# Emanem/spath

Measured on AMD Instinct MI355X. Metric: Mray/s (primary x spp x bounces), higher is better.
Workload: dtype f32 (stage-1 filter: f16 hi/lo products on the matrix pipe, f32 accumulate)

## Files before the change

spath_amd/csrc/sp_cyl_scan.h:

```cpp
#pragma once

#include "sp_kernels.h"
#include "sp_filter_scan.h"

namespace sp {

#ifndef SP_CYL_TILE
#define SP_CYL_TILE 384
#endif
constexpr uint32_t kCylTile = SP_CYL_TILE;
static_assert(kCylTile % 128 == 0, "whole waves per LDS-DMA pass, whole words of group bits");
constexpr uint32_t kCylTileQ = 2u * kCylTile;
constexpr uint32_t kCylGroups = kCylTile / 4u;
SP_DEV constexpr uint32_t cyl_slot(uint32_t group, uint32_t chunk) { return chunk * kCylGroups + group; }

struct CylStream {
	const float4* rec;
	const uint32_t* hdr;
	const float4* big;
};

SP_DEV void cyl_store(float4* __restrict__ tile, uint32_t grp, uint32_t u, const float4 q0, const float4 q1) {
	tile[cyl_slot(grp, u)] = q0;
	float* mh = (float*)(tile + cyl_slot(grp, 4u + (u >> 1))) + 2u * (u & 1u);
	mh[0] = q1.x; mh[1] = q1.y;
	((float*)(tile + cyl_slot(grp, 6u)))[u] = q1.z;
	if (u == 0u) tile[cyl_slot(grp, 7u)] = make_float4(0.0f, 0.0f, 0.0f, 0.0f);
}

struct CylGroup {
	float4 q0[4];
	float4 mh01, mh23;
};
SP_DEV CylGroup cyl_group(const float4* tile, uint32_t grp) {
	CylGroup G;
#pragma unroll
	for (int u = 0; u < 4; ++u) G.q0[u] = tile[cyl_slot(grp, (uint32_t)u)];
	G.mh01 = tile[cyl_slot(grp, 4u)]; G.mh23 = tile[cyl_slot(grp, 5u)];
	return G;
}
SP_DEV float cyl_mz(const CylGroup& G, int u) { return u == 0 ? G.mh01.x : u == 1 ? G.mh01.z : u == 2 ? G.mh23.x : G.mh23.z; }
SP_DEV float cyl_h(const CylGroup& G, int u) { return u == 0 ? G.mh01.y : u == 1 ? G.mh01.w : u == 2 ? G.mh23.y : G.mh23.w; }

SP_DEV int cyl_record(const float* __restrict__ t, uint32_t idx, float4& q0, float4& q1) {
	const double A[3] = { t[0], t[1], t[2] }, B[3] = { t[3], t[4], t[5] }, C[3] = { t[6], t[7], t[8] };
	const double e1[3] = { (double)(t[3] - t[0]), (double)(t[4] - t[1]), (double)(t[5] - t[2]) };
	const double e2[3] = { (double)(t[6] - t[0]), (double)(t[7] - t[1]), (double)(t[8] - t[2]) };
	const double c[3] = { e2[0] - e1[0], e2[1] - e1[1], e2[2] - e1[2] };
	const double l1 = e1[0] * e1[0] + e1[1] * e1[1] + e1[2] * e1[2];
	const double l2 = e2[0] * e2[0] + e2[1] * e2[1] + e2[2] * e2[2];
	const double lc = c[0] * c[0] + c[1] * c[1] + c[2] * c[2];
	const double* w3; const double* p0; const double* p1; double len2;
	if (l2 >= l1 && l2 >= lc) { w3 = e2; p0 = A; p1 = B; len2 = l2; }
	else if (l1 >= lc)        { w3 = e1; p0 = A; p1 = C; len2 = l1; }
	else                      { w3 = c;  p0 = B; p1 = A; len2 = lc; }
	const double len = sqrt(len2);
	const double w[3] = { w3[0] / len, w3[1] / len, w3[2] / len };
	const double ax = fabs(w[0]), ay = fabs(w[1]), az = fabs(w[2]);
	const int a = (ax >= ay && ax >= az) ? 0 : (ay >= az ? 1 : 2);
	const int b = a == 2 ? 0 : a + 1, cc = b == 2 ? 0 : b + 1;
	const double s = 1.0 / w[a];
	const double pc[3] = { 0.5 * (p0[0] + p1[0]), 0.5 * (p0[1] + p1[1]), 0.5 * (p0[2] + p1[2]) };
	const double ph[3] = { 0.5 * (p1[0] - p0[0]), 0.5 * (p1[1] - p0[1]), 0.5 * (p1[2] - p0[2]) };
	const double mc[3] = { (w[1] * pc[2] - w[2] * pc[1]) * s, (w[2] * pc[0] - w[0] * pc[2]) * s, (w[0] * pc[1] - w[1] * pc[0]) * s };
	const double hv[3] = { (w[1] * ph[2] - w[2] * ph[1]) * s, (w[2] * ph[0] - w[0] * ph[2]) * s, (w[0] * ph[1] - w[1] * ph[0]) * s };
	const float beta = (float)(w[b] * s), gamma = (float)(w[cc] * s);
	const float mx = (float)mc[0], my = (float)mc[1], mz = (float)mc[2];
	float H = (float)(sqrt(hv[0] * hv[0] + hv[1] * hv[1] + hv[2] * hv[2]) * (1.0 + 0x1p-20));
	const float chk = beta + gamma + mx + my + mz + H;
	const bool ok = (chk - chk) == 0.0f;
	q0 = ok ? make_float4(beta, gamma, mx, my) : make_float4(0.0f, 0.0f, 0.0f, 0.0f);
	q1 = make_float4(ok ? mz : 0.0f, ok ? H : __builtin_inff(), __uint_as_float(idx), 0.0f);
	return ok ? a : 0;
}

SP_DEV int cyl_class(const float* __restrict__ t) {
	float4 q0, q1;
	return cyl_record(t, 0u, q0, q1);
}

__global__ void __launch_bounds__(256) k_cyl_count(const float* __restrict__ tris, uint32_t n, uint32_t* __restrict__ block_counts) {
	const uint32_t i = blockIdx.x * 256u + threadIdx.x;
	const int cls = i < n ? cyl_class(tris + (size_t)i * 12) : -1;
#pragma unroll
	for (int k = 0; k < 3; ++k) {
		const int cnt = __syncthreads_count(cls == k);
		if (threadIdx.x == 0) block_counts[(size_t)blockIdx.x * 3 + k] = (uint32_t)cnt;
	}
}

__global__ void __launch_bounds__(256) k_cyl_offsets(uint32_t* __restrict__ block_counts, uint32_t nblocks, uint32_t* __restrict__ hdr, uint32_t tile_sz) {
	__shared__ uint32_t part[256];
	__shared__ uint32_t total[3];
	const uint32_t tid = threadIdx.x;
	const uint32_t per = (nblocks + 255u) / 256u;
	const uint32_t lo = tid * per < nblocks ? tid * per : nblocks, hi = lo + per < nblocks ? lo + per : nblocks;
	for (int k = 0; k < 3; ++k) {
		uint32_t sum = 0;
		for (uint32_t b = lo; b < hi; ++b) sum += block_counts[(size_t)b * 3 + k];
		part[tid] = sum;
		__syncthreads();
		if (tid == 0) {
			uint32_t run = 0;
			for (int j = 0; j < 256; ++j) { const uint32_t v = part[j]; part[j] = run; run += v; }
			total[k] = run;
		}
		__syncthreads();
		uint32_t run = part[tid];
		for (uint32_t b = lo; b < hi; ++b) { const uint32_t v = block_counts[(size_t)b * 3 + k]; block_counts[(size_t)b * 3 + k] = run; run += v; }
		__syncthreads();
	}
	if (tid == 0) {
		uint32_t tile = 0;
		for (int k = 0; k < 3; ++k) { hdr[k] = total[k]; hdr[3 + k] = tile; tile += (total[k] + tile_sz - 1u) / tile_sz; }
		hdr[6] = tile;
	}
}

__global__ void __launch_bounds__(256) k_cyl_scatter(const float* __restrict__ tris, uint32_t n, const uint32_t* __restrict__ block_offsets,
                                                    const uint32_t* __restrict__ hdr, float4* __restrict__ rec) {
	__shared__ uint32_t wave_cnt[4][3];
	const uint32_t tid = threadIdx.x, i = blockIdx.x * 256u + tid, wv = tid >> 6, lane = tid & 63u;
	float4 q0, q1;
	q0 = q1 = make_float4(0.0f, 0.0f, 0.0f, 0.0f);
	const int cls = i < n ? cyl_record(tris + (size_t)i * 12, i, q0, q1) : -1;
	uint32_t rank = 0;
#pragma unroll
	for (int k = 0; k < 3; ++k) {
		const unsigned long long m = __ballot(cls == k);
		if (cls == k) rank = (uint32_t)__popcll(m & ((1ull << lane) - 1ull));
		if (lane == 0) wave_cnt[wv][k] = (uint32_t)__popcll(m);
	}
	__syncthreads();
	if (cls >= 0) {
		for (uint32_t v = 0; v < wv; ++v) rank += wave_cnt[v][cls];
		const size_t pos = (size_t)hdr[3 + cls] * kCylTile + block_offsets[(size_t)blockIdx.x * 3 + cls] + rank;
		const size_t tile = pos / kCylTile;
		const uint32_t in_tile = (uint32_t)(pos - tile * kCylTile), grp = in_tile >> 2, u = in_tile & 3u;
		cyl_store(rec + tile * kCylTileQ, grp, u, q0, q1);
	}
}

__global__ void __launch_bounds__(256) k_cyl_pad(const uint32_t* __restrict__ hdr, uint32_t n_tris, float4* __restrict__ rec) {
	const uint32_t k = blockIdx.x, tid = threadIdx.x;
	const uint32_t n = hdr[k], first = hdr[3 + k] * kCylTile;
	for (uint32_t pos = n + tid; pos < (n + kCylTile - 1u) / kCylTile * kCylTile; pos += 256u) {
		const size_t gpos = (size_t)first + pos, tile = gpos / kCylTile;
		const uint32_t in_tile = (uint32_t)(gpos - tile * kCylTile), grp = in_tile >> 2, u = in_tile & 3u;
		cyl_store(rec + tile * kCylTileQ, grp, u, make_float4(0.0f, 0.0f, 0.0f, 0.0f), make_float4(0.0f, -__builtin_inff(), __uint_as_float(n_tris), 0.0f));
	}
}

SP_DEV void cyl_tile_dma(const float4* __restrict__ src, float4* dst, uint32_t tid, uint32_t wbase) {
	typedef __attribute__((address_space(1))) const void* gptr_t;
	typedef __attribute__((address_space(3))) void* lptr_t;
	static_assert(kCylTileQ % 256 == 0, "whole workgroup passes");
#pragma unroll
	for (int p = 0; p < (int)(kCylTileQ / 256u); ++p)
		__builtin_amdgcn_global_load_lds((gptr_t)(src + p * 256 + tid), (lptr_t)(dst + p * 256 + wbase), 16, 0, 0);
}

SP_DEV float cyl_x(const float4 q0, float mz, float H, float Pa, float Pb, float Pc, float ndx, float ndy, float ndz, float D) {
	float gm = __builtin_fmaf(q0.x, Pb, Pa);
	gm = __builtin_fmaf(q0.y, Pc, gm);
	gm = __builtin_fmaf(ndx, q0.z, gm);
	gm = __builtin_fmaf(ndy, q0.w, gm);
	gm = __builtin_fmaf(ndz, mz, gm);
	return __builtin_fmaf(-H, D, __builtin_fabsf(gm));
}

template <int R>
struct CylRay {
	float Pa[R], Pb[R], Pc[R];
	float ndx[R], ndy[R], ndz[R];
	float D[R], Dq[R];
};

template <int R>
SP_DEV void cyl_setup(float rv, const RaySlots<R>& s, CylRay<R>& f) {
#pragma unroll
	for (int r = 0; r < R; ++r) {
		const f3 P = cross3(s.o[r], s.dir[r]);
		const float adx = fabsf(s.dir[r].x), ady = fabsf(s.dir[r].y), adz = fabsf(s.dir[r].z);
		const float dn = adx + ady + adz;
		const float on = fabsf(s.o[r].x) + fabsf(s.o[r].y) + fabsf(s.o[r].z);
		const float dmax = fmaxf(adx, fmaxf(ady, adz));
		const float mag = dn * (on + 2.0f * rv);
		const bool fin = (mag < 1e37f) && (dmax > 1e-18f) && (dmax < 1e18f);
		const bool on_ = fin && s.act[r];
		f.Pa[r] = on_ ? P.x : 0.0f; f.Pb[r] = on_ ? P.y : 0.0f; f.Pc[r] = on_ ? P.z : 0.0f;
		f.ndx[r] = on_ ? -s.dir[r].x : 0.0f; f.ndy[r] = on_ ? -s.dir[r].y : 0.0f; f.ndz[r] = on_ ? -s.dir[r].z : 0.0f;
		f.D[r] = on_ ? __builtin_sqrtf(s.dir[r].x * s.dir[r].x + s.dir[r].y * s.dir[r].y + s.dir[r].z * s.dir[r].z) * (1.0f + 0x1p-21f) : 1.0f;
		const float dq = fmaxf(0x1p-16f * 1.01f * mag * (1.0f + 0x1p-20f), 1e-37f);
		f.Dq[r] = !s.act[r] ? -__builtin_inff() : (fin ? dq : __builtin_inff());
	}
}

template <int R>
SP_DEV void scan_cyl(const KArgs& a, const CylStream cs, float rv, const RaySlots<R>& s, float (&bd)[R], int (&bi)[R]) {
	__shared__ float4 sm[2 * kCylTileQ];
	static_assert(R == 1 || R == 2 || R == 4, "bits per group must divide 32");
	constexpr uint32_t kGPW = 32u / R;
	constexpr int kNW = (int)((kCylTile / 4u) / kGPW);
	__shared__ uint32_t wq[kNW * 256];
	const uint32_t tid = threadIdx.x;
	const uint32_t wbase = tid & ~63u;

	CylRay<R> f;
	cyl_setup<R>(rv, s, f);
#pragma unroll
	for (int r = 0; r < R; ++r) { bd[r] = kMaxDist; bi[r] = -1; }

	const uint32_t total_tiles = cs.hdr[6];
	uint32_t cls = 0;
	__syncthreads();
	cyl_tile_dma(cs.rec, sm, tid, wbase);
	__syncthreads();
	for (uint32_t gt = 0; gt < total_tiles; ++gt) {
		while (cls < 2u && gt >= cs.hdr[4 + cls]) {
#pragma unroll
			for (int r = 0; r < R; ++r) { const float t0 = f.Pa[r]; f.Pa[r] = f.Pb[r]; f.Pb[r] = f.Pc[r]; f.Pc[r] = t0; }
			++cls;
		}
		const float4* cur = sm + (gt & 1u) * kCylTileQ;
		const uint32_t left = cs.hdr[cls] - (gt - cs.hdr[3 + cls]) * kCylTile;
		const uint32_t ngroups = (uint32_t)__builtin_amdgcn_readfirstlane((int)(((left < kCylTile ? left : kCylTile) + 3u) / 4u));
		uint32_t nz = 0;
		uint32_t g = 0;
#pragma unroll
		for (int wi = 0; wi < kNW; ++wi) {
			uint32_t wv = 0;
			const uint32_t gend = ngroups < (uint32_t)(wi + 1) * kGPW ? ngroups : (uint32_t)(wi + 1) * kGPW;
			const uint32_t g0 = g;
			for (; g < gend; ++g) {
				const CylGroup G = cyl_group(cur, g);
#pragma unroll
				for (int r = 0; r < R; ++r) {
					float x[4];
#pragma unroll
					for (int u = 0; u < 4; ++u) x[u] = cyl_x(G.q0[u], cyl_mz(G, u), cyl_h(G, u), f.Pa[r], f.Pb[r], f.Pc[r], f.ndx[r], f.ndy[r], f.ndz[r], f.D[r]);
					const float m = __builtin_fminf(__builtin_fminf(x[0], x[1]), __builtin_fminf(x[2], x[3]));
					wv = __builtin_amdgcn_alignbit(wv, __float_as_uint(m - f.Dq[r]), 31);
				}
			}
			const uint32_t done = (g - g0) * R;
			const uint32_t wd = done == 0u ? 0u : (wv << (32u - done));
			wq[wi * 256 + tid] = wd;
			nz |= (wd != 0u ? 1u : 0u) << wi;
		}
		if (gt + 1u < total_tiles) cyl_tile_dma(cs.rec + (size_t)(gt + 1u) * kCylTileQ, sm + ((gt + 1u) & 1u) * kCylTileQ, tid, wbase);
#ifdef SP_FILTER_STATS
		uint32_t st_bits = 0, st_rounds = 0, st_exact = 0;
#pragma unroll
		for (int wi = 0; wi < kNW; ++wi) st_bits += (uint32_t)__builtin_popcount(wq[wi * 256 + tid]);
#endif
		uint32_t sub = 0;
		uint32_t wid = nz ? (uint32_t)__builtin_ctz(nz) : 0u;
		uint32_t curw = nz ? wq[wid * 256 + tid] : 0u;
		for (;;) {
			if (!__any(nz != 0u)) break;
#ifdef SP_FILTER_STATS
			++st_rounds;
#endif
			if (nz != 0u) {
				const uint32_t nz2 = nz & (nz - 1u);
				const uint32_t wid2 = nz2 ? (uint32_t)__builtin_ctz(nz2) : 0u;
				const uint32_t nextw = wq[wid2 * 256 + tid];
				const uint32_t e = (uint32_t)__builtin_clz(curw);
				const uint32_t grp = wid * kGPW + e / R;
				const int slot = (int)(e % R);
				float Pa = f.Pa[0], Pb = f.Pb[0], Pc = f.Pc[0], ndx = f.ndx[0], ndy = f.ndy[0], ndz = f.ndz[0], D = f.D[0], Dq = f.Dq[0];
				float ox = s.o[0].x, oy = s.o[0].y, oz = s.o[0].z;
				float dx = s.dir[0].x, dy = s.dir[0].y, dz = s.dir[0].z;
				int src = s.src[0];
				float best = bd[0]; int besti = bi[0];
#pragma unroll
				for (int r = 1; r < R; ++r) {
					const bool pick = (slot == r);
					Pa = pick ? f.Pa[r] : Pa; Pb = pick ? f.Pb[r] : Pb; Pc = pick ? f.Pc[r] : Pc;
					ndx = pick ? f.ndx[r] : ndx; ndy = pick ? f.ndy[r] : ndy; ndz = pick ? f.ndz[r] : ndz;
					D = pick ? f.D[r] : D; Dq = pick ? f.Dq[r] : Dq;
					ox = pick ? s.o[r].x : ox; oy = pick ? s.o[r].y : oy; oz = pick ? s.o[r].z : oz;
					dx = pick ? s.dir[r].x : dx; dy = pick ? s.dir[r].y : dy; dz = pick ? s.dir[r].z : dz;
					src = pick ? s.src[r] : src;
					best = pick ? bd[r] : best; besti = pick ? bi[r] : besti;
				}
				uint32_t cand = 0; int idx = 0;
				const CylGroup G = cyl_group(cur, grp);
				const float4 gi = cur[cyl_slot(grp, 6u)];
#pragma unroll
				for (int u = 3; u >= 0; --u) {
					const float x = cyl_x(G.q0[u], cyl_mz(G, u), cyl_h(G, u), Pa, Pb, Pc, ndx, ndy, ndz, D);
					const bool sv = !(x - Dq >= 0.0f) && !((sub >> u) & 1u);
					cand = sv ? (cand | (1u << u)) : cand;
					idx = sv ? (int)__float_as_uint(u == 0 ? gi.x : u == 1 ? gi.y : u == 2 ? gi.z : gi.w) : idx;
				}
				const uint32_t lowest = cand & (0u - cand);
				const bool last = (cand == lowest);
				sub = last ? 0u : (sub | lowest);
				curw = last ? (curw & ~(0x80000000u >> e)) : curw;
				if (cand != 0u) {
#ifdef SP_FILTER_STATS
					++st_exact;
#endif
					const float4 x0 = a.scan[3 * (size_t)idx + 0], x1 = a.scan[3 * (size_t)idx + 1], x2 = a.scan[3 * (size_t)idx + 2];
					const float d = ray_tri_strict(mk3(ox, oy, oz), mk3(dx, dy, dz), mk3(x0.x, x0.y, x0.z), mk3(x0.w, x1.x, x1.y), mk3(x1.z, x1.w, x2.x));
					const bool take = (d > 0.0f) && (idx != src) && ((d < best) || (d == best && idx < besti));
					best = take ? d : best;
					besti = take ? idx : besti;
#pragma unroll
					for (int r = 0; r < R; ++r) { const bool pick = (slot == r); bd[r] = pick ? best : bd[r]; bi[r] = pick ? besti : bi[r]; }
				}
				const bool adv = (curw == 0u);
				nz = adv ? nz2 : nz;
				wid = adv ? wid2 : wid;
				curw = adv ? nextw : curw;
			}
		}
#ifdef SP_FILTER_STATS
		{
			uint32_t v = st_bits, x = st_exact;
			for (int off = 32; off > 0; off >>= 1) { v += __shfl_xor(v, off, 64); x += __shfl_xor(x, off, 64); }
// ... 171 lines not shown
```

spath_amd/csrc/sp_cylm_scan.h:

```cpp
#ifndef SP_CYLM_NS
#error "include sp_cylm_both.h, not this file"
#endif

namespace sp { namespace SP_CYLM_NS {

typedef _Float16 half8 __attribute__((ext_vector_type(8)));
typedef float float16v __attribute__((ext_vector_type(16)));

#ifndef SP_CYLM_TILE
#define SP_CYLM_TILE SP_CYLM_THREADS
#endif

constexpr uint32_t kMThreads = SP_CYLM_THREADS;
constexpr uint32_t kMWaves = kMThreads / 64u;
constexpr uint32_t kMTile = SP_CYLM_TILE;
constexpr uint32_t kMGroups = kMTile / 4u;
constexpr uint32_t kMBlocks = kMTile / 32u;
#ifndef SP_CYLM_GROUP
#define SP_CYLM_GROUP 4
#endif
constexpr uint32_t kMGrp = SP_CYLM_GROUP;
static_assert(kMGrp == 4u || kMGrp == 8u, "quads or octets (all sixteen rows of a lane as one group: -8 % / -4 % at 10^5 / 10^6 triangles against octets)");
constexpr uint32_t kMBitsFrag = 16u / kMGrp;
constexpr uint32_t kMFragsPerWord = 32u / kMBitsFrag;
constexpr uint32_t kMWords = (kMBlocks * kMBitsFrag + 31u) / 32u;
constexpr uint32_t kMRecQ = kMGroups * 8u;
constexpr uint32_t kMTileQ = kMRecQ + kMBlocks * 64u;
static_assert(kMThreads % 64u == 0u && kMThreads <= 1024u, "whole waves");
static_assert(kMTileQ % kMThreads == 0u, "whole workgroup LDS-DMA passes");
static_assert(kMGroups <= 128u, "7-bit group index in a list entry");
static_assert(kMBlocks * 2u <= kMGroups, "the Hmax table fits chunk 7");
SP_DEV constexpr uint32_t cylm_slot(uint32_t group, uint32_t chunk) { return chunk * kMGroups + group; }
SP_DEV constexpr uint32_t cylm_hmq(uint32_t tb, uint32_t hh) { return 7u * kMGroups + tb * 2u + hh; }
SP_DEV constexpr uint32_t cylm_kq() { return 7u * kMGroups + kMBlocks * 2u; }
static_assert(kMBlocks * 2u + 1u <= kMGroups, "Hmax table and kappa fit chunk 7");

SP_DEV float cylm_scale(float rv) {
	if (!(rv > 1e-30f && rv < 1e30f)) return 0.0f;
	const uint32_t e = (__float_as_uint(rv) >> 23) & 255u;
	return __uint_as_float((e + 2u) << 23);
}

SP_DEV _Float16 to_half(float v) {
	uint32_t b = (uint32_t)__builtin_bit_cast(unsigned short, (_Float16)v);
#ifndef SP_CYLM_UNPINNED
	__asm__ volatile("" : "+v"(b));
#endif
	return __builtin_bit_cast(_Float16, (unsigned short)b);
}

SP_DEV void half_split(float v, _Float16& hi, _Float16& lo) {
	hi = to_half(v);
	lo = to_half(v - (float)hi);
}

SP_DEV void cylm_store(float4* __restrict__ tile, uint32_t in_tile, const float4 q0, const float4 q1, float S) {
	const uint32_t grp = in_tile >> 2, u = in_tile & 3u;
	tile[cylm_slot(grp, u)] = q0;
	float* mh = (float*)(tile + cylm_slot(grp, 4u + (u >> 1))) + 2u * (u & 1u);
	mh[0] = q1.x; mh[1] = q1.y;
	((float*)(tile + cylm_slot(grp, 6u)))[u] = q1.z;
	const float m = S > 0.0f ? 16.0f / S : 0.0f;
	_Float16 bh, bl, ch, cl, xh, xl, yh, yl, zh, zl;
	half_split(S > 0.0f ? 16.0f * q0.x : 0.0f, bh, bl); half_split(S > 0.0f ? 16.0f * q0.y : 0.0f, ch, cl);
	half_split(q0.z * m, xh, xl); half_split(q0.w * m, yh, yl); half_split(q1.x * m, zh, zl);
	const _Float16 z = (_Float16)0.0f;
	const half8 k0 = { bh, bl, bh, ch, cl, ch, xh, xl }, k1 = { xh, yh, yl, yh, zh, zl, zh, S > 0.0f ? (_Float16)16.0f : z };
	half8* frag = (half8*)(tile + kMRecQ) + (in_tile >> 5) * 64u + (in_tile & 31u);
	frag[0] = k0; frag[32] = k1;
}

constexpr uint32_t kMBig = 64u;
constexpr int kMBigLevels = 4;

SP_DEV int cylm_big_level(float H, float S) {
	if (!(S > 0.0f) || !(H < __builtin_inff())) return -1;
	const float r = H / S;
	return r >= 1.0f ? 3 : r >= 0.25f ? 2 : r >= 0.0625f ? 1 : r >= 0.015625f ? 0 : -1;
}

__global__ void __launch_bounds__(256) k_cylm_count_big(const float* __restrict__ tris, uint32_t n, const unsigned int* __restrict__ bounds, uint32_t* __restrict__ hdr) {
	const uint32_t i = blockIdx.x * 256u + threadIdx.x;
	const float S = cylm_scale(__uint_as_float(bounds[0]));
	int lvl = -1;
	if (i < n) {
		float4 q0, q1;
		(void)cyl_record(tris + (size_t)i * 12, i, q0, q1);
		lvl = cylm_big_level(q1.y, S);
	}
#pragma unroll
	for (int k = 0; k < kMBigLevels; ++k) {
		const int cnt = __syncthreads_count(lvl >= k);
		if (threadIdx.x == 0 && cnt) atomicAdd(hdr + 9 + k, (uint32_t)cnt);
	}
}

SP_DEV int cylm_big_threshold(const uint32_t* __restrict__ hdr) {
	for (int k = 0; k < kMBigLevels; ++k) if (hdr[9 + k] <= kMBig) return k;
	return kMBigLevels;
}

__global__ void __launch_bounds__(256) k_cylm_keys(const float* __restrict__ tris, uint32_t n, const unsigned int* __restrict__ bounds, uint32_t* __restrict__ keys,
                                                  uint32_t* __restrict__ vals, uint32_t* __restrict__ hdr) {
	const uint32_t i = blockIdx.x * 256u + threadIdx.x;
	const float S = cylm_scale(__uint_as_float(bounds[0]));
	const int thr = cylm_big_threshold(hdr);
	int cls = -1;
	if (i < n) {
		float4 q0, q1;
		cls = cyl_record(tris + (size_t)i * 12, i, q0, q1);
		const int lvl = cylm_big_level(q1.y, S);
		if (lvl >= 0 && lvl >= thr) cls = 3;
		keys[i] = ((uint32_t)cls << 30) | (__float_as_uint(q1.y) >> 2);
		vals[i] = i;
	}
#pragma unroll
	for (int k = 0; k < 4; ++k) {
		const int cnt = __syncthreads_count(cls == k);
		if (threadIdx.x == 0 && cnt) atomicAdd(hdr + (k < 3 ? k : 8), (uint32_t)cnt);
	}
}

__global__ void k_cylm_hdr(uint32_t* __restrict__ hdr, const unsigned int* __restrict__ bounds) {
	uint32_t tile = 0;
	for (int k = 0; k < 3; ++k) { hdr[3 + k] = tile; tile += (hdr[k] + kMTile - 1u) / kMTile; }
	hdr[6] = tile;
	((float*)hdr)[7] = cylm_scale(__uint_as_float(bounds[0]));
}

__global__ void __launch_bounds__(256) k_cylm_scatter(const float* __restrict__ tris, uint32_t n, const uint32_t* __restrict__ sorted,
                                                     const uint32_t* __restrict__ hdr, float4* __restrict__ rec, const float4* __restrict__ scan, float4* __restrict__ big) {
	const uint32_t p = blockIdx.x * 256u + threadIdx.x;
	if (p >= n) return;
	const uint32_t i = sorted[p];
	const float S = ((const float*)hdr)[7];
	const uint32_t n_stream = hdr[0] + hdr[1] + hdr[2];
	if (p >= n_stream) {
		const uint32_t b = p - n_stream;
		const float4 x2 = scan[3 * (size_t)i + 2];
		big[3 * b + 0] = scan[3 * (size_t)i + 0]; big[3 * b + 1] = scan[3 * (size_t)i + 1];
		big[3 * b + 2] = make_float4(x2.x, __uint_as_float(i), 0.0f, 0.0f);
		return;
	}
	float4 q0, q1;
	const int cls = cyl_record(tris + (size_t)i * 12, i, q0, q1);
	const uint32_t c0 = cls == 0 ? 0u : cls == 1 ? hdr[0] : hdr[0] + hdr[1];
	const size_t pos = (size_t)hdr[3 + cls] * kMTile + (p - c0);
	const size_t tile = pos / kMTile;
	cylm_store(rec + tile * kMTileQ, (uint32_t)(pos - tile * kMTile), q0, q1, S);
}

__global__ void __launch_bounds__(256) k_cylm_pad(const uint32_t* __restrict__ hdr, uint32_t n_tris, float4* __restrict__ rec) {
	const uint32_t k = blockIdx.x, tid = threadIdx.x;
	const uint32_t n = hdr[k], first = hdr[3 + k] * kMTile;
	const float S = ((const float*)hdr)[7];
	for (uint32_t pos = n + tid; pos < (n + kMTile - 1u) / kMTile * kMTile; pos += 256u) {
		const size_t gpos = (size_t)first + pos, tile = gpos / kMTile;
		cylm_store(rec + tile * kMTileQ, (uint32_t)(gpos - tile * kMTile), make_float4(0.0f, 0.0f, 0.0f, 0.0f),
		           make_float4(0.0f, -__builtin_inff(), __uint_as_float(n_tris), 0.0f), S);
	}
}

__global__ void __launch_bounds__(kMGroups) k_cylm_hmax(const uint32_t* __restrict__ hdr, float4* __restrict__ rec) {
	__shared__ uint32_t s_max, s_min;
	__shared__ float s_h[kMGroups];
	if (blockIdx.x >= hdr[6]) return;
	if (threadIdx.x == 0) { s_max = 0u; s_min = 0x7f800000u; }
	float4* tile = rec + (size_t)blockIdx.x * kMTileQ;
	const uint32_t grp = threadIdx.x, tb = grp >> 3, j = (grp & 7u) >> 1, hh = grp & 1u;
	const float S = ((const float*)hdr)[7];
	const float k = S > 0.0f ? 256.0f / S : 1.0f;
	const float4 a = tile[cylm_slot(grp, 4u)], b = tile[cylm_slot(grp, 5u)];
	s_h[grp] = fmaxf(fmaxf(a.y, a.w), fmaxf(b.y, b.w)) * k;
	__syncthreads();
	float hm = kMGrp == 8u ? fmaxf(s_h[grp], s_h[grp ^ 2u]) : s_h[grp];
	const bool regular = hm >= 0.0f && hm < __builtin_inff();
	if (regular) atomicMax(&s_max, __float_as_uint(hm));
	__syncthreads();
	const float floor_ = fmaxf(__uint_as_float(s_max) * 0x1p-10f, 0x1p-60f);
	if (regular) { hm = fmaxf(hm, floor_); atomicMin(&s_min, __float_as_uint(hm)); }
	__syncthreads();
	if (kMGrp == 4u) ((float*)(tile + cylm_hmq(tb, hh)))[j] = hm;
	else if ((j & 1u) == 0u) ((float*)(tile + cylm_hmq(tb, hh)))[j >> 1] = hm;
	if (threadIdx.x == 0) {
		const float hmin = s_min == 0x7f800000u ? 1.0f : __uint_as_float(s_min);
		tile[cylm_kq()] = make_float4((1.0f / hmin) * (1.0f + 0x1p-20f), 0.0f, 0.0f, 0.0f);
	}
}

SP_DEV void cylm_tile_dma(const float4* __restrict__ src, float4* dst, uint32_t tid, uint32_t wbase) {
	typedef __attribute__((address_space(1))) const void* gptr_t;
	typedef __attribute__((address_space(3))) void* lptr_t;
#pragma unroll
	for (int p = 0; p < (int)(kMTileQ / kMThreads); ++p)
		__builtin_amdgcn_global_load_lds((gptr_t)(src + p * kMThreads + tid), (lptr_t)(dst + p * kMThreads + wbase), 16, 0, 0);
}

struct CylmGroup { float4 q0[4]; float4 mh01, mh23; };
SP_DEV CylmGroup cylm_group(const float4* tile, uint32_t grp) {
	CylmGroup G;
#pragma unroll
	for (int u = 0; u < 4; ++u) G.q0[u] = tile[cylm_slot(grp, (uint32_t)u)];
	G.mh01 = tile[cylm_slot(grp, 4u)]; G.mh23 = tile[cylm_slot(grp, 5u)];
	return G;
}

__global__ void __launch_bounds__(64) k_selftest_cylm(const float* __restrict__ in, uint32_t n, float* __restrict__ out) {
	const uint32_t i = blockIdx.x, lane = threadIdx.x, hh = lane >> 5;
	if (i >= n) return;
	const float* q = in + 12 * (size_t)i;
	_Float16 th[5], tl[5], rh[5], rl[5];
#pragma unroll
	for (int k = 0; k < 5; ++k) { half_split(q[k], th[k], tl[k]); half_split(q[5 + k], rh[k], rl[k]); }
	const _Float16 ah = to_half(q[10]), z = (_Float16)0.0f, one16 = (_Float16)16.0f;
	const half8 a0 = { th[0], tl[0], th[0], th[1], tl[1], th[1], th[2], tl[2] }, a1 = { th[2], th[3], tl[3], th[3], th[4], tl[4], th[4], one16 };
	const half8 b0 = { rh[0], rh[0], rl[0], rh[1], rh[1], rl[1], rh[2], rh[2] }, b1 = { rl[2], rh[3], rh[3], rl[3], rh[4], rh[4], rl[4], ah };
	const half8 zero8 = { z, z, z, z, z, z, z, z };
	const bool mine = (lane & 31u) == 0u;
	const half8 af = mine ? (hh ? a1 : a0) : zero8, bf = mine ? (hh ? b1 : b0) : zero8;
	float16v c;
#pragma unroll
	for (int k = 0; k < 16; ++k) c[k] = 0.0f;
	const float16v g = __builtin_amdgcn_mfma_f32_32x32x16_f16(af, bf, c, 0, 0, 0);
	if (lane == 0) {
		double sum = 0.0;
#pragma unroll
		for (int k = 0; k < 8; ++k) sum += (double)(float)a0[k] * (double)(float)b0[k] + (double)(float)a1[k] * (double)(float)b1[k];
		out[2 * (size_t)i] = g[0];
		out[2 * (size_t)i + 1] = (float)sum;
	}
}

struct CylmHdr {
	uint32_t n0, n1, n2, f1, f2, tiles;
	uint32_t nbig;
	float S;
	uint32_t cls, cn, cfirst, cend;
	SP_DEV void load(const uint32_t* __restrict__ hdr) {
		n0 = (uint32_t)__builtin_amdgcn_readfirstlane((int)hdr[0]); n1 = (uint32_t)__builtin_amdgcn_readfirstlane((int)hdr[1]);
		n2 = (uint32_t)__builtin_amdgcn_readfirstlane((int)hdr[2]);
		f1 = (uint32_t)__builtin_amdgcn_readfirstlane((int)hdr[4]); f2 = (uint32_t)__builtin_amdgcn_readfirstlane((int)hdr[5]);
		tiles = (uint32_t)__builtin_amdgcn_readfirstlane((int)hdr[6]);
		S = __uint_as_float((uint32_t)__builtin_amdgcn_readfirstlane((int)hdr[7]));
		nbig = (uint32_t)__builtin_amdgcn_readfirstlane((int)hdr[8]);
		cls = 0u; cn = n0; cfirst = 0u; cend = f1;
	}
	SP_DEV bool next_class(uint32_t gt) {
		if (cls >= 2u || gt < cend) return false;
		++cls;
		if (cls == 1u) { cn = n1; cfirst = f1; cend = f2; } else { cn = n2; cfirst = f2; cend = tiles; }
		return true;
	}
	SP_DEV uint32_t fragments(uint32_t gt) const {
		const uint32_t left = cn - (gt - cfirst) * kMTile;
		return ((left < kMTile ? left : kMTile) + 31u) / 32u;
	}
};

struct CylmRay {
	CylRay<1> f;
	float Pw[3], Nw[3];
	float Dh, Dqh;
	bool on_m;
	half8 bfr[2];
	float Dn[2], Dqn[2];

	SP_DEV void setup(float rv, float S, const RaySlots<1>& s) {
		cyl_setup<1>(rv, s, f);
		const float adx = fabsf(s.dir[0].x), ady = fabsf(s.dir[0].y), adz = fabsf(s.dir[0].z);
		const float on = fabsf(s.o[0].x) + fabsf(s.o[0].y) + fabsf(s.o[0].z);
		const float dmax = fmaxf(adx, fmaxf(ady, adz));
		const bool on0 = (f.Dq[0] < __builtin_inff()) && (f.Dq[0] > 0.0f) && (S > 0.0f) && (on + 2.0f * rv <= 512.0f * S);
		const uint32_t ed = (__float_as_uint(dmax) >> 23) & 255u;
		const float sd0 = on0 ? __uint_as_float((254u - ed) << 23) : 0.0f;
		const float kP0 = on0 ? sd0 * (16.0f / S) : 0.0f, kC0 = on0 ? sd0 * (256.0f / S) : 0.0f;
		on_m = on0 && (kC0 < 1e30f) && (kP0 > 1e-30f);
		const float s_d = on_m ? sd0 : 0.0f;
		const float kP = on_m ? kP0 : 0.0f, kN = 16.0f * s_d, kC = on_m ? kC0 : 0.0f;
		Dh = on_m ? f.D[0] * s_d : 1.0f;
		Dqh = on_m ? f.Dq[0] * kC : (s.act[0] ? __builtin_inff() : -__builtin_inff());
		Pw[0] = f.Pa[0] * kP; Pw[1] = f.Pb[0] * kP; Pw[2] = f.Pc[0] * kP;
		Nw[0] = f.ndx[0] * kN; Nw[1] = f.ndy[0] * kN; Nw[2] = f.ndz[0] * kN;
	}

	SP_DEV void build(uint32_t cls, uint32_t lane) {
		const uint32_t hh = lane >> 5;
		const float Pa_ = cls == 0u ? Pw[0] : cls == 1u ? Pw[1] : Pw[2];
		const float Pb_ = cls == 0u ? Pw[1] : cls == 1u ? Pw[2] : Pw[0], Pc_ = cls == 0u ? Pw[2] : cls == 1u ? Pw[0] : Pw[1];
		const _Float16 ah = to_half(Pa_);
		const float fa = (float)ah;
		const bool big = fabsf(Pa_) >= 0x1p-10f;
		const float t = big ? fa / Pa_ : 1.0f;
		const float extra = big ? 0.0f : fabsf(Pa_ - fa) * 16.0f;
		_Float16 bh, bl, ch, cl, nh[3], nl[3];
		half_split(Pb_ * t, bh, bl); half_split(Pc_ * t, ch, cl);
		half_split(Nw[0] * t, nh[0], nl[0]); half_split(Nw[1] * t, nh[1], nl[1]); half_split(Nw[2] * t, nh[2], nl[2]);
		const half8 k0 = { bh, bh, bl, ch, ch, cl, nh[0], nh[0] };
		const half8 k1 = { nl[0], nh[1], nh[1], nl[1], nh[2], nh[2], nl[2], ah };
		const float Dt = Dh * t;
		const float Dqt = on_m ? (Dqh * t + extra) * (1.0f + 0x1p-20f) : Dqh;
		typedef int int4v __attribute__((ext_vector_type(4)));
		const int4v v0 = __builtin_bit_cast(int4v, k0), v1 = __builtin_bit_cast(int4v, k1);
#pragma unroll
		for (int rb = 0; rb < 2; ++rb) {
			const int src = (int)((lane & 31u) + 32u * (uint32_t)rb);
			int4v o;
#pragma unroll
			for (int c = 0; c < 4; ++c) { const int va = __shfl(v0[c], src, 64), vb = __shfl(v1[c], src, 64); o[c] = hh ? vb : va; }
			bfr[rb] = __builtin_bit_cast(half8, o);
			Dn[rb] = __shfl(Dt, src, 64);
			Dqn[rb] = __shfl(Dqt, src, 64);
		}
	}
};

#ifndef SP_CYLM_MIN
#define SP_CYLM_MIN 1
#endif
SP_DEV float min4_abs(float a, float b, float c, float d) {
#if SP_CYLM_MIN == 1
	return __builtin_elementwise_minimum(__builtin_elementwise_minimum(__builtin_elementwise_minimum(__builtin_fabsf(a), __builtin_fabsf(b)), __builtin_fabsf(c)), __builtin_fabsf(d));
#elif SP_CYLM_MIN == 2
	return __builtin_fminf(__builtin_fminf(__builtin_amdgcn_fmed3f(__builtin_fabsf(a), __builtin_fabsf(b), 0.0f), __builtin_fabsf(c)), __builtin_fabsf(d));
#else
	return __builtin_fminf(__builtin_fminf(__builtin_fminf(__builtin_fabsf(a), __builtin_fabsf(b)), __builtin_fabsf(c)), __builtin_fabsf(d));
#endif
}

SP_DEV void cylm_tile_bound(const float4* cur, const CylmRay& R, float (&Dt)[2]) {
	const float kappa = cur[cylm_kq()].x;
#pragma unroll
	for (int rb = 0; rb < 2; ++rb) Dt[rb] = __builtin_fmaf(R.Dqn[rb], kappa, R.Dn[rb]) * (1.0f + 0x1p-22f);
}

SP_DEV float min8_abs(float a, float b, float c, float d, float e, float f, float g, float h) {
	typedef float T;
	const T m1 = __builtin_elementwise_minimum(__builtin_elementwise_minimum(__builtin_fabsf(a), __builtin_fabsf(b)), __builtin_fabsf(c));
	const T m2 = __builtin_elementwise_minimum(__builtin_elementwise_minimum(__builtin_fabsf(d), __builtin_fabsf(e)), __builtin_fabsf(f));
	const T m3 = __builtin_elementwise_minimum(__builtin_elementwise_minimum(m1, __builtin_fabsf(g)), __builtin_fabsf(h));
	return __builtin_elementwise_minimum(m3, m2);
}

SP_DEV uint32_t cylm_bits(const float16v& g, const float4 Hm, float Dt, uint32_t word) {
	if constexpr (kMGrp == 4u) {
#pragma unroll
		for (int j = 0; j < 4; ++j) {
			const float hm = j == 0 ? Hm.x : j == 1 ? Hm.y : j == 2 ? Hm.z : Hm.w;
			const float m = min4_abs(g[4 * j + 0], g[4 * j + 1], g[4 * j + 2], g[4 * j + 3]);
			word = __builtin_amdgcn_alignbit(word, __float_as_uint(__builtin_fmaf(-hm, Dt, m)), 31);
		}
	} else {
#pragma unroll
		for (int q = 0; q < 2; ++q) {
			const float hm = q == 0 ? Hm.x : Hm.y;
			const float m = min8_abs(g[8 * q + 0], g[8 * q + 1], g[8 * q + 2], g[8 * q + 3], g[8 * q + 4], g[8 * q + 5], g[8 * q + 6], g[8 * q + 7]);
			word = __builtin_amdgcn_alignbit(word, __float_as_uint(__builtin_fmaf(-hm, Dt, m)), 31);
		}
	}
	return word;
}

SP_DEV void cylm_stage1(const float4* cur, uint32_t tb0, uint32_t nblk, uint32_t lane, const CylmRay& R, const float (&Dt)[2], uint32_t (&word)[2]) {
	if (nblk == 0u) return;
	const half8* frags = (const half8*)(cur + kMRecQ) + tb0 * 64u + lane;
	const float4* hmq = cur + cylm_hmq(tb0, lane >> 5);
	float16v zero;
#pragma unroll
	for (int i = 0; i < 16; ++i) zero[i] = 0.0f;
#define SP_S1_STEP(afr_cur_Hm, afr_next)                                                     \
		__builtin_amdgcn_sched_barrier(0);                                                   \
		word[0] = cylm_bits(g0, afr_cur_Hm, Dt[0], word[0]);                                 \
		__builtin_amdgcn_sched_barrier(0);                                                   \
		g0 = __builtin_amdgcn_mfma_f32_32x32x16_f16(afr_next, R.bfr[0], zero, 0, 0, 0);      \
		__builtin_amdgcn_sched_barrier(0);                                                   \
		word[1] = cylm_bits(g1, afr_cur_Hm, Dt[1], word[1]);                                 \
		__builtin_amdgcn_sched_barrier(0);                                                   \
		g1 = __builtin_amdgcn_mfma_f32_32x32x16_f16(afr_next, R.bfr[1], zero, 0, 0, 0);
	half8 afrA = frags[0], afrB;
	float4 HmA = hmq[0], HmB;
	float16v g0 = __builtin_amdgcn_mfma_f32_32x32x16_f16(afrA, R.bfr[0], zero, 0, 0, 0);
	float16v g1 = __builtin_amdgcn_mfma_f32_32x32x16_f16(afrA, R.bfr[1], zero, 0, 0, 0);
	uint32_t tb = 1;
	for (; tb + 1u < nblk; tb += 2u) {
		afrB = frags[tb * 64u]; HmB = hmq[tb * 2u];
		SP_S1_STEP(HmA, afrB)
		afrA = frags[(tb + 1u) * 64u]; HmA = hmq[(tb + 1u) * 2u];
		SP_S1_STEP(HmB, afrA)
	}
	if (tb < nblk) {
		afrB = frags[tb * 64u]; HmB = hmq[tb * 2u];
		SP_S1_STEP(HmA, afrB)
		HmA = HmB;
	}
#undef SP_S1_STEP
	word[0] = cylm_bits(g0, HmA, Dt[0], word[0]);
	word[1] = cylm_bits(g1, HmA, Dt[1], word[1]);
}

constexpr uint32_t kMCap = 384u;
constexpr uint32_t kMQ2 = 128u;
constexpr uint32_t kMIdxBits = 26u;

SP_DEV float wave_fetch(uint32_t addr4, float v) { return __int_as_float(__builtin_amdgcn_ds_bpermute((int)addr4, __float_as_int(v))); }
SP_DEV int wave_fetch(uint32_t addr4, int v) { return __builtin_amdgcn_ds_bpermute((int)addr4, v); }

SP_DEV uint32_t wave_incl_scan(uint32_t x) {
	x += (uint32_t)__builtin_amdgcn_update_dpp(0, (int)x, 0x111, 0xf, 0xf, true);
	x += (uint32_t)__builtin_amdgcn_update_dpp(0, (int)x, 0x112, 0xf, 0xf, true);
	x += (uint32_t)__builtin_amdgcn_update_dpp(0, (int)x, 0x114, 0xf, 0xf, true);
	x += (uint32_t)__builtin_amdgcn_update_dpp(0, (int)x, 0x118, 0xf, 0xf, true);
	x += (uint32_t)__builtin_amdgcn_update_dpp(0, (int)x, 0x142, 0xa, 0xf, false);
	x += (uint32_t)__builtin_amdgcn_update_dpp(0, (int)x, 0x143, 0xc, 0xf, false);
	return x;
}

template <bool BOUNDED = false>
SP_DEV void scan_cylm(const KArgs& a, const CylStream cs, float rv, const RaySlots<1>& s, float (&bd)[1], int (&bi)[1],
                      const float* tmax = nullptr, bool shadow = false) {
	__shared__ float4 sm0[kMTileQ];
	__shared__ float4 sm1[kMTileQ];
	__shared__ unsigned short lst[kMWaves * kMCap];
	__shared__ uint32_t q2[kMWaves * kMQ2];
	__shared__ unsigned long long cell[kMThreads];
	const uint32_t tid = threadIdx.x, lane = tid & 63u, wbase = tid & ~63u, hh = lane >> 5;
	unsigned short* const mylst = lst + (tid >> 6) * kMCap;
	uint32_t* const myq2 = q2 + (tid >> 6) * kMQ2;
	CylmHdr hd;
	hd.load(cs.hdr);

	CylmRay R;
	R.setup(rv, hd.S, s);
	CylRay<1>& f = R.f;

	const float tm = tmax ? tmax[0] : kMaxDist;
	{
		float bd0 = tm; int bi0 = -1;
		typedef float f4v __attribute__((ext_vector_type(4)));
		typedef __attribute__((address_space(4))) const f4v* cptr_t;
		const cptr_t big = (cptr_t)(uintptr_t)cs.big;
		for (uint32_t b = 0; b < hd.nbig; ++b) {
			const f4v x0 = big[3 * b + 0], x1 = big[3 * b + 1], x2 = big[3 * b + 2];
			const int idx = (int)__float_as_uint(x2.y);
			const float d = ray_tri_strict(s.o[0], s.dir[0], mk3(x0.x, x0.y, x0.z), mk3(x0.w, x1.x, x1.y), mk3(x1.z, x1.w, x2.x));
			const bool take = (d > 0.0f) && (idx != s.src[0]) && ((d < bd0) || (d == bd0 && idx < bi0));
			bd0 = take ? d : bd0;
			bi0 = take ? idx : bi0;
		}
		cell[tid] = ((unsigned long long)__float_as_uint(bd0) << 32) | (unsigned long long)(uint32_t)bi0;
		if (BOUNDED && shadow && !s.act[0]) cell[tid] = 0ull;
	}
	R.build(0u, lane);

	uint32_t q2n = 0;
	auto exact_batch = [&](uint32_t n) {
#ifdef SP_EXP_NO_EXACT
		q2n -= n;
		return;
#endif
		const bool ok = lane < n;
		const uint32_t e = ok ? myq2[q2n - n + lane] : ((lane << kMIdxBits) | a.n_tris);
		const uint32_t la = (e >> (kMIdxBits - 2u)) & 0xfcu;
		const int idx = (int)(e & ((1u << kMIdxBits) - 1u));
		const float4* const rec = (const float4*)((const char*)a.scan + ((((uint32_t)idx << 1) + (uint32_t)idx) << 4));
		const float4 x0 = rec[0], x1 = rec[1], x2 = rec[2];
		const float ox = wave_fetch(la, s.o[0].x), oy = wave_fetch(la, s.o[0].y), oz = wave_fetch(la, s.o[0].z);
		const float dx = wave_fetch(la, s.dir[0].x), dy = wave_fetch(la, s.dir[0].y), dz = wave_fetch(la, s.dir[0].z);
		const int src = wave_fetch(la, s.src[0]);
		const float tmx = tmax ? wave_fetch(la, tm) : kMaxDist;
		const float d = ray_tri_strict(mk3(ox, oy, oz), mk3(dx, dy, dz), mk3(x0.x, x0.y, x0.z), mk3(x0.w, x1.x, x1.y), mk3(x1.z, x1.w, x2.x));
		if (ok && (d > 0.0f) && (d < tmx) && (idx != src))
			atomicMin(&cell[wbase + (la >> 2)], ((unsigned long long)__float_as_uint(d) << 32) | (unsigned long long)(uint32_t)idx);
		q2n -= n;
#ifdef SP_FILTER_STATS
		if (lane == 0) { atomicAdd(a.scans + 5, 1ull); atomicAdd(a.scans + 4, (unsigned long long)n); }
#endif
	};

	const uint32_t total_tiles = hd.tiles;
#ifdef SP_EXP_NO_STAGE2
	uint32_t exp_acc = 0;
#endif
#ifdef SP_PHASE_TIMERS
	unsigned long long ph_s1 = 0, ph_list = 0, ph_retest = 0, ph_exact = 0, ph_bar = 0, ph_t0 = 0, ph_t1 = 0;
#define SP_PH_STAMP(v) v = __builtin_amdgcn_s_memtime()
#define SP_PH_ADD(acc, a_, b_) acc += (b_) - (a_)
#else
#define SP_PH_STAMP(v)
#define SP_PH_ADD(acc, a_, b_)
#endif
	__syncthreads();
	cylm_tile_dma(cs.rec, sm0, tid, wbase);
	__syncthreads();
	auto tile_body = [&](auto parity, const uint32_t gt) {
		const float4* const cur = decltype(parity)::value ? sm1 : sm0;
		float4* const nxt = decltype(parity)::value ? sm0 : sm1;
#ifndef SP_CYLM_LATE_DMA
		if (gt + 1u < total_tiles) cylm_tile_dma(cs.rec + (size_t)(gt + 1u) * kMTileQ, nxt, tid, wbase);
#endif
		SP_PH_STAMP(ph_t0);
		while (hd.next_class(gt)) {
			const float t0 = f.Pa[0]; f.Pa[0] = f.Pb[0]; f.Pb[0] = f.Pc[0]; f.Pc[0] = t0;
			R.build(hd.cls, lane);
		}
		const uint32_t nblk = hd.fragments(gt);
		float Dt[2];
		cylm_tile_bound(cur, R, Dt);
		uint32_t word[kMWords][2];
#pragma unroll
		for (int w = 0; w < (int)kMWords; ++w) {
			word[w][0] = word[w][1] = 0u;
			const uint32_t tb0 = kMFragsPerWord * (uint32_t)w;
			const uint32_t nb = nblk > tb0 ? (nblk - tb0 < kMFragsPerWord ? nblk - tb0 : kMFragsPerWord) : 0u;
			cylm_stage1(cur, tb0, nb, lane, R, Dt, word[w]);
			const uint32_t done = nb * kMBitsFrag;
#pragma unroll
			for (int rb = 0; rb < 2; ++rb) word[w][rb] = done == 0u ? 0u : (word[w][rb] << (32u - done));
#ifdef SP_DBG_ALLBITS
			word[w][0] = word[w][1] = done == 0u ? 0u : (0xffffffffu << (32u - done));
#endif
		}
		if (BOUNDED && shadow) {
#pragma unroll
			for (int rb = 0; rb < 2; ++rb) {
				const bool fin = (uint32_t)cell[wbase + (lane & 31u) + 32u * (uint32_t)rb] != 0xffffffffu;
#pragma unroll
				for (int w = 0; w < (int)kMWords; ++w) word[w][rb] = fin ? 0u : word[w][rb];
			}
		}
		SP_PH_STAMP(ph_t1); SP_PH_ADD(ph_s1, ph_t0, ph_t1);
#ifdef SP_CYLM_LATE_DMA
		if (gt + 1u < total_tiles) cylm_tile_dma(cs.rec + (size_t)(gt + 1u) * kMTileQ, nxt, tid, wbase);
#endif
#ifdef SP_EXP_NO_STAGE2
		for (int w = 0; w < (int)kMWords; ++w) exp_acc ^= word[w][0] ^ word[w][1];
		for (; false;) {
#else
		for (;;) {
#endif
			uint32_t c = 0;
#pragma unroll
			for (int w = 0; w < (int)kMWords; ++w) c += (uint32_t)__builtin_popcount(word[w][0]) + (uint32_t)__builtin_popcount(word[w][1]);
			const uint32_t incl = wave_incl_scan(c);
			const uint32_t all = (uint32_t)__builtin_amdgcn_readlane((int)incl, 63);
			if (all == 0u) break;
			uint32_t j = incl - c;
			const uint32_t jend = incl < kMCap ? incl : kMCap;
			if (all <= kMCap) {
#pragma unroll
				for (int w = 0; w < (int)kMWords; ++w)
#pragma unroll
				for (int rb = 0; rb < 2; ++rb) {
					uint32_t m = word[w][rb];
					const uint32_t eb = (((lane & 31u) + 32u * (uint32_t)rb) << 2) | ((16u * kMGrp * (uint32_t)w + hh) << 8);
					while (m != 0u) {
						const uint32_t e = (uint32_t)__builtin_clz(m);
						mylst[j++] = (unsigned short)(eb + (e << (kMGrp == 8u ? 10 : 9)));
						m &= ~(0x80000000u >> e);
					}
					word[w][rb] = 0u;
				}
			} else
#pragma unroll
			for (int w = 0; w < (int)kMWords; ++w)
#pragma unroll
			for (int rb = 0; rb < 2; ++rb) {
				uint32_t m = word[w][rb];
				const uint32_t ray = (lane & 31u) + 32u * (uint32_t)rb;
				while (__any(m != 0u && j < jend)) {
					if (m != 0u && j < jend) {
						const uint32_t e = (uint32_t)__builtin_clz(m);
						mylst[j++] = (unsigned short)((ray << 2) | ((16u * kMGrp * (uint32_t)w + (kMGrp / 2u) * e + hh) << 8));
						m &= ~(0x80000000u >> e);
					}
				}
				word[w][rb] = m;
			}
			__builtin_amdgcn_wave_barrier();
			const uint32_t total = all < kMCap ? all : kMCap;
#ifdef SP_FILTER_STATS
			if (lane == 0) { atomicAdd(a.scans + 1, (unsigned long long)total); atomicAdd(a.scans + 2, (unsigned long long)((total + 63u) / 64u)); }
#endif
			SP_PH_STAMP(ph_t0); SP_PH_ADD(ph_list, ph_t1, ph_t0);
			for (uint32_t base = 0; base < total; base += 64u) {
				const uint32_t ent = base + lane;
				const bool ok = ent < total;
				const uint32_t entry = ok ? (uint32_t)mylst[ent] : (lane << 2);
				const uint32_t la = entry & 0xfcu;
				const uint32_t grp = entry >> 8;
				const float dx = wave_fetch(la, s.dir[0].x), dy = wave_fetch(la, s.dir[0].y), dz = wave_fetch(la, s.dir[0].z);
				const float Pa = wave_fetch(la, f.Pa[0]), Pb = wave_fetch(la, f.Pb[0]), Pc = wave_fetch(la, f.Pc[0]);
				const float D = wave_fetch(la, f.D[0]), Dq = wave_fetch(la, f.Dq[0]);
				uint32_t cand = 0;
#pragma unroll
				for (int h = 0; h < (int)(kMGrp / 4u); ++h) {
					const CylmGroup G = cylm_group(cur, grp + 2u * (uint32_t)h);
#pragma unroll
					for (int u = 0; u < 4; ++u) {
						const float mz = u == 0 ? G.mh01.x : u == 1 ? G.mh01.z : u == 2 ? G.mh23.x : G.mh23.z;
						const float Hh = u == 0 ? G.mh01.y : u == 1 ? G.mh01.w : u == 2 ? G.mh23.y : G.mh23.w;
						const float x = cyl_x(G.q0[u], mz, Hh, Pa, Pb, Pc, -dx, -dy, -dz, D);
						cand = __builtin_amdgcn_alignbit(cand, __float_as_uint(x - Dq), 31);
					}
				}
				cand = ok ? cand : 0u;
				SP_PH_STAMP(ph_t1); SP_PH_ADD(ph_retest, ph_t0, ph_t1);
				const uint32_t* const gidx = (const uint32_t*)(cur + cylm_slot(grp, 6u));
				const uint32_t lhi = la << (kMIdxBits - 2u);
				for (;;) {
					const bool mine = cand != 0u;
					const unsigned long long mk = __ballot(mine);
					if (mk == 0ull) break;
					const uint32_t cnt = (uint32_t)__popcll(mk);
					if (q2n + cnt > kMQ2) exact_batch(64u);
					const uint32_t k = mine ? (uint32_t)__builtin_ctz(cand) : kMGrp - 1u;
					const uint32_t u = kMGrp - 1u - k;
					const uint32_t idx = gidx[8u * (u >> 2) + (u & 3u)];
					if (mine) myq2[q2n + __builtin_amdgcn_mbcnt_hi((uint32_t)(mk >> 32), __builtin_amdgcn_mbcnt_lo((uint32_t)mk, 0u))] = lhi | idx;
					q2n += cnt;
					cand &= cand - 1u;
				}
				__builtin_amdgcn_wave_barrier();
				SP_PH_STAMP(ph_t0); SP_PH_ADD(ph_exact, ph_t1, ph_t0);
			}
			SP_PH_STAMP(ph_t1);
		}
#ifdef SP_EXP_DRAIN_ALL
		while (q2n) exact_batch(q2n < 64u ? q2n : 64u);
#else
		while (q2n >= 64u) exact_batch(64u);
#endif
#ifdef SP_FILTER_STATS
		if (lane == 0) atomicAdd(a.scans + 3, 1ull);
#endif
		SP_PH_STAMP(ph_t0); SP_PH_ADD(ph_list, ph_t1, ph_t0);
		if (BOUNDED && shadow) {
			__asm__ volatile("s_waitcnt vmcnt(0)" ::: "memory");
			if (!__syncthreads_or((uint32_t)cell[tid] == 0xffffffffu ? 1 : 0)) return false;
		} else
		__syncthreads();
		SP_PH_STAMP(ph_t1); SP_PH_ADD(ph_bar, ph_t0, ph_t1);
		return true;
	};
	if constexpr (BOUNDED) {
		bool all_done = false;
		for (uint32_t gt = 0; gt < total_tiles; gt += 2u) {
			if (!tile_body(std::integral_constant<int, 0>{}, gt)) { all_done = true; break; }
			if (gt + 1u < total_tiles && !tile_body(std::integral_constant<int, 1>{}, gt + 1u)) { all_done = true; break; }
		}
		if (q2n && !all_done) exact_batch(q2n);
	} else {
		for (uint32_t gt = 0; gt < total_tiles; gt += 2u) {
			tile_body(std::integral_constant<int, 0>{}, gt);
			if (gt + 1u < total_tiles) tile_body(std::integral_constant<int, 1>{}, gt + 1u);
		}
		if (q2n) exact_batch(q2n);
	}
#ifdef SP_PHASE_TIMERS
	if (lane == 0) {
		atomicAdd(a.scans + 8, ph_s1); atomicAdd(a.scans + 9, ph_list); atomicAdd(a.scans + 10, ph_retest); atomicAdd(a.scans + 11, ph_exact);
		atomicAdd(a.scans + 12, ph_bar); atomicAdd(a.scans + 13, 1ull);
	}
#endif
#ifdef SP_EXP_NO_STAGE2
	if (exp_acc == 0x12345678u) cell[tid] = 0ull;
#endif
	__builtin_amdgcn_wave_barrier();
	const unsigned long long k = cell[tid];
	bd[0] = __uint_as_float((uint32_t)(k >> 32));
	bi[0] = (int)(uint32_t)k;
}

__global__ void __launch_bounds__(64) k_selftest_stage1(const float* __restrict__ rays, uint32_t n_rays, const CylStream cs, const unsigned int* __restrict__ bounds,
                                                      uint32_t* __restrict__ out_words, uint32_t* __restrict__ out_tri, int* __restrict__ out_order) {
	__shared__ float4 sm[kMTileQ];
	const uint32_t lane = threadIdx.x, hh = lane >> 5;
	const float rv = __uint_as_float(bounds[0]);
	CylmHdr hd;
	hd.load(cs.hdr);
	const uint32_t k = blockIdx.x * 64u + lane, kk = k < n_rays ? k : n_rays - 1u;
	RaySlots<1> s;
	const float* p = rays + (size_t)kk * 6;
	s.o[0] = mk3(p[0], p[1], p[2]); s.dir[0] = mk3(p[3], p[4], p[5]); s.src[0] = -1; s.act[0] = true;
	CylmRay R;
	R.setup(rv, hd.S, s);
	R.build(0u, lane);
	const float kH = hd.S > 0.0f ? 256.0f / hd.S : 1.0f;
	const uint32_t total_tiles = hd.tiles;
	for (uint32_t gt = 0; gt < total_tiles; ++gt) {
		while (hd.next_class(gt)) R.build(hd.cls, lane);
		__syncthreads();
		for (uint32_t q = lane; q < kMTileQ; q += 64u) sm[q] = cs.rec[(size_t)gt * kMTileQ + q];
		__syncthreads();
		const uint32_t nblk = hd.fragments(gt);
		float Dt[2];
		cylm_tile_bound(sm, R, Dt);
		for (uint32_t w = 0; w < kMWords; ++w) {
			uint32_t word[2] = { 0u, 0u };
			const uint32_t tb0 = kMFragsPerWord * w;
			const uint32_t nb = nblk > tb0 ? (nblk - tb0 < kMFragsPerWord ? nblk - tb0 : kMFragsPerWord) : 0u;
			cylm_stage1(sm, tb0, nb, lane, R, Dt, word);
			const uint32_t done = nb * kMBitsFrag;
#pragma unroll
			for (int rb = 0; rb < 2; ++rb)
				if (k < n_rays) out_words[(((size_t)k * total_tiles + gt) * 2u + (uint32_t)rb) * kMWords + w] = done == 0u ? 0u : (word[rb] << (32u - done));
		}
		if (out_tri) {
			float16v zero;
#pragma unroll
			for (int i = 0; i < 16; ++i) zero[i] = 0.0f;
			for (uint32_t tb = 0; tb < kMBlocks; ++tb) {
				const half8 afr = ((const half8*)(sm + kMRecQ))[tb * 64u + lane];
				const float16v g0 = __builtin_amdgcn_mfma_f32_32x32x16_f16(afr, R.bfr[0], zero, 0, 0, 0);
				const float16v g1 = __builtin_amdgcn_mfma_f32_32x32x16_f16(afr, R.bfr[1], zero, 0, 0, 0);
#pragma unroll
				for (int rb = 0; rb < 2; ++rb) {
					const float16v& g = rb == 0 ? g0 : g1;
					uint32_t w = 0;
#pragma unroll
					for (int j = 0; j < 4; ++j) {
						const uint32_t grp = tb * 8u + 2u * (uint32_t)j + hh;
						const float4 a = sm[cylm_slot(grp, 4u)], b = sm[cylm_slot(grp, 5u)];
						const float H4[4] = { a.y * kH, a.w * kH, b.y * kH, b.w * kH };
#pragma unroll
						for (int i = 0; i < 4; ++i) {
							const float x = __builtin_fmaf(-H4[i], R.Dn[rb], __builtin_fabsf(g[4 * j + i]));
							w = __builtin_amdgcn_alignbit(w, __float_as_uint(x - R.Dqn[rb]), 31);
						}
					}
					if (k < n_rays) {
						uint32_t* o = out_tri + (((size_t)k * total_tiles + gt) * 2u + (uint32_t)rb) * (kMTile / 64u) + (tb >> 1);
						if (tb >= nblk) w = 0u;
						if ((tb & 1u) == 0u) *o = w << 16; else *o |= (w & 0xffffu);
					}
				}
			}
		}
		if (blockIdx.x == 0) {
			for (uint32_t grp = lane; grp < kMGroups; grp += 64u) {
				const float4 gi = sm[cylm_slot(grp, 6u)];
				int* o = out_order + (size_t)gt * kMTile + 4u * grp;
				o[0] = (int)__float_as_uint(gi.x); o[1] = (int)__float_as_uint(gi.y); o[2] = (int)__float_as_uint(gi.z); o[3] = (int)__float_as_uint(gi.w);
			}
		}
	}
}

} }
#undef SP_PH_STAMP
#undef SP_PH_ADD
```

spath_amd/csrc/spath_hip.hip:

```cpp
#include "spath_hip.h"
#include "sp_kernels.h"
#include "sp_filter_scan.h"
#include "sp_cyl_scan.h"
#include "sp_scan_kernels.h"
#include "sp_bvh.h"
#include "sp_bvh_build.h"
#include "sp_adaptive.h"
#include "sp_denoise.h"

#include <hip/hip_runtime.h>

#include <cstdarg>
#include <cstdlib>
#include <dlfcn.h>
#include <thread>
#include <mutex>
#include <cstdio>
#include <cstring>
#include <algorithm>
#include <cmath>
#include <string>
#include <vector>

namespace {

thread_local std::string g_create_error;

struct DevBuf {
	void* p = nullptr;
	size_t cap = 0;
};

}

struct sphip_ctx {
	int device = 0;
	hipStream_t own_stream = nullptr;
	hipEvent_t ev_k0 = nullptr, ev_k1 = nullptr, ev_u0 = nullptr, ev_u1 = nullptr, ev_d0 = nullptr, ev_d1 = nullptr;
	DevBuf tris, mats, scan, filt, bounds, samp, rays, rgba, accum, counter, work, bvh_nodes, bvh_rec, bvh_idx, sort_kv, sort_hist, bvh_meta, cyl_rec, cyl_cnt, cyl_hdr, prim, cylm_rec, cylm_hdr, cylm_big;
	bool bvh_valid = false, filt_valid = false, cyl_valid = false, cylm_valid = false;
	bool cylm_wide = false;
	uint32_t bvh_leaves = 0;
	size_t n_tris = 0;
	bool have_scene = false;
	bool have_render = false, timed_upload = false, timed_download = false;
	sphip_stats stats{};
	std::string err;
	std::string desc;
	hipStream_t last_stream = nullptr;
	std::vector<sphip_ctx*> kids;
	int gather_kind = SPHIP_GATHER_NONE;
	void* rccl_lib = nullptr;
	std::vector<void*> comms;
	DevBuf gath, gath_acc, img, img_acc;
	std::vector<hipEvent_t> ev_tile;
	hipEvent_t ev_g0 = nullptr, ev_g1 = nullptr;
	DevBuf acc_rays, acc_sum;
	bool acc_on = false;
	bool acc_stale = false;
	size_t acc_w = 0, acc_h = 0;
	uint64_t acc_seed = 0, acc_total = 0;
	int acc_flags = 0;
	DevBuf adp_s12, adp_cnt, adp_list[2], adp_rays, adp_keep, adp_blk, adp_nact_d, adp_wst;
	bool adp_on = false;
	int adp_cur = 0;
	uint32_t adp_nact = 0, adp_nact_rb = 0;
	double adp_t = 0.0, adp_floor = 0.0;
	uint32_t adp_min = 0;
	DevBuf dn_cls, dn_hit, dn_gbuf, dn_a, dn_b, dn_rays;
	bool dn_cls_valid = false;
	DevBuf nee_tab;
	bool nee_valid = false, nee_bad = false;
	uint32_t nee_n = 0;
	double nee_W = 0.0;
	std::string nee_msg;
	bool dn_gbuf_ok = false;
	sphip_lens lens{};
	sphip_lens acc_lens{};
	sphip_camera acc_cam{};
	bool acc_has_cam = false;
	DevBuf spec;
	bool have_spec = false;
};

namespace {

int fail(sphip_ctx* c, int code, const char* fmt, ...) {
	char buf[512];
	va_list ap;
	va_start(ap, fmt);
	vsnprintf(buf, sizeof buf, fmt, ap);
	va_end(ap);
	if (c) c->err = buf; else g_create_error = buf;
	return code;
}

#define HIP_TRY(c, expr)                                                                         \
	do {                                                                                         \
		hipError_t e_ = (expr);                                                                  \
		if (e_ != hipSuccess)                                                                    \
			return fail((c), SPHIP_E_DEVICE, "%s failed: %s (%s:%d)", #expr, hipGetErrorString(e_), __FILE__, __LINE__); \
	} while (0)

int ensure(sphip_ctx* c, DevBuf& b, size_t bytes) {
	if (bytes <= b.cap && b.p) return SPHIP_OK;
	if (b.p) { HIP_TRY(c, hipFree(b.p)); b.p = nullptr; b.cap = 0; }
	const size_t want = bytes < 256 ? 256 : bytes;
	HIP_TRY(c, hipMalloc(&b.p, want));
	b.cap = want;
	return SPHIP_OK;
}

constexpr int kVariantAccel = 8;
constexpr int kVariantLast = 16;
constexpr uint64_t kChunkTargetBlocks = 262144;
constexpr uint64_t kChunkMaxBytes = 16ull << 30;
const char* const kVariantNames[kVariantLast + 1] = { "auto", "rpl_sload", "rpl_lds", "rpl_filter2", "rpl_filter4", "rpl_filter1", "rpl_filter2s", "rpl_filter4s",
                                                      "accel_lbvh", "rpl_cyl1", "rpl_cyl2", "rpl_cyl4", "rpl_cyl2s", "rpl_cyl4s", "rpl_cylw4", "rpl_cylw4s", "rpl_cylm" };

struct TwoStage { int R; bool split; int scan; };
bool two_stage(int variant, TwoStage* out) {
	static const TwoStage tab[kVariantLast + 1] = { {0, false, 0}, {0, false, 0}, {0, false, 0}, {2, false, 0}, {4, false, 0}, {1, false, 0}, {2, true, 0}, {4, true, 0},
	                                                {0, false, 0}, {1, false, 1}, {2, false, 1}, {4, false, 1}, {2, true, 1}, {4, true, 1}, {4, false, 2}, {4, true, 2}, {1, false, 3} };
	if (variant < 0 || variant > kVariantLast || tab[variant].R == 0) return false;
	if (out) *out = tab[variant];
	return true;
}

constexpr bool shape_shipped(int R, bool split, int scan) { return scan >= 3 || (scan == 2 && R == 4 && split); }
bool variant_shipped(int v) {
	TwoStage ts;
	return v == 1 || v == 2 || v == kVariantAccel || (two_stage(v, &ts) && shape_shipped(ts.R, ts.split, ts.scan));
}
bool variant_built(int v) {
#ifdef SP_ALL_VARIANTS
	return v >= 1 && v <= kVariantLast;
#else
	return variant_shipped(v);
#endif
}

constexpr size_t kSlotHist = 40, kSlotAcc = 12, kSlotNeeL = 48, kSlotMisD = 60, kSlotAdaptWst = 16;
constexpr size_t work_slot_bytes(bool nee, bool mis) { return kSlotHist + kSlotAcc + (mis ? kSlotMisD : nee ? kSlotNeeL : 0); }

int pick_variant(int flags, size_t n_tris) {
	if (flags & SPHIP_FLAG_ACCEL) return kVariantAccel;
	const int v = flags & SPHIP_KERNEL_MASK;
	if (v >= 1 && v <= kVariantLast) return v;
	if (n_tris < 64) return 1;
	if (n_tris >= (1ull << sp::kMIdxBits)) return 15;
	return 16;
}

int repack(sphip_ctx* c, hipStream_t st) {
	const uint32_t n = (uint32_t)c->n_tris;
	const uint32_t n_pad = (n / sp::kTile + 1) * sp::kTile;
	int rc;
	if ((rc = ensure(c, c->scan, (size_t)n_pad * 48)) || (rc = ensure(c, c->bounds, 256))) return rc;
	HIP_TRY(c, hipMemsetAsync(c->bounds.p, 0, 256, st));
	hipLaunchKernelGGL(sp::k_repack, dim3((n_pad + 255) / 256), dim3(256), 0, st,
	                   (const float*)c->tris.p, (float4*)c->scan.p, (unsigned int*)c->bounds.p, n, n_pad);
	HIP_TRY(c, hipGetLastError());
	c->have_scene = true;
	c->bvh_valid = c->filt_valid = c->cyl_valid = c->cylm_valid = false;
	c->nee_valid = false;
	c->have_spec = false;
	return SPHIP_OK;
}

int radix_sort(sphip_ctx* c, uint32_t n, uint32_t key_bits, hipStream_t st, int* out_half) {
	const uint32_t rs_blocks = (n + sp::kRsPerBlock - 1) / sp::kRsPerBlock;
	int rc = ensure(c, c->sort_hist, (size_t)rs_blocks * 16 * 4);
	if (rc) return rc;
	uint32_t* keys[2] = { (uint32_t*)c->sort_kv.p, (uint32_t*)c->sort_kv.p + (size_t)n };
	uint32_t* vals[2] = { (uint32_t*)c->sort_kv.p + (size_t)2 * n, (uint32_t*)c->sort_kv.p + (size_t)3 * n };
	int cur = 0;
	for (uint32_t shift = 0; shift < key_bits; shift += 4, cur ^= 1) {
		hipLaunchKernelGGL(sp::k_rs_hist, dim3(rs_blocks), dim3(256), 0, st, (const uint32_t*)keys[cur], n, shift, rs_blocks, (uint32_t*)c->sort_hist.p);
		hipLaunchKernelGGL(sp::k_rs_scan, dim3(1), dim3(256), 0, st, (uint32_t*)c->sort_hist.p, rs_blocks * 16u);
		hipLaunchKernelGGL(sp::k_rs_scatter, dim3(rs_blocks), dim3(256), 0, st, (const uint32_t*)keys[cur], (const uint32_t*)vals[cur], n, shift, rs_blocks,
		                   (const uint32_t*)c->sort_hist.p, keys[cur ^ 1], vals[cur ^ 1]);
	}
	HIP_TRY(c, hipGetLastError());
	*out_half = cur;
	return SPHIP_OK;
}

template <bool WIDE>
int build_cylm(sphip_ctx* c, hipStream_t st) {
#define SP_CM(x) (WIDE ? sp::cylm512::x : sp::cylm256::x)
	const uint32_t n = (uint32_t)c->n_tris, nblocks = (n + 255) / 256, max_tiles = n / SP_CM(kMTile) + 4;
	int rc;
	if ((rc = ensure(c, c->sort_kv, (size_t)n * 16)) || (rc = ensure(c, c->cylm_hdr, 256)) || (rc = ensure(c, c->cylm_big, sp::cylm256::kMBig * 48)) ||
	    (rc = ensure(c, c->cylm_rec, (size_t)max_tiles * SP_CM(kMTileQ) * 16))) return rc;
	uint32_t* keys = (uint32_t*)c->sort_kv.p;
	uint32_t* vals = (uint32_t*)c->sort_kv.p + (size_t)2 * n;
	uint32_t* hdr = (uint32_t*)c->cylm_hdr.p;
	const float* tris = (const float*)c->tris.p;
	const unsigned int* bnd = (const unsigned int*)c->bounds.p;
	float4* rec = (float4*)c->cylm_rec.p;
	HIP_TRY(c, hipMemsetAsync(hdr, 0, 256, st));
	hipLaunchKernelGGL(sp::cylm256::k_cylm_count_big, dim3(nblocks), dim3(256), 0, st, tris, n, bnd, hdr);
	hipLaunchKernelGGL(sp::cylm256::k_cylm_keys, dim3(nblocks), dim3(256), 0, st, tris, n, bnd, keys, vals, hdr);
	int half = 0;
	if ((rc = radix_sort(c, n, 32, st, &half))) return rc;
	const uint32_t* sorted = vals + (size_t)half * n;
	if (WIDE) {
		hipLaunchKernelGGL(sp::cylm512::k_cylm_hdr, dim3(1), dim3(1), 0, st, hdr, bnd);
		hipLaunchKernelGGL(sp::cylm512::k_cylm_scatter, dim3(nblocks), dim3(256), 0, st, tris, n, sorted, (const uint32_t*)hdr, rec, (const float4*)c->scan.p, (float4*)c->cylm_big.p);
		hipLaunchKernelGGL(sp::cylm512::k_cylm_pad, dim3(3), dim3(256), 0, st, (const uint32_t*)hdr, n, rec);
		hipLaunchKernelGGL(sp::cylm512::k_cylm_hmax, dim3(max_tiles), dim3(sp::cylm512::kMGroups), 0, st, (const uint32_t*)hdr, rec);
	} else {
		hipLaunchKernelGGL(sp::cylm256::k_cylm_hdr, dim3(1), dim3(1), 0, st, hdr, bnd);
		hipLaunchKernelGGL(sp::cylm256::k_cylm_scatter, dim3(nblocks), dim3(256), 0, st, tris, n, sorted, (const uint32_t*)hdr, rec, (const float4*)c->scan.p, (float4*)c->cylm_big.p);
		hipLaunchKernelGGL(sp::cylm256::k_cylm_pad, dim3(3), dim3(256), 0, st, (const uint32_t*)hdr, n, rec);
		hipLaunchKernelGGL(sp::cylm256::k_cylm_hmax, dim3(max_tiles), dim3(sp::cylm256::kMGroups), 0, st, (const uint32_t*)hdr, rec);
	}
#undef SP_CM
	HIP_TRY(c, hipGetLastError());
	c->cylm_valid = true;
	c->cylm_wide = WIDE;
	return SPHIP_OK;
}

bool cylm_wants_wide(const sphip_ctx* c) {
	if (const char* e = getenv("SPATH_HIP_CYLM_SHAPE")) return atoi(e) == 512;
	return c->n_tris >= sp::kMBigSceneTris;
}

int ensure_cylm(sphip_ctx* c, hipStream_t st) {
	if (c->cylm_valid) return SPHIP_OK;
	return cylm_wants_wide(c) ? build_cylm<true>(c, st) : build_cylm<false>(c, st);
}

int ensure_cyl(sphip_ctx* c, hipStream_t st) {
	if (c->cyl_valid) return SPHIP_OK;
	const uint32_t n = (uint32_t)c->n_tris, nblocks = (n + 255) / 256;
	int rc;
	if ((rc = ensure(c, c->cyl_cnt, (size_t)nblocks * 3 * sizeof(uint32_t))) || (rc = ensure(c, c->cyl_hdr, 256)) ||
	    (rc = ensure(c, c->cyl_rec, ((size_t)n / sp::kCylTile + 4) * sp::kCylTile * 32))) return rc;
	hipLaunchKernelGGL(sp::k_cyl_count, dim3(nblocks), dim3(256), 0, st, (const float*)c->tris.p, n, (uint32_t*)c->cyl_cnt.p);
	hipLaunchKernelGGL(sp::k_cyl_offsets, dim3(1), dim3(256), 0, st, (uint32_t*)c->cyl_cnt.p, nblocks, (uint32_t*)c->cyl_hdr.p, sp::kCylTile);
	hipLaunchKernelGGL(sp::k_cyl_scatter, dim3(nblocks), dim3(256), 0, st, (const float*)c->tris.p, n, (const uint32_t*)c->cyl_cnt.p,
	                   (const uint32_t*)c->cyl_hdr.p, (float4*)c->cyl_rec.p);
	hipLaunchKernelGGL(sp::k_cyl_pad, dim3(3), dim3(256), 0, st, (const uint32_t*)c->cyl_hdr.p, n, (float4*)c->cyl_rec.p);
	HIP_TRY(c, hipGetLastError());
	c->cyl_valid = true;
	return SPHIP_OK;
}

#ifdef SP_ALL_VARIANTS
int ensure_filt(sphip_ctx* c, hipStream_t st) {
	if (c->filt_valid) return SPHIP_OK;
	const uint32_t n = (uint32_t)c->n_tris, n_pad = (n / sp::kTile + 1) * sp::kTile;
	int rc = ensure(c, c->filt, (size_t)n_pad * 48);
	if (rc) return rc;
	hipLaunchKernelGGL(sp::k_repack_filter, dim3((n_pad + 255) / 256), dim3(256), 0, st, (const float*)c->tris.p, (float4*)c->filt.p, n, n_pad);
	HIP_TRY(c, hipGetLastError());
	c->filt_valid = true;
	return SPHIP_OK;
}
#endif

int ensure_bvh(sphip_ctx* c, hipStream_t st) {
	if (c->bvh_valid) return SPHIP_OK;
	const uint32_t n = (uint32_t)c->n_tris;
	uint32_t nl = 1;
	while ((uint64_t)nl * 4 < n) nl <<= 1;
	const uint32_t nblocks = (n + 255) / 256;
	int rc;
	if ((rc = ensure(c, c->bvh_nodes, (size_t)2 * nl * 32)) || (rc = ensure(c, c->bvh_rec, ((size_t)nl * 4 + sp::kBvhMaxBig) * 48)) ||
	    (rc = ensure(c, c->bvh_idx, ((size_t)nl * 4 + sp::kBvhMaxBig) * 4)) || (rc = ensure(c, c->sort_kv, (size_t)n * 16)) ||
	    (rc = ensure(c, c->bvh_meta, 256))) return rc;
	uint32_t* meta = (uint32_t*)c->bvh_meta.p;
	uint32_t* vals[2] = { (uint32_t*)c->sort_kv.p + (size_t)2 * n, (uint32_t*)c->sort_kv.p + (size_t)3 * n };
	const float* tris = (const float*)c->tris.p;
	const dim3 b256(256);
	hipLaunchKernelGGL(sp::k_bvh_meta_init, dim3(1), b256, 0, st, meta);
	hipLaunchKernelGGL(sp::k_bvh_box, dim3(nblocks), b256, 0, st, tris, n, meta);
	hipLaunchKernelGGL(sp::k_bvh_count_big, dim3(nblocks), b256, 0, st, tris, n, meta);
	hipLaunchKernelGGL(sp::k_bvh_keys, dim3(nblocks), b256, 0, st, tris, n, meta, (uint32_t*)c->sort_kv.p, vals[0]);
	int cur = 0;
	if ((rc = radix_sort(c, n, 32, st, &cur))) return rc;
	hipLaunchKernelGGL(sp::k_bvh_leaves, dim3((nl + 255) / 256), b256, 0, st, tris, n, (const uint32_t*)meta, (const uint32_t*)vals[cur], nl,
	                   (float4*)c->bvh_nodes.p, (float4*)c->bvh_rec.p, (int*)c->bvh_idx.p);
	hipLaunchKernelGGL(sp::k_bvh_bigs, dim3(1), b256, 0, st, tris, n, (const uint32_t*)meta, (const uint32_t*)vals[cur], nl, (float4*)c->bvh_rec.p, (int*)c->bvh_idx.p);
	for (uint32_t first = nl >> 1; first >= 1; first >>= 1)
		hipLaunchKernelGGL(sp::k_bvh_refit, dim3((first + 255) / 256), b256, 0, st, (float4*)c->bvh_nodes.p, first);
	HIP_TRY(c, hipGetLastError());
	c->bvh_leaves = nl;
	c->bvh_valid = true;
	return SPHIP_OK;
}

int ensure_lights(sphip_ctx* c, hipStream_t st) {
	if (c->nee_valid) return c->nee_bad ? fail(c, SPHIP_E_INVALID, "%s", c->nee_msg.c_str()) : SPHIP_OK;
	const size_t n = c->n_tris;
	std::vector<float> t(n * 12), m(n * 6);
	HIP_TRY(c, hipMemcpyAsync(t.data(), c->tris.p, n * 48, hipMemcpyDeviceToHost, st));
	HIP_TRY(c, hipMemcpyAsync(m.data(), c->mats.p, n * 24, hipMemcpyDeviceToHost, st));
	HIP_TRY(c, hipStreamSynchronize(st));
	std::vector<double> cdf;
	std::vector<int> tri;
	std::vector<float> ipdf;
	std::vector<double> esum;
	double W = 0.0;
	c->nee_bad = false;
	for (size_t i = 0; i < n; ++i) {
		const float* e = &m[i * 6 + 3];
		for (int k = 0; k < 3; ++k)
			if (!(e[k] >= 0.0f) || !std::isfinite(e[k])) {
				char buf[160];
				snprintf(buf, sizeof buf, "SPHIP_FLAG_NEE: triangle %zu has emittance component %d = %g (must be finite and >= 0)", i, k, (double)e[k]);
				c->nee_msg = buf;
				c->nee_bad = true;
				c->nee_valid = true;
				return fail(c, SPHIP_E_INVALID, "%s", buf);
			}
		const double es = ((double)e[0] + (double)e[1]) + (double)e[2];
		if (!(es > 0.0)) continue;
		const float* v = &t[i * 12];
		const double e1[3] = { (double)v[3] - (double)v[0], (double)v[4] - (double)v[1], (double)v[5] - (double)v[2] };
		const double e2[3] = { (double)v[6] - (double)v[0], (double)v[7] - (double)v[1], (double)v[8] - (double)v[2] };
		const double cx = e1[1] * e2[2] - e1[2] * e2[1], cy = e1[2] * e2[0] - e1[0] * e2[2], cz = e1[0] * e2[1] - e1[1] * e2[0];
		const double w = (0.5 * std::sqrt((cx * cx + cy * cy) + cz * cz)) * es;
		if (!(w > 0.0) || !std::isfinite(w)) continue;
		W = W + w;
		cdf.push_back(W); tri.push_back((int)i); esum.push_back(es);
	}
	const size_t ne = cdf.size();
	for (size_t k = 0; k < ne; ++k) ipdf.push_back((float)(W / esum[k]));
	std::vector<float> tipdf(n, 0.0f);
	for (size_t k = 0; k < ne; ++k) tipdf[(size_t)tri[k]] = ipdf[k];
	int rc;
	if ((rc = ensure(c, c->nee_tab, ne * 16 + n * 4 + 16))) return rc;
	std::vector<char> blob(ne * 16 + n * 4);
	memcpy(blob.data(), cdf.data(), ne * 8);
	memcpy(blob.data() + ne * 8, tri.data(), ne * 4);
	memcpy(blob.data() + ne * 12, ipdf.data(), ne * 4);
	memcpy(blob.data() + ne * 16, tipdf.data(), n * 4);
	if (!blob.empty()) {
		HIP_TRY(c, hipMemcpyAsync(c->nee_tab.p, blob.data(), blob.size(), hipMemcpyHostToDevice, st));
		HIP_TRY(c, hipStreamSynchronize(st));
	}
	c->nee_n = (uint32_t)ne;
	c->nee_W = W;
	c->nee_valid = true;
	return SPHIP_OK;
}

constexpr int kModeHits = 2;

template <typename F>
void with_accum(const sp::AccumArgs* prog, const sp::AdaptArgs* ad, F&& f) {
	if (ad) f(*ad);
	else if (prog) f(*prog);
	else f();
}
template <typename F>
void with_pack(const sp::AccumArgs* prog, const sp::AdaptArgs* ad, const sp::NeeArgs* ne, const sp::MisArgs* me, const sp::SpecArgs* spc,
               const sp::CamArgs* cam, F&& f) {
	with_accum(prog, ad, [&](const auto&... acc) {
		auto est = [&](const auto&... e) {
			auto tail = [&](const auto&... t) {
				if (cam) f(acc..., e..., t..., *cam);
				else f(acc..., e..., t...);
			};
			if constexpr (sizeof...(e) == 0 || sp::IsMis<std::decay_t<decltype(e)>...>::value) { if (spc) { tail(*spc); return; } }
			tail();
		};
		if (me) est(*me);
		else if (ne) est(*ne);
		else est();
	});
}

template <int R_, bool SPLIT_, int SCAN_> struct Shape {
	static constexpr int R = R_, SCAN = SCAN_;
	static constexpr bool SPLIT = SPLIT_, shipped = shape_shipped(R_, SPLIT_, SCAN_);
};
template <int SCAN, typename F>
void with_lane_shape(const TwoStage& ts, F&& f) {
	if (ts.split) { if (ts.R == 4) f(Shape<4, true, SCAN>{}); else f(Shape<2, true, SCAN>{}); }
	else if (ts.R == 4) f(Shape<4, false, SCAN>{});
	else if (ts.R == 2) f(Shape<2, false, SCAN>{});
	else f(Shape<1, false, SCAN>{});
}
template <typename F>
void with_scan_shape(const TwoStage& ts, F&& f) {
	if (ts.scan == 3) f(Shape<1, false, 3>{});
	else if (ts.scan == 4) f(Shape<1, false, 4>{});
	else if (ts.scan == 2 && ts.split) f(Shape<4, true, 2>{});
#ifdef SP_ALL_VARIANTS
	else if (ts.scan == 2) f(Shape<4, false, 2>{});
	else if (ts.scan == 1) with_lane_shape<1>(ts, f);
	else with_lane_shape<0>(ts, f);
#endif
}

int launch_render(sphip_ctx* c, const void* d_rays, size_t n_rays, const sphip_shard* shard, size_t ,
                  size_t n_samples, uint64_t seed, int mode, int flags, void* d_rgba, void* d_accum, hipStream_t st,
                  const int* d_src = nullptr, const sp::AccumArgs* prog = nullptr, const sp::AdaptArgs* adapt = nullptr,
                  const sp::CamArgs* cams = nullptr) {
	if (adapt) prog = adapt;
	if (!c->have_scene) return fail(c, SPHIP_E_STATE, "render called before a scene was set");
	if (!d_rays || !d_rgba) return fail(c, SPHIP_E_INVALID, "null ray or output pointer");
	if (n_rays == 0 || n_rays > 0xffffffffull) return fail(c, SPHIP_E_INVALID, "n_rays %zu out of range", n_rays);
	if (mode != SPHIP_MODE_FLAT && mode != SPHIP_MODE_PT && mode != kModeHits) return fail(c, SPHIP_E_INVALID, "unknown mode %d", mode);
	if (mode == kModeHits && !d_accum) return fail(c, SPHIP_E_INVALID, "null distance output");
	if (mode == SPHIP_MODE_PT && (n_samples == 0 || n_samples > 0x7fffffffull))
		return fail(c, SPHIP_E_INVALID, "n_samples must be in [1, 2^31) (the reference divides by it, cpu_renderer.cpp:77)");
	if (prog && (mode != SPHIP_MODE_PT || !prog->sum)) return fail(c, SPHIP_E_INVALID, "progressive accumulation needs path tracing and a sum buffer");
	if (prog && (uint64_t)prog->sample_base + n_samples > 0x7fffffffull)
		return fail(c, SPHIP_E_INVALID, "sample_base + n_samples = %llu: the total must stay below 2^31", (unsigned long long)prog->sample_base + n_samples);
	const uint64_t n_total = (prog ? (uint64_t)prog->sample_base : 0) + n_samples;
	int rc = ensure(c, c->counter, 16 * sizeof(unsigned long long));
	if (rc) return rc;

	sp::KArgs a{};
	a.rays = (const float*)d_rays;
	a.scan = (const float4*)c->scan.p;
	a.tris = (const float*)c->tris.p;
	a.mats = (const float*)c->mats.p;
	a.out_rgba = (uint32_t*)d_rgba;
	a.out_accum = (float*)d_accum;
	a.scans = (unsigned long long*)c->counter.p;
	a.n_rays = (uint32_t)n_rays;
	a.n_tris = (uint32_t)c->n_tris;
	a.n_samples = (uint32_t)n_samples;
	a.flags = (uint32_t)flags;
	a.seed = seed;
	if (shard) {
		if (shard->tile_px == 0) return fail(c, SPHIP_E_INVALID, "shard.tile_px must be > 0");
		a.pixel_base = shard->pixel_base; a.tile_px = shard->tile_px; a.tile_stride_px = shard->tile_stride_px;
	} else {
		a.pixel_base = 0; a.tile_px = n_rays; a.tile_stride_px = 0;
	}
	a.inv_n = (float)(1.0 / (double)(n_total ? n_total : 1));

	const int variant = pick_variant(flags, c->n_tris);
	if (variant == 16 && c->n_tris >= (1ull << sp::kMIdxBits))
		return fail(c, SPHIP_E_INVALID, "rpl_cylm handles scenes of fewer than 2^%u triangles (this one has %zu); use rpl_cylw4s", sp::kMIdxBits, c->n_tris);
	if (!variant_built(variant))
		return fail(c, SPHIP_E_INVALID, "kernel variant %d (%s) is not compiled into this build of libspath_hip (rebuild with -DSP_ALL_VARIANTS)", variant, kVariantNames[variant]);
	const bool nee = mode == SPHIP_MODE_PT && (flags & SPHIP_FLAG_NEE);
	const bool mis = mode == SPHIP_MODE_PT && (flags & SPHIP_FLAG_MIS);
	if (mis && !nee) return fail(c, SPHIP_E_INVALID, "SPHIP_FLAG_MIS needs SPHIP_FLAG_NEE");
	sp::NeeArgs ne{};
	if (nee) {
		if (!variant_shipped(variant))
			return fail(c, SPHIP_E_INVALID, "SPHIP_FLAG_NEE is not available with kernel variant %d (%s)", variant, kVariantNames[variant]);
		if ((rc = ensure_lights(c, st))) return rc;
		ne.cdf = (const double*)c->nee_tab.p;
		ne.tri = (const int*)((const char*)c->nee_tab.p + (size_t)c->nee_n * 8);
		ne.ipdf = (const float*)((const char*)c->nee_tab.p + (size_t)c->nee_n * 12);
		ne.n = c->nee_n;
		ne.W = c->nee_W;
	}
	const bool camf = mode == SPHIP_MODE_PT && (flags & SPHIP_FLAG_CAMERA_SAMPLES);
	if (camf && !cams)
		return fail(c, SPHIP_E_INVALID, "SPHIP_FLAG_CAMERA_SAMPLES needs a camera (sphip_render_camera, sphip_accum_begin[_adaptive] with cam), not rays");
	if (camf && (flags & SPHIP_FLAG_PRIMARY_REUSE))
		return fail(c, SPHIP_E_INVALID, "SPHIP_FLAG_CAMERA_SAMPLES and SPHIP_FLAG_PRIMARY_REUSE exclude each other (every sample has its own primary ray)");
	if (camf && !variant_shipped(variant))
		return fail(c, SPHIP_E_INVALID, "SPHIP_FLAG_CAMERA_SAMPLES is not available with kernel variant %d (%s)", variant, kVariantNames[variant]);
	if (!camf) cams = nullptr;
	if (mode == SPHIP_MODE_FLAT && (flags & SPHIP_FLAG_SPECULAR)) return fail(c, SPHIP_E_INVALID, "SPHIP_FLAG_SPECULAR is valid for SPHIP_MODE_PT only");
	const bool specf = mode == SPHIP_MODE_PT && (flags & SPHIP_FLAG_SPECULAR);
	if (specf && nee && !mis)
		return fail(c, SPHIP_E_INVALID, "SPHIP_FLAG_SPECULAR works with the plain estimator and with SPHIP_FLAG_NEE | SPHIP_FLAG_MIS, not with SPHIP_FLAG_NEE alone");
	if (specf && !variant_shipped(variant))
		return fail(c, SPHIP_E_INVALID, "SPHIP_FLAG_SPECULAR is not available with kernel variant %d (%s)", variant, kVariantNames[variant]);
	if (specf && !c->have_spec) return fail(c, SPHIP_E_STATE, "SPHIP_FLAG_SPECULAR needs a specular table (sphip_set_specular)");
	const sp::SpecArgs spa{ (const float4*)c->spec.p };
	HIP_TRY(c, hipMemsetAsync(c->counter.p, 0, 16 * sizeof(unsigned long long), st));
	uint32_t chunks = 1;
	TwoStage ts{1, false, 0};
	const bool is_ts = two_stage(variant, &ts);
	const uint32_t slots = is_ts && ts.split ? (uint32_t)ts.R : 1u;
	if (is_ts && ts.scan == 3 && (rc = ensure_cylm(c, st))) return rc;
	if (is_ts && ts.scan == 3 && c->cylm_wide) ts.scan = 4;
	const uint32_t bthreads = is_ts && ts.scan == 4 ? sp::cylm512::kMThreads : 256u;
	const uint32_t rays_per_block = is_ts && !ts.split ? bthreads * (uint32_t)ts.R : bthreads;
	const uint64_t chunk_target = kChunkTargetBlocks * 256u / bthreads;
	if (mode == SPHIP_MODE_PT && is_ts) {
		const uint64_t px_blocks = (n_rays + rays_per_block - 1) / rays_per_block;
		const uint64_t n_iter = (n_samples + slots - 1) / slots;
		const uint32_t forced = ((uint32_t)flags & SPHIP_FLAG_CHUNKS_MASK) >> SPHIP_FLAG_CHUNKS_SHIFT;
		if (forced) chunks = forced;
		else while (px_blocks * chunks < chunk_target && chunks < 128) chunks *= 2;
		if (chunks > n_iter) chunks = (uint32_t)n_iter;
		const uint64_t samp_bytes = (uint64_t)n_samples * 12 * ((n_rays + 255) / 256 * 256);
		if (chunks > 1 && !forced) {
			size_t free_b = 0, total_b = 0;
			bool asked = false;
			if (samp_bytes > kChunkMaxBytes) chunks = 1;
			const uint64_t lanes = (uint64_t)((n_rays + 1023) / 1024 * 1024) * slots;
			while (chunks > 1) {
				const uint64_t work_bytes = lanes * chunks * (work_slot_bytes(nee, mis) + (adapt ? kSlotAdaptWst : 0));
				const uint64_t need = (samp_bytes > c->samp.cap ? samp_bytes : 0) + (work_bytes > c->work.cap ? work_bytes : 0);
				if (need == 0) break;
				if (!asked) { asked = true; if (hipMemGetInfo(&free_b, &total_b) != hipSuccess) { chunks = 1; break; } }
				if (need <= (uint64_t)((double)free_b * 0.9)) break;
				chunks /= 2;
			}
		}
		if (chunks > 1) {
			a.n_chunks = chunks; a.px_blocks = (uint32_t)px_blocks; a.samp_stride = (uint32_t)((n_rays + 255) / 256 * 256);
			if ((rc = ensure(c, c->samp, (size_t)samp_bytes))) return rc;
			a.samp = (float*)c->samp.p;
		}
	}
	const dim3 block(256), block_ts(bthreads);
	const dim3 grid((unsigned)((n_rays + 255) / 256 * chunks));
	const uint32_t rpb1 = is_ts ? bthreads * (uint32_t)ts.R : 256u;
	const dim3 grid_px((unsigned)((n_rays + rpb1 - 1) / rpb1));
	const dim3 grid_pt((unsigned)((n_rays + rays_per_block - 1) / rays_per_block * chunks));
	const uint64_t n_work64 = (uint64_t)((n_rays + 1023) / 1024 * 1024) * slots * chunks;
	if (mode == SPHIP_MODE_PT && is_ts && n_work64 > 0xffffffffull)
		return fail(c, SPHIP_E_INVALID, "n_rays %zu too large for one launch of this kernel variant; shard the frame", n_rays);
	const uint32_t n_work = (uint32_t)n_work64;
	int2* hist = nullptr; float* acc = nullptr;
	sp::AdaptArgs ad{};
	if (adapt) ad = *adapt;
	if (mode == SPHIP_MODE_PT && is_ts) {
		if ((rc = ensure(c, c->work, (size_t)n_work * work_slot_bytes(nee, mis)))) return rc;
		hist = (int2*)c->work.p;
		acc = (float*)((char*)c->work.p + (size_t)n_work * kSlotHist);
		ne.L = (float*)((char*)c->work.p + (size_t)n_work * (kSlotHist + kSlotAcc));
		if (adapt && (rc = ensure(c, c->adp_wst, (size_t)n_work * kSlotAdaptWst))) return rc;
		ad.wst = (double*)c->adp_wst.p;
	}
	sp::ScanSrc src2{};
	if (is_ts && (ts.scan == 1 || ts.scan == 2) && (rc = ensure_cyl(c, st))) return rc;
#ifdef SP_ALL_VARIANTS
	if (is_ts && ts.scan == 0 && (rc = ensure_filt(c, st))) return rc;
#endif
	src2.filt = (const float4*)c->filt.p;
	src2.cyl.rec = (const float4*)c->cyl_rec.p;
	src2.cyl.hdr = (const uint32_t*)c->cyl_hdr.p;
	src2.cylm.rec = (const float4*)c->cylm_rec.p;
	src2.cylm.hdr = (const uint32_t*)c->cylm_hdr.p;
	src2.cylm.big = (const float4*)c->cylm_big.p;
	const unsigned int* bnd = (const unsigned int*)c->bounds.p;
	sp::BvhArgs B{};
	if (variant == kVariantAccel) {
		if ((rc = ensure_bvh(c, st))) return rc;
		B.nodes = (const float4*)c->bvh_nodes.p; B.leaf_rec = (const float4*)c->bvh_rec.p; B.leaf_idx = (const int*)c->bvh_idx.p;
		B.n_leaves = c->bvh_leaves; B.first_leaf = c->bvh_leaves; B.meta = (const uint32_t*)c->bvh_meta.p;
	}
	HIP_TRY(c, hipEventRecord(c->ev_k0, st));
	auto hit_filter = [&](const sp::KArgs& ka, const int* src_idx, int* oi, float* od) {
		with_scan_shape(ts, [&](auto shape) {
			using S = decltype(shape);
			hipLaunchKernelGGL((sp::k_hit_filter<S::R, S::SCAN>), grid_px, block_ts, 0, st, ka, src2, bnd, src_idx, oi, od);
		});
	};
	bool prim_pass = false;
	if (mode == SPHIP_MODE_PT && is_ts && (flags & SPHIP_FLAG_PRIMARY_REUSE)) {
		if ((rc = ensure(c, c->prim, n_rays * 8))) return rc;
		int* oi = (int*)c->prim.p; float* od = (float*)((char*)c->prim.p + n_rays * 4);
		sp::KArgs h = a;
		h.n_chunks = 0; h.samp = nullptr;
		hit_filter(h, nullptr, oi, od);
		a.prim_idx = oi; a.prim_d = od;
		prim_pass = true;
	}
	sp::MisArgs me{};
	if (mis) {
		static_cast<sp::NeeArgs&>(me) = ne;
		me.tipdf = (const float*)((const char*)c->nee_tab.p + (size_t)c->nee_n * 16);
	}
	const sp::AdaptArgs* adp = adapt ? &ad : nullptr;
	auto pt_pack = [&](auto&& f) { with_pack(prog, adp, nee ? &ne : nullptr, mis ? &me : nullptr, specf ? &spa : nullptr, cams, f); };
	auto accel = [&](auto mode_c, const int* src_idx, int* oi, float* od, const auto&... p) {
		hipLaunchKernelGGL((sp::k_accel<decltype(mode_c)::value, std::decay_t<decltype(p)>...>), grid, block, 0, st, a, B, src_idx, oi, od, p...);
	};
	auto with_exact = [&](auto&& f) {
		if (variant == 2) f(std::integral_constant<int, 2>{});
		else f(std::integral_constant<int, 1>{});
	};
	if (mode == kModeHits) {
		int* oi = (int*)d_rgba; float* od = (float*)d_accum;
		if (variant == kVariantAccel) accel(std::integral_constant<int, 2>{}, d_src, oi, od);
		else if (is_ts) hit_filter(a, d_src, oi, od);
		else with_exact([&](auto v) { hipLaunchKernelGGL((sp::k_hit<decltype(v)::value>), grid, block, 0, st, a, d_src, oi, od); });
	} else if (mode == SPHIP_MODE_FLAT) {
		if (variant == kVariantAccel) accel(std::integral_constant<int, 0>{}, nullptr, nullptr, nullptr);
		else if (is_ts) with_scan_shape(ts, [&](auto shape) {
			using S = decltype(shape);
			hipLaunchKernelGGL((sp::k_flat_filter<S::R, S::SCAN>), grid_px, block_ts, 0, st, a, src2, bnd);
		});
		else with_exact([&](auto v) { hipLaunchKernelGGL((sp::k_flat<decltype(v)::value>), grid, block, 0, st, a); });
	} else if (variant == kVariantAccel) {
		pt_pack([&](const auto&... p) { accel(std::integral_constant<int, 1>{}, nullptr, nullptr, nullptr, p...); });
	} else if (is_ts) {
		with_scan_shape(ts, [&](auto shape) {
			using S = decltype(shape);
			pt_pack([&](const auto&... p) {
				if constexpr (S::shipped || !(sp::IsNee<std::decay_t<decltype(p)>...>::value || sp::IsCam<std::decay_t<decltype(p)>...>::value ||
				                              sp::IsSpec<std::decay_t<decltype(p)>...>::value))
					hipLaunchKernelGGL((sp::k_pt_filter<S::R, S::SPLIT, S::SCAN, std::decay_t<decltype(p)>...>), grid_pt, block_ts, 0, st,
					                   a, src2, bnd, hist, acc, n_work, p...);
			});
		});
	} else {
		with_exact([&](auto v) {
			pt_pack([&](const auto&... p) { hipLaunchKernelGGL((sp::k_pt<decltype(v)::value, std::decay_t<decltype(p)>...>), grid, block, 0, st, a, p...); });
		});
	}
	if (chunks > 1)
		with_accum(prog, adp, [&](const auto&... q) {
			hipLaunchKernelGGL((sp::k_resolve<std::decay_t<decltype(q)>...>), dim3((unsigned)((n_rays + 255) / 256)), block, 0, st, a, q...);
		});
	HIP_TRY(c, hipGetLastError());
	HIP_TRY(c, hipEventRecord(c->ev_k1, st));
	c->have_render = true;
	c->last_stream = st;
	c->stats.n_tris = c->n_tris;
	c->stats.n_pixels = n_rays;
	c->stats.kernel_variant = (uint32_t)variant;
	c->stats.n_launches = (chunks > 1 ? 2u : 1u) + (prim_pass ? 1u : 0u);
	return SPHIP_OK;
}


sp::ViewArgs view_args(const sphip_camera* cam) {
	sp::ViewArgs v{};
	const float x_size = (float)(1.0 * (double)cam->res_x / (double)cam->res_y), y_size = 1.0f;
	v.x_max = (float)((double)x_size / 2.0);
	v.x_step = x_size / (float)cam->res_x;
	v.h_x_step = (float)((double)v.x_step / 2.0);
	v.y_max = (float)((double)y_size / 2.0);
	v.y_step = y_size / (float)cam->res_y;
	v.h_y_step = (float)((double)v.y_step / 2.0);
	v.focal = cam->focal; v.cos_y = cam->cos_y; v.sin_y = cam->sin_y; v.cos_x = cam->cos_x; v.sin_x = cam->sin_x;
	v.px = cam->pos[0]; v.py = cam->pos[1]; v.pz = cam->pos[2];
	v.res_x = cam->res_x; v.res_y = cam->res_y;
	v.n_local = cam->res_x * cam->res_y;
	v.pixel_base = 0; v.tile_px = v.n_local; v.tile_stride_px = 0;
	return v;
}

sp::CamArgs cam_args_of(const sphip_camera* cam, const sphip_lens& lens) {
	sp::CamArgs ca{};
	ca.v = view_args(cam);
	ca.aperture = lens.aperture;
	ca.focus_dist = lens.focus_dist;
	return ca;
}

int launch_viewport(sphip_ctx* c, const sphip_camera* cam, void* d_rays, hipStream_t st, const sphip_shard* shard = nullptr, size_t n_local = 0) {
	if (!cam || !d_rays) return fail(c, SPHIP_E_INVALID, "null camera or ray pointer");
	if (cam->res_x == 0 || cam->res_y == 0 || (uint64_t)cam->res_x * cam->res_y > 0xffffffffull)
		return fail(c, SPHIP_E_INVALID, "bad viewport size %ux%u", cam->res_x, cam->res_y);
	sp::ViewArgs v = view_args(cam);
	const uint32_t n = shard ? (uint32_t)n_local : cam->res_x * cam->res_y;
	v.n_local = n;
	if (shard) { v.pixel_base = shard->pixel_base; v.tile_px = shard->tile_px; v.tile_stride_px = shard->tile_stride_px; }
	else { v.pixel_base = 0; v.tile_px = n; v.tile_stride_px = 0; }
	if (n == 0) return SPHIP_OK;
	hipLaunchKernelGGL(sp::k_viewport, dim3((n + 255) / 256), dim3(256), 0, st, v, (float*)d_rays);
	HIP_TRY(c, hipGetLastError());
	return SPHIP_OK;
}



int plan_tile_rows(size_t height, int n_dev) {
	for (int tr = 8; tr >= 1; --tr)
		if (height % (size_t)tr == 0 && (height / (size_t)tr) % (size_t)n_dev == 0) return tr;
	return 8;
}

struct RowPlan {
	size_t w, h, tile_rows, tile_px, n_tiles, npix;
	int g;
	RowPlan(size_t w_, size_t h_, int g_, size_t tr) : w(w_), h(h_), tile_rows(tr), tile_px(tr * w_), n_tiles((h_ + tr - 1) / tr), npix(w_ * h_), g(g_) {}
	size_t n_rays(int rank) const {
		size_t n = 0;
		for (size_t t = (size_t)rank; t < n_tiles; t += (size_t)g) n += std::min(tile_px, npix - t * tile_px);
		return n;
	}
	size_t max_rays() const { size_t m = 0; for (int r = 0; r < g; ++r) m = std::max(m, n_rays(r)); return m; }
	sphip_shard shard(int rank) const { return sphip_shard{ (uint64_t)rank * tile_px, (uint64_t)tile_px, (uint64_t)g * tile_px }; }
};

typedef int (*nccl_init_all_t)(void**, int, const int*);
typedef int (*nccl_comm_destroy_t)(void*);
typedef int (*nccl_group_t)(void);
typedef int (*nccl_send_t)(const void*, size_t, int, int, void*, hipStream_t);
typedef int (*nccl_recv_t)(void*, size_t, int, int, void*, hipStream_t);
typedef const char* (*nccl_errstr_t)(int);
struct Rccl {
	nccl_init_all_t init_all = nullptr; nccl_comm_destroy_t destroy = nullptr; nccl_group_t group_start = nullptr, group_end = nullptr;
	nccl_send_t send = nullptr; nccl_recv_t recv = nullptr; nccl_errstr_t errstr = nullptr;
} g_rccl;
constexpr int kNcclUint8 = 1;

void* load_rccl() {
	static std::mutex mu;
	static void* loaded = nullptr;
	std::lock_guard<std::mutex> lock(mu);
	if (loaded) return loaded;
	const char* names[] = { "librccl.so.1", "librccl.so", "/opt/rocm/lib/librccl.so.1" };
	for (const char* n : names) {
		void* h = dlopen(n, RTLD_NOW | RTLD_LOCAL);
		if (!h) continue;
		g_rccl.init_all = (nccl_init_all_t)dlsym(h, "ncclCommInitAll");
		g_rccl.destroy = (nccl_comm_destroy_t)dlsym(h, "ncclCommDestroy");
		g_rccl.group_start = (nccl_group_t)dlsym(h, "ncclGroupStart");
		g_rccl.group_end = (nccl_group_t)dlsym(h, "ncclGroupEnd");
		g_rccl.send = (nccl_send_t)dlsym(h, "ncclSend");
		g_rccl.recv = (nccl_recv_t)dlsym(h, "ncclRecv");
		g_rccl.errstr = (nccl_errstr_t)dlsym(h, "ncclGetErrorString");
		if (g_rccl.init_all && g_rccl.destroy && g_rccl.group_start && g_rccl.group_end && g_rccl.send && g_rccl.recv) { loaded = h; return h; }
		g_rccl = Rccl{};
		dlclose(h);
	}
	return nullptr;
}

int multi_set_scene(sphip_ctx* c, const float* tris, const float* mats, size_t n_tris) {
	const int g = (int)c->kids.size();
	std::vector<int> rcs((size_t)g, SPHIP_OK);
	std::vector<std::thread> th;
	for (int r = 0; r < g; ++r) th.emplace_back([&, r] { rcs[(size_t)r] = sphip_set_scene(c->kids[(size_t)r], tris, mats, n_tris); });
	for (auto& t : th) t.join();
	for (int r = 0; r < g; ++r)
		if (rcs[(size_t)r]) return fail(c, rcs[(size_t)r], "device %d: %s", c->kids[(size_t)r]->device, c->kids[(size_t)r]->err.c_str());
	c->n_tris = n_tris;
	c->have_scene = true;
	c->have_spec = false;
	return SPHIP_OK;
}

int deal_rays(sphip_ctx* k, const RowPlan& plan, int r, const float* rays, const sphip_camera* cam, void* d_rays, hipStream_t st) {
	if (rays) {
		size_t k0 = 0;
		for (size_t t = (size_t)r; t < plan.n_tiles; t += (size_t)plan.g) {
			const size_t cnt = std::min(plan.tile_px, plan.npix - t * plan.tile_px);
			HIP_TRY(k, hipMemcpyAsync((char*)d_rays + k0 * 24, rays + t * plan.tile_px * 6, cnt * 24, hipMemcpyHostToDevice, st));
			k0 += cnt;
		}
		return SPHIP_OK;
	}
	const sphip_shard sh = plan.shard(r);
	return launch_viewport(k, cam, d_rays, st, &sh, plan.n_rays(r));
}

template <class RenderShard>
int multi_frame_impl(sphip_ctx* c, size_t w, size_t h, uint8_t* out_rgba, float* out_accum, const RenderShard& render_shard) {
	const int g = (int)c->kids.size();
	const RowPlan plan(w, h, g, (size_t)plan_tile_rows(h, g));
	const size_t pad = plan.max_rays(), npix = plan.npix;
	sphip_ctx* root = c->kids[0];
	HIP_TRY(c, hipSetDevice(root->device));
	int rc;
	if ((rc = ensure(c, c->gath, (size_t)g * pad * 4)) || (rc = ensure(c, c->img, npix * 4))) return rc;
	if (out_accum && ((rc = ensure(c, c->gath_acc, (size_t)g * pad * 12)) || (rc = ensure(c, c->img_acc, npix * 12)))) return rc;
	HIP_TRY(c, hipEventRecord(c->ev_g0, root->own_stream));
	const bool peer = c->gather_kind != SPHIP_GATHER_RCCL;
	std::vector<int> rcs((size_t)g, SPHIP_OK);
	std::vector<std::thread> th;
	for (int r = 0; r < g; ++r) th.emplace_back([&, r] {
		sphip_ctx* k = c->kids[(size_t)r];
		auto body = [&]() -> int {
			const size_t n = plan.n_rays(r);
			k->have_render = false;
			if (n == 0) return SPHIP_OK;
			HIP_TRY(k, hipSetDevice(k->device));
			hipStream_t st = k->own_stream;
			int rc2;
			if ((rc2 = ensure(k, k->rgba, pad * 4))) return rc2;
			if (out_accum && (rc2 = ensure(k, k->accum, pad * 12))) return rc2;
			if ((rc2 = render_shard(k, r, n, plan.shard(r)))) return rc2;
			k->timed_upload = k->timed_download = false;
			if (peer) {
				const bool same = k->device == root->device;
				if (same) HIP_TRY(k, hipMemcpyAsync((char*)c->gath.p + (size_t)r * pad * 4, k->rgba.p, n * 4, hipMemcpyDeviceToDevice, st));
				else HIP_TRY(k, hipMemcpyPeerAsync((char*)c->gath.p + (size_t)r * pad * 4, root->device, k->rgba.p, k->device, n * 4, st));
				if (out_accum && same) HIP_TRY(k, hipMemcpyAsync((char*)c->gath_acc.p + (size_t)r * pad * 12, k->accum.p, n * 12, hipMemcpyDeviceToDevice, st));
				else if (out_accum) HIP_TRY(k, hipMemcpyPeerAsync((char*)c->gath_acc.p + (size_t)r * pad * 12, root->device, k->accum.p, k->device, n * 12, st));
				HIP_TRY(k, hipEventRecord(c->ev_tile[(size_t)r], st));
			}
			return SPHIP_OK;
		};
		rcs[(size_t)r] = body();
	});
	for (auto& t : th) t.join();
	for (int r = 0; r < g; ++r)
		if (rcs[(size_t)r]) return fail(c, rcs[(size_t)r], "device %d: %s", c->kids[(size_t)r]->device, c->kids[(size_t)r]->err.c_str());
	HIP_TRY(c, hipSetDevice(root->device));
	hipStream_t rs = root->own_stream;
	auto gather_peer_now = [&]() -> int {
		for (int r = 0; r < g; ++r) {
			const size_t n = plan.n_rays(r);
			if (!n) continue;
			sphip_ctx* k = c->kids[(size_t)r];
			HIP_TRY(c, hipSetDevice(k->device));
			const bool same = k->device == root->device;
			if (same) HIP_TRY(c, hipMemcpyAsync((char*)c->gath.p + (size_t)r * pad * 4, k->rgba.p, n * 4, hipMemcpyDeviceToDevice, k->own_stream));
			else HIP_TRY(c, hipMemcpyPeerAsync((char*)c->gath.p + (size_t)r * pad * 4, root->device, k->rgba.p, k->device, n * 4, k->own_stream));
			if (out_accum && same) HIP_TRY(c, hipMemcpyAsync((char*)c->gath_acc.p + (size_t)r * pad * 12, k->accum.p, n * 12, hipMemcpyDeviceToDevice, k->own_stream));
			else if (out_accum) HIP_TRY(c, hipMemcpyPeerAsync((char*)c->gath_acc.p + (size_t)r * pad * 12, root->device, k->accum.p, k->device, n * 12, k->own_stream));
			HIP_TRY(c, hipEventRecord(c->ev_tile[(size_t)r], k->own_stream));
		}
		HIP_TRY(c, hipSetDevice(root->device));
		return SPHIP_OK;
	};
	bool wait_tiles = peer;
	if (!peer) {
		if (plan.n_rays(0)) {
			HIP_TRY(c, hipMemcpyAsync(c->gath.p, root->rgba.p, plan.n_rays(0) * 4, hipMemcpyDeviceToDevice, rs));
			if (out_accum) HIP_TRY(c, hipMemcpyAsync(c->gath_acc.p, root->accum.p, plan.n_rays(0) * 12, hipMemcpyDeviceToDevice, rs));
		}
		int nrc = g_rccl.group_start();
		for (int r = 1; r < g && !nrc; ++r) {
			const size_t n = plan.n_rays(r);
			if (!n) continue;
			sphip_ctx* k = c->kids[(size_t)r];
			if (!nrc) nrc = g_rccl.send(k->rgba.p, n * 4, kNcclUint8, 0, c->comms[(size_t)r], k->own_stream);
			if (!nrc) nrc = g_rccl.recv((char*)c->gath.p + (size_t)r * pad * 4, n * 4, kNcclUint8, r, c->comms[0], rs);
			if (out_accum && !nrc) nrc = g_rccl.send(k->accum.p, n * 12, kNcclUint8, 0, c->comms[(size_t)r], k->own_stream);
			if (out_accum && !nrc) nrc = g_rccl.recv((char*)c->gath_acc.p + (size_t)r * pad * 12, n * 12, kNcclUint8, r, c->comms[0], rs);
		}
		const int erc = g_rccl.group_end();
		if (nrc || erc) {
			fprintf(stderr, "libspath_hip: RCCL gather failed (%s); falling back to peer copies\n", g_rccl.errstr ? g_rccl.errstr(nrc ? nrc : erc) : "?");
			c->gather_kind = SPHIP_GATHER_PEER;
			if ((rc = gather_peer_now())) return rc;
			wait_tiles = true;
		}
	}
	if (wait_tiles)
		for (int r = 1; r < g; ++r) if (plan.n_rays(r)) HIP_TRY(c, hipStreamWaitEvent(rs, c->ev_tile[(size_t)r], 0));
	const dim3 grid((unsigned)((npix + 255) / 256)), block(256);
	hipLaunchKernelGGL(sp::k_assemble<1>, grid, block, 0, rs, (const uint32_t*)c->gath.p, (uint32_t*)c->img.p, (uint32_t)npix, (uint32_t)plan.tile_px, (uint32_t)g, (uint32_t)pad);
	if (out_accum)
		hipLaunchKernelGGL(sp::k_assemble<3>, grid, block, 0, rs, (const uint32_t*)c->gath_acc.p, (uint32_t*)c->img_acc.p, (uint32_t)npix, (uint32_t)plan.tile_px, (uint32_t)g, (uint32_t)pad);
	HIP_TRY(c, hipGetLastError());
	HIP_TRY(c, hipEventRecord(c->ev_g1, rs));
	HIP_TRY(c, hipMemcpyAsync(out_rgba, c->img.p, npix * 4, hipMemcpyDeviceToHost, rs));
	if (out_accum) HIP_TRY(c, hipMemcpyAsync(out_accum, c->img_acc.p, npix * 12, hipMemcpyDeviceToHost, rs));
	HIP_TRY(c, hipStreamSynchronize(rs));
	for (int r = 1; r < g; ++r) {
// ... 257 lines not shown
int gbuffer_dev(sphip_ctx* c, const void* d_rays, size_t n, int flags, void* d_out, hipStream_t st) {
	if (!c->have_scene) return fail(c, SPHIP_E_STATE, "G-buffer requested before a scene was set");
	if (!d_rays || !d_out) return fail(c, SPHIP_E_INVALID, "null ray or G-buffer pointer");
	if (n == 0 || n > 0xffffffffull) return fail(c, SPHIP_E_INVALID, "n_rays %zu out of range", n);
	int rc;
	if ((rc = ensure_classes(c, st)) || (rc = ensure(c, c->dn_hit, n * 8))) return rc;
	int* idx = (int*)c->dn_hit.p;
	float* dist = (float*)((char*)c->dn_hit.p + n * 4);
	if ((rc = launch_render(c, d_rays, n, nullptr, 0, 1, 0, kModeHits, flags, idx, dist, st))) return rc;
	hipLaunchKernelGGL(sp::k_gbuffer, dim3((unsigned)((n + 255) / 256)), dim3(256), 0, st, (const float*)d_rays, (const int*)idx,
	                   (const float*)dist, (const float*)c->tris.p, (const float*)c->mats.p, (const int*)c->dn_cls.p, (uint32_t)n, (float4*)d_out);
	HIP_TRY(c, hipGetLastError());
	HIP_TRY(c, hipEventRecord(c->ev_k1, st));
	c->stats.n_launches += 1;
	return SPHIP_OK;
}

int atrous_run(sphip_ctx* c, const DevBuf& a, const DevBuf& b, const sphip_denoise* P, size_t w, size_t h, bool use_var, const void* gbuf,
               uint32_t* rgba, float* rgb, hipStream_t st, uint32_t* launches) {
	const char* kenv = std::getenv("SPATH_HIP_ATROUS");
	const bool lds = !(kenv && std::strcmp(kenv, "l2") == 0);
	for (uint32_t i = 0; i < P->iterations; ++i) {
		const bool last = i + 1 == P->iterations;
		sp::AtrousArgs A{};
		A.in = (const float4*)(i % 2 ? b.p : a.p);
		A.out = (float4*)(i % 2 ? a.p : b.p);
		A.gbuf = (const float4*)gbuf;
		A.w = (uint32_t)w; A.h = (uint32_t)h;
		A.s = 1 << i;
		A.zs = P->sigma_depth * (float)A.s;
		A.sl2 = P->sigma_lum * P->sigma_lum;
		A.normal_log2 = P->normal_log2;
		A.use_var = use_var ? 1u : 0u;
		A.rgba = last ? rgba : nullptr;
		A.rgb = last ? rgb : nullptr;
		if (lds) {
			const size_t su = (w + (size_t)A.s - 1) / (size_t)A.s, sv = (h + (size_t)A.s - 1) / (size_t)A.s;
			const dim3 grid((unsigned)((su + 15) / 16 * (size_t)A.s), (unsigned)((sv + 15) / 16 * (size_t)A.s));
			hipLaunchKernelGGL(sp::k_atrous_lds, grid, dim3(256), 0, st, A);
		} else {
			const dim3 grid((unsigned)((w + 15) / 16), (unsigned)((h + 15) / 16));
			hipLaunchKernelGGL(sp::k_atrous, grid, dim3(256), 0, st, A);
		}
	}
	HIP_TRY(c, hipGetLastError());
	*launches += P->iterations;
	return SPHIP_OK;
}

int dn_clock_start(sphip_ctx* c, hipStream_t st) {
	int rc;
	if ((rc = ensure(c, c->counter, 16 * sizeof(unsigned long long)))) return rc;
	HIP_TRY(c, hipMemsetAsync(c->counter.p, 0, 16 * sizeof(unsigned long long), st));
	HIP_TRY(c, hipEventRecord(c->ev_k0, st));
	c->stats.n_launches = 0;
	return SPHIP_OK;
}

int accum_denoise_dev(sphip_ctx* c, sphip_ctx* k, const sphip_denoise* P, const void* d_rays, bool have4, bool use_var, bool want_rgb,
                      hipStream_t st) {
	const size_t w = c->acc_w, h = c->acc_h, n = w * h;
	int rc;
	if ((rc = ensure(c, c->dn_gbuf, n * 32)) || (rc = ensure(c, c->dn_a, n * 16)) || (rc = ensure(c, c->dn_b, n * 16)) ||
	    (rc = ensure(k, k->rgba, n * 4)) || (want_rgb && (rc = ensure(k, k->accum, n * 12)))) return rc;
	const bool build = !c->dn_gbuf_ok;
	if (build) {
		if ((rc = gbuffer_dev(k, d_rays, n, c->acc_flags, c->dn_gbuf.p, st))) return rc;
	} else if ((rc = dn_clock_start(k, st))) return rc;
	uint32_t* rgba = (uint32_t*)k->rgba.p;
	float* rgb = want_rgb ? (float*)k->accum.p : nullptr;
	const bool k0 = P->iterations == 0;
	if (!have4) {
		hipLaunchKernelGGL(sp::k_dn_prep, dim3((unsigned)((n + 255) / 256)), dim3(256), 0, st, (const float*)c->acc_sum.p,
		                   c->adp_on ? (const uint32_t*)c->adp_cnt.p : nullptr, (uint32_t)c->acc_total, c->adp_on ? (const double*)c->adp_s12.p : nullptr,
		                   (uint32_t)n, (float4*)c->dn_a.p, k0 ? rgba : nullptr, k0 ? rgb : nullptr);
		k->stats.n_launches += 1;
	} else if (k0) {
		hipLaunchKernelGGL(sp::k_dn_emit4, dim3((unsigned)((n + 255) / 256)), dim3(256), 0, st, (const float4*)c->dn_a.p, (uint32_t)n, rgba, rgb);
		k->stats.n_launches += 1;
	}
	HIP_TRY(k, hipGetLastError());
	if ((rc = atrous_run(k, c->dn_a, c->dn_b, P, w, h, use_var, c->dn_gbuf.p, rgba, rgb, st, &k->stats.n_launches))) return rc;
	HIP_TRY(k, hipEventRecord(k->ev_k1, st));
	if (build) c->dn_gbuf_ok = true;
	k->have_render = true;
	k->last_stream = st;
	k->stats.n_pixels = n;
	k->stats.n_tris = k->n_tris;
	k->stats.kernel_variant = (uint32_t)pick_variant(c->acc_flags, k->n_tris);
	return SPHIP_OK;
}

int multi_accum_denoise(sphip_ctx* c, const sphip_denoise* P, uint8_t* out_rgba, float* out_rgb) {
	const int g = (int)c->kids.size();
	const RowPlan plan(c->acc_w, c->acc_h, g, (size_t)plan_tile_rows(c->acc_h, g));
	const size_t npix = plan.npix;
	const bool need_rays = !c->dn_gbuf_ok;
	sphip_ctx* root = c->kids[0];
	auto body = [&]() -> int {
		std::vector<float4> img4(npix), loc;
		std::vector<float> rays(need_rays ? npix * 6 : 0), lrays;
		int rc;
		for (int r = 0; r < g; ++r) {
			sphip_ctx* k = c->kids[(size_t)r];
			k->have_render = false;
			const size_t n = plan.n_rays(r);
			if (n == 0) continue;
			HIP_TRY(c, hipSetDevice(k->device));
			hipStream_t st = k->own_stream;
			if ((rc = ensure(k, k->dn_a, n * 16))) return fail(c, rc, "device %d: %s", k->device, k->err.c_str());
			hipLaunchKernelGGL(sp::k_dn_prep, dim3((unsigned)((n + 255) / 256)), dim3(256), 0, st, (const float*)k->acc_sum.p,
			                   c->adp_on ? (const uint32_t*)k->adp_cnt.p : nullptr, (uint32_t)c->acc_total, c->adp_on ? (const double*)k->adp_s12.p : nullptr,
			                   (uint32_t)n, (float4*)k->dn_a.p, (uint32_t*)nullptr, (float*)nullptr);
			HIP_TRY(c, hipGetLastError());
			loc.resize(n);
			HIP_TRY(c, hipMemcpyAsync(loc.data(), k->dn_a.p, n * 16, hipMemcpyDeviceToHost, st));
			if (need_rays) { lrays.resize(n * 6); HIP_TRY(c, hipMemcpyAsync(lrays.data(), k->acc_rays.p, n * 24, hipMemcpyDeviceToHost, st)); }
			HIP_TRY(c, hipStreamSynchronize(st));
			const sphip_shard sh = plan.shard(r);
			for (size_t i = 0; i < n; ++i) {
				const size_t p = sh.pixel_base + (i / sh.tile_px) * sh.tile_stride_px + i % sh.tile_px;
				img4[p] = loc[i];
				if (need_rays) std::memcpy(&rays[p * 6], &lrays[i * 6], 24);
			}
		}
		HIP_TRY(c, hipSetDevice(root->device));
		hipStream_t rs = root->own_stream;
		if ((rc = ensure(c, c->dn_a, npix * 16)) || (need_rays && (rc = ensure(c, c->dn_rays, npix * 24)))) return rc;
		HIP_TRY(c, hipEventRecord(c->ev_g0, rs));
		HIP_TRY(c, hipMemcpyAsync(c->dn_a.p, img4.data(), npix * 16, hipMemcpyHostToDevice, rs));
		if (need_rays) HIP_TRY(c, hipMemcpyAsync(c->dn_rays.p, rays.data(), npix * 24, hipMemcpyHostToDevice, rs));
		if ((rc = accum_denoise_dev(c, root, P, c->dn_rays.p, true, c->adp_on, out_rgb != nullptr, rs)))
			return fail(c, rc, "device %d: %s", root->device, root->err.c_str());
		HIP_TRY(c, hipEventRecord(c->ev_g1, rs));
		HIP_TRY(c, hipMemcpyAsync(out_rgba, root->rgba.p, npix * 4, hipMemcpyDeviceToHost, rs));
		if (out_rgb) HIP_TRY(c, hipMemcpyAsync(out_rgb, root->accum.p, npix * 12, hipMemcpyDeviceToHost, rs));
		HIP_TRY(c, hipStreamSynchronize(rs));
		root->timed_upload = root->timed_download = false;
		c->have_render = true;
		c->stats.n_pixels = npix;
		c->stats.n_tris = c->n_tris;
		return SPHIP_OK;
	};
	const int rc = body();
	if (rc) {
		for (sphip_ctx* k : c->kids)
			if (hipSetDevice(k->device) == hipSuccess && k->own_stream) (void)hipStreamSynchronize(k->own_stream);
		(void)hipGetLastError();
	}
	return rc;
}

}

extern "C" {

int sphip_abi_version(void) { return SPHIP_ABI_VERSION; }

const char* sphip_kernel_name(int variant) {
	if (variant < 0 || variant > kVariantLast) return nullptr;
	return kVariantNames[variant];
}

#ifndef SP_SOURCE_HASH
#define SP_SOURCE_HASH "unknown"
#endif
const char* sphip_build_info(void) { return "src=" SP_SOURCE_HASH; }

int sphip_kernel_available(int variant) { return variant_built(variant) ? 1 : 0; }

int sphip_plan_tile_rows(size_t height, int n_devices) {
	if (height == 0 || n_devices < 1) return SPHIP_E_INVALID;
	return plan_tile_rows(height, n_devices);
}

int sphip_plan_shard(size_t width, size_t height, int n_devices, size_t tile_rows, int rank, sphip_shard* shard_out, size_t* n_rays_out) {
	if (width == 0 || height == 0 || n_devices < 1 || tile_rows == 0 || rank < 0 || rank >= n_devices) return SPHIP_E_INVALID;
	const RowPlan plan(width, height, n_devices, tile_rows);
	if (shard_out) *shard_out = plan.shard(rank);
	if (n_rays_out) *n_rays_out = plan.n_rays(rank);
	return SPHIP_OK;
}

int sphip_device_count(const sphip_t* c) { return c ? (c->kids.empty() ? 1 : (int)c->kids.size()) : 0; }

int sphip_create_multi(const int* device_ids, int n_devices, sphip_t** out) {
	if (!out) return fail(nullptr, SPHIP_E_INVALID, "out is NULL");
	*out = nullptr;
	std::vector<int> ids;
	if (device_ids) {
		if (n_devices < 1 || n_devices > 64) return fail(nullptr, SPHIP_E_INVALID, "n_devices %d out of range [1,64]", n_devices);
		ids.assign(device_ids, device_ids + n_devices);
	} else if (const char* env = getenv("SPATH_HIP_DEVICES")) {
		for (const char* p = env; *p;) {
			char* end = nullptr;
			const long v = strtol(p, &end, 10);
			if (end == p) return fail(nullptr, SPHIP_E_INVALID, "SPATH_HIP_DEVICES=\"%s\" is not a comma-separated list of device numbers", env);
			ids.push_back((int)v);
			p = (*end == ',') ? end + 1 : end;
			if (*end && *end != ',') return fail(nullptr, SPHIP_E_INVALID, "SPATH_HIP_DEVICES=\"%s\" is not a comma-separated list of device numbers", env);
		}
		if (ids.empty() || ids.size() > 64) return fail(nullptr, SPHIP_E_INVALID, "SPATH_HIP_DEVICES lists %zu devices", ids.size());
	} else {
		int n = 0;
		const hipError_t e = hipGetDeviceCount(&n);
		if (e != hipSuccess || n <= 0)
			return fail(nullptr, SPHIP_E_DEVICE, "no HIP device available (%s)", e != hipSuccess ? hipGetErrorString(e) : "device count 0");
		for (int i = 0; i < n; ++i) ids.push_back(i);
	}
	const char* want = getenv("SPATH_HIP_GATHER");
	if (ids.size() == 1 && !(want && !strcmp(want, "rccl"))) return sphip_create(ids[0], out);
	sphip_ctx* c = new (std::nothrow) sphip_ctx();
	if (!c) return fail(nullptr, SPHIP_E_DEVICE, "out of host memory");
	bool distinct = true;
	for (size_t i = 0; i < ids.size(); ++i) for (size_t j = 0; j < i; ++j) distinct &= ids[i] != ids[j];
	for (int id : ids) {
		sphip_ctx* k = nullptr;
		if (sphip_create(id, &k) != SPHIP_OK) { sphip_destroy(c); return SPHIP_E_DEVICE; }
		c->kids.push_back(k);
	}
	sphip_ctx* root = c->kids[0];
	c->device = root->device;
	hipError_t e = hipSetDevice(root->device);
	if (e == hipSuccess) e = hipEventCreate(&c->ev_g0);
	if (e == hipSuccess) e = hipEventCreate(&c->ev_g1);
	for (size_t r = 0; r < c->kids.size() && e == hipSuccess; ++r) {
		hipEvent_t ev = nullptr;
		if ((e = hipSetDevice(c->kids[r]->device)) == hipSuccess && (e = hipEventCreateWithFlags(&ev, hipEventDisableTiming)) == hipSuccess) c->ev_tile.push_back(ev);
		if (e == hipSuccess && c->kids[r]->device != root->device) (void)hipDeviceEnablePeerAccess(root->device, 0);
		(void)hipGetLastError();
	}
	if (e != hipSuccess) { fail(nullptr, SPHIP_E_DEVICE, "multi-device init failed: %s", hipGetErrorString(e)); sphip_destroy(c); return SPHIP_E_DEVICE; }
	c->gather_kind = SPHIP_GATHER_PEER;
	if (distinct && !(want && !strcmp(want, "peer"))) {
		c->rccl_lib = load_rccl();
		if (c->rccl_lib) {
			c->comms.assign(ids.size(), nullptr);
			const int nrc = g_rccl.init_all(c->comms.data(), (int)ids.size(), ids.data());
			if (nrc == 0) c->gather_kind = SPHIP_GATHER_RCCL;
			else { c->comms.clear(); if (want && !strcmp(want, "rccl")) { fail(nullptr, SPHIP_E_DEVICE, "ncclCommInitAll failed: %s", g_rccl.errstr ? g_rccl.errstr(nrc) : "?"); sphip_destroy(c); return SPHIP_E_DEVICE; } }
		} else if (want && !strcmp(want, "rccl")) { fail(nullptr, SPHIP_E_DEVICE, "SPATH_HIP_GATHER=rccl but librccl could not be loaded: %s", dlerror()); sphip_destroy(c); return SPHIP_E_DEVICE; }
	} else if (want && !strcmp(want, "rccl") && !distinct) {
		fail(nullptr, SPHIP_E_INVALID, "SPATH_HIP_GATHER=rccl needs distinct devices (a communicator holds a GPU once)"); sphip_destroy(c); return SPHIP_E_INVALID;
	}
	char d[320];
	snprintf(d, sizeof d, "HIP - Path Tracing (%zu devices, first: %s; pixel-row tiles, %s gather)", ids.size(),
	         root->desc.c_str() + (root->desc.rfind("(") == std::string::npos ? 0 : root->desc.rfind("(") + 1), c->gather_kind == SPHIP_GATHER_RCCL ? "RCCL" : "peer-copy");
	c->desc = d;
	*out = c;
	return SPHIP_OK;
}

int sphip_create(int device_id, sphip_t** out) {
	if (!out) return fail(nullptr, SPHIP_E_INVALID, "out is NULL");
	*out = nullptr;
	int n = 0;
	hipError_t e = hipGetDeviceCount(&n);
	if (e != hipSuccess || n <= 0)
		return fail(nullptr, SPHIP_E_DEVICE, "no HIP device available (%s)", e != hipSuccess ? hipGetErrorString(e) : "device count 0");
	if (device_id < 0 || device_id >= n) return fail(nullptr, SPHIP_E_INVALID, "device %d out of range [0,%d)", device_id, n);
	sphip_ctx* c = new (std::nothrow) sphip_ctx();
	if (!c) return fail(nullptr, SPHIP_E_DEVICE, "out of host memory");
	c->device = device_id;
	hipDeviceProp_t prop;
	if ((e = hipSetDevice(device_id)) != hipSuccess || (e = hipGetDeviceProperties(&prop, device_id)) != hipSuccess ||
	    (e = hipStreamCreateWithFlags(&c->own_stream, hipStreamNonBlocking)) != hipSuccess) {
		fail(nullptr, SPHIP_E_DEVICE, "device %d init failed: %s", device_id, hipGetErrorString(e));
		delete c;
		return SPHIP_E_DEVICE;
	}
	hipEvent_t* evs[6] = { &c->ev_k0, &c->ev_k1, &c->ev_u0, &c->ev_u1, &c->ev_d0, &c->ev_d1 };
	for (auto ev : evs) {
		if ((e = hipEventCreate(ev)) != hipSuccess) {
			fail(nullptr, SPHIP_E_DEVICE, "hipEventCreate failed: %s", hipGetErrorString(e));
			sphip_destroy(c);
			return SPHIP_E_DEVICE;
		}
	}
	char d[256];
	snprintf(d, sizeof d, "HIP - Path Tracing (%s, %s, %d CUs)", prop.name, prop.gcnArchName, prop.multiProcessorCount);
	c->desc = d;
	*out = c;
	return SPHIP_OK;
}

void sphip_destroy(sphip_t* c) {
	if (!c) return;
	if (!c->kids.empty()) {
		for (void* comm : c->comms) if (comm) (void)g_rccl.destroy(comm);
		(void)hipSetDevice(c->kids[0]->device);
		(void)hipDeviceSynchronize();
		DevBuf* mb[9] = { &c->gath, &c->gath_acc, &c->img, &c->img_acc, &c->dn_hit, &c->dn_gbuf, &c->dn_a, &c->dn_b, &c->dn_rays };
		for (auto b : mb) if (b->p) (void)hipFree(b->p);
		if (c->ev_g0) (void)hipEventDestroy(c->ev_g0);
		if (c->ev_g1) (void)hipEventDestroy(c->ev_g1);
		for (size_t r = 0; r < c->ev_tile.size(); ++r) { (void)hipSetDevice(c->kids[r]->device); (void)hipEventDestroy(c->ev_tile[r]); }
		for (sphip_ctx* k : c->kids) sphip_destroy(k);
		delete c;
		return;
	}
	(void)hipSetDevice(c->device);
	if (c->own_stream) (void)hipStreamSynchronize(c->own_stream);
	DevBuf* bufs[] = { &c->tris, &c->mats, &c->scan, &c->filt, &c->bounds, &c->samp, &c->rays, &c->rgba, &c->accum, &c->counter, &c->work,
	                   &c->bvh_nodes, &c->bvh_rec, &c->bvh_idx, &c->sort_kv, &c->sort_hist, &c->bvh_meta, &c->cyl_rec, &c->cyl_cnt, &c->cyl_hdr, &c->prim, &c->cylm_rec, &c->cylm_hdr, &c->cylm_big,
	                   &c->acc_rays, &c->acc_sum, &c->adp_s12, &c->adp_cnt, &c->adp_list[0], &c->adp_list[1], &c->adp_rays, &c->adp_keep,
	                   &c->adp_blk, &c->adp_nact_d, &c->adp_wst, &c->dn_cls, &c->dn_hit, &c->dn_gbuf, &c->dn_a, &c->dn_b, &c->dn_rays, &c->nee_tab, &c->spec };
	for (auto b : bufs) if (b->p) (void)hipFree(b->p);
	hipEvent_t evs[6] = { c->ev_k0, c->ev_k1, c->ev_u0, c->ev_u1, c->ev_d0, c->ev_d1 };
	for (auto ev : evs) if (ev) (void)hipEventDestroy(ev);
	if (c->own_stream) (void)hipStreamDestroy(c->own_stream);
	delete c;
}

const char* sphip_last_error(const sphip_t* c) { return c ? c->err.c_str() : g_create_error.c_str(); }

const char* sphip_description(const sphip_t* c) { return c ? c->desc.c_str() : "HIP - Path Tracing"; }

int sphip_set_scene(sphip_t* c, const float* tris, const float* mats, size_t n_tris) {
	if (!c) return SPHIP_E_INVALID;
	if (!tris || !mats || n_tris == 0 || n_tris > 0x7fffffffull) return fail(c, SPHIP_E_INVALID, "bad scene arguments (n_tris=%zu)", n_tris);
	c->acc_stale = c->acc_on;
	c->dn_cls_valid = false;
	if (!c->kids.empty()) return multi_set_scene(c, tris, mats, n_tris);
	HIP_TRY(c, hipSetDevice(c->device));
	int rc;
	if ((rc = ensure(c, c->tris, n_tris * 48)) || (rc = ensure(c, c->mats, n_tris * 24))) return rc;
	c->n_tris = n_tris;
	HIP_TRY(c, hipMemcpyAsync(c->tris.p, tris, n_tris * 48, hipMemcpyHostToDevice, c->own_stream));
	HIP_TRY(c, hipMemcpyAsync(c->mats.p, mats, n_tris * 24, hipMemcpyHostToDevice, c->own_stream));
	if ((rc = repack(c, c->own_stream))) return rc;
	HIP_TRY(c, hipStreamSynchronize(c->own_stream));
	return SPHIP_OK;
}

int sphip_set_scene_device(sphip_t* c, const void* d_tris, const void* d_mats, size_t n_tris, void* stream) {
	if (!c) return SPHIP_E_INVALID;
	if (!c->kids.empty()) return fail(c, SPHIP_E_STATE, "device-pointer entry points need a single-device context (sphip_create)");
	if (!d_tris || !d_mats || n_tris == 0 || n_tris > 0x7fffffffull) return fail(c, SPHIP_E_INVALID, "bad scene arguments (n_tris=%zu)", n_tris);
	c->acc_stale = c->acc_on;
	c->dn_cls_valid = false;
	HIP_TRY(c, hipSetDevice(c->device));
	hipStream_t st = (hipStream_t)stream;
	int rc;
	if ((rc = ensure(c, c->tris, n_tris * 48)) || (rc = ensure(c, c->mats, n_tris * 24))) return rc;
	c->n_tris = n_tris;
	HIP_TRY(c, hipMemcpyAsync(c->tris.p, d_tris, n_tris * 48, hipMemcpyDeviceToDevice, st));
	HIP_TRY(c, hipMemcpyAsync(c->mats.p, d_mats, n_tris * 24, hipMemcpyDeviceToDevice, st));
	return repack(c, st);
}

static size_t spec_first_bad(const float* spec, size_t n_tris) {
	for (size_t i = 0; i < n_tris; ++i) {
		const float* q = spec + i * 4;
		for (int k = 0; k < 4; ++k) if (!std::isfinite(q[k]) || !(q[k] >= 0.0f)) return i;
		if (!(q[3] <= 1.0f)) return i;
	}
	return n_tris;
}

int sphip_set_specular(sphip_t* c, const float* spec) {
	if (!c) return SPHIP_E_INVALID;
	if (!c->have_scene) return fail(c, SPHIP_E_STATE, "sphip_set_specular called before a scene was set");
	if (spec) {
		if (c->n_tris >= (size_t)sp::kSpecBit) return fail(c, SPHIP_E_INVALID, "a specular table needs a scene of fewer than 2^30 triangles (this one has %zu)", c->n_tris);
		const size_t bad = spec_first_bad(spec, c->n_tris);
		if (bad < c->n_tris) {
			const float* q = spec + bad * 4;
			return fail(c, SPHIP_E_INVALID, "specular table: triangle %zu has {ks %g %g %g, p %g} (every value finite, ks >= 0, 0 <= p <= 1)", bad,
			            (double)q[0], (double)q[1], (double)q[2], (double)q[3]);
		}
	}
	c->acc_stale = c->acc_on;
	if (!c->kids.empty()) {
		c->have_spec = false;
		for (sphip_ctx* k : c->kids)
			if (const int rc = sphip_set_specular(k, spec)) {
				for (sphip_ctx* q : c->kids) q->have_spec = false;
				return fail(c, rc, "device %d: %s", k->device, k->err.c_str());
			}
		c->have_spec = spec != nullptr;
		return SPHIP_OK;
	}
	c->have_spec = false;
	if (!spec) return SPHIP_OK;
	HIP_TRY(c, hipSetDevice(c->device));
	int rc;
	if ((rc = ensure(c, c->spec, c->n_tris * 16))) return rc;
	HIP_TRY(c, hipMemcpyAsync(c->spec.p, spec, c->n_tris * 16, hipMemcpyHostToDevice, c->own_stream));
	HIP_TRY(c, hipStreamSynchronize(c->own_stream));
	c->have_spec = true;
	return SPHIP_OK;
}

int sphip_set_specular_device(sphip_t* c, const void* d_spec, void* stream) {
	if (!c) return SPHIP_E_INVALID;
	if (!c->kids.empty()) return fail(c, SPHIP_E_STATE, "device-pointer entry points need a single-device context (sphip_create)");
	if (!c->have_scene) return fail(c, SPHIP_E_STATE, "sphip_set_specular_device called before a scene was set");
	c->acc_stale = c->acc_on;
	c->have_spec = false;
	if (!d_spec) return SPHIP_OK;
	if (c->n_tris >= (size_t)sp::kSpecBit) return fail(c, SPHIP_E_INVALID, "a specular table needs a scene of fewer than 2^30 triangles (this one has %zu)", c->n_tris);
	HIP_TRY(c, hipSetDevice(c->device));
	int rc;
	if ((rc = ensure(c, c->spec, c->n_tris * 16))) return rc;
	HIP_TRY(c, hipMemcpyAsync(c->spec.p, d_spec, c->n_tris * 16, hipMemcpyDeviceToDevice, (hipStream_t)stream));
	c->have_spec = true;
	return SPHIP_OK;
}

int sphip_render_device(sphip_t* c, const void* d_rays, size_t n_rays, const sphip_shard* shard, size_t image_width,
                        size_t n_samples, uint64_t seed, int mode, int flags, void* d_out_rgba, void* d_out_accum, void* stream) {
	if (!c) return SPHIP_E_INVALID;
	if (!c->kids.empty()) return fail(c, SPHIP_E_STATE, "device-pointer entry points need a single-device context (sphip_create)");
	HIP_TRY(c, hipSetDevice(c->device));
	c->timed_upload = c->timed_download = false;
	return launch_render(c, d_rays, n_rays, shard, image_width, n_samples, seed, mode, flags, d_out_rgba, d_out_accum, (hipStream_t)stream);
}

int sphip_render_device_accum(sphip_t* c, const void* d_rays, size_t n_rays, const sphip_shard* shard, size_t image_width,
                              uint64_t sample_base, size_t n_samples, uint64_t seed, int flags, void* d_sum,
                              void* d_out_rgba, void* d_out_mean, void* stream) {
	if (!c) return SPHIP_E_INVALID;
	if (!c->kids.empty()) return fail(c, SPHIP_E_STATE, "device-pointer entry points need a single-device context (sphip_create)");
	if (!d_sum) return fail(c, SPHIP_E_INVALID, "null sum pointer");
	if (sample_base > 0x7fffffffull) return fail(c, SPHIP_E_INVALID, "sample_base %llu: the total must stay below 2^31", (unsigned long long)sample_base);
	HIP_TRY(c, hipSetDevice(c->device));
	c->timed_upload = c->timed_download = false;
	const sp::AccumArgs p{ (float*)d_sum, (uint32_t)sample_base };
	return launch_render(c, d_rays, n_rays, shard, image_width, n_samples, seed, SPHIP_MODE_PT, flags, d_out_rgba, d_out_mean, (hipStream_t)stream,
	                     nullptr, &p);
}


int sphip_accum_begin(sphip_t* c, const float* rays, const sphip_camera* cam, size_t w, size_t h, uint64_t seed, int flags) {
	if (!c) return SPHIP_E_INVALID;
	return accum_begin(c, rays, cam, w, h, seed, flags, nullptr);
}

int sphip_accum_begin_adaptive(sphip_t* c, const float* rays, const sphip_camera* cam, size_t w, size_t h, uint64_t seed, int flags,
                               const sphip_adaptive* a) {
	if (!c) return SPHIP_E_INVALID;
	if (!a) return fail(c, SPHIP_E_INVALID, "null sphip_adaptive");
	if (!std::isfinite(a->rel_error) || a->rel_error < 0.0 || !std::isfinite(a->floor) || a->floor < 0.0 || a->min_samples < 2 || a->reserved != 0)
		return fail(c, SPHIP_E_INVALID, "bad sphip_adaptive {rel_error %g, floor %g, min_samples %u, reserved %u}: t and floor finite and >= 0, "
		            "min_samples >= 2, reserved 0", a->rel_error, a->floor, a->min_samples, a->reserved);
	return accum_begin(c, rays, cam, w, h, seed, flags, a);
}

int sphip_accum_counts(sphip_t* c, uint32_t* out_counts, uint64_t* n_active_out) {
	if (!c) return SPHIP_E_INVALID;
	if (!c->acc_on) return fail(c, SPHIP_E_STATE, "sphip_accum_counts called with no accumulation begun");
	const size_t npix = c->acc_w * c->acc_h;
	if (n_active_out) *n_active_out = c->adp_on ? c->adp_nact : npix;
	if (!out_counts) return SPHIP_OK;
	if (!c->adp_on) {
		std::fill(out_counts, out_counts + npix, (uint32_t)c->acc_total);
		return SPHIP_OK;
	}
	if (c->kids.empty()) {
		HIP_TRY(c, hipSetDevice(c->device));
		HIP_TRY(c, hipMemcpyAsync(out_counts, c->adp_cnt.p, npix * 4, hipMemcpyDeviceToHost, c->own_stream));
		HIP_TRY(c, hipStreamSynchronize(c->own_stream));
		return SPHIP_OK;
	}
	const int g = (int)c->kids.size();
	const RowPlan plan(c->acc_w, c->acc_h, g, (size_t)plan_tile_rows(c->acc_h, g));
	std::vector<uint32_t> loc;
	for (int r = 0; r < g; ++r) {
		sphip_ctx* k = c->kids[(size_t)r];
		const size_t n = plan.n_rays(r);
		if (n == 0) continue;
		loc.resize(n);
		HIP_TRY(c, hipSetDevice(k->device));
		HIP_TRY(c, hipMemcpyAsync(loc.data(), k->adp_cnt.p, n * 4, hipMemcpyDeviceToHost, k->own_stream));
		HIP_TRY(c, hipStreamSynchronize(k->own_stream));
		const sphip_shard sh = plan.shard(r);
		for (size_t i = 0; i < n; ++i) out_counts[sh.pixel_base + (i / sh.tile_px) * sh.tile_stride_px + i % sh.tile_px] = loc[i];
	}
	return SPHIP_OK;
}

int sphip_accum_step(sphip_t* c, size_t n_samples, uint8_t* out_rgba, float* out_mean, uint64_t* total_out) {
	if (!c) return SPHIP_E_INVALID;
	if (!c->acc_on) return fail(c, SPHIP_E_STATE, "sphip_accum_step called with no accumulation begun (sphip_accum_begin)");
	if (c->acc_stale) return fail(c, SPHIP_E_STATE, "the scene changed since sphip_accum_begin: begin a new accumulation");
	if (!out_rgba) return fail(c, SPHIP_E_INVALID, "null output pointer");
	if (n_samples == 0 || c->acc_total + n_samples > 0x7fffffffull)
		return fail(c, SPHIP_E_INVALID, "n_samples = %zu after %llu: each step renders at least one sample, and the total must stay below 2^31",
		            n_samples, (unsigned long long)c->acc_total);
	const bool traced = !c->adp_on || c->adp_nact > 0;
	int rc;
	if (!c->kids.empty()) {
		rc = multi_accum_step(c, n_samples, out_rgba, out_mean);
	} else {
		auto body = [&]() -> int {
			HIP_TRY(c, hipSetDevice(c->device));
			const size_t n = c->acc_w * c->acc_h;
			hipStream_t st = c->own_stream;
			int rc2;
			if ((rc2 = ensure(c, c->rgba, n * 4))) return rc2;
			if (out_mean && (rc2 = ensure(c, c->accum, n * 12))) return rc2;
			const sp::AccumArgs p{ (float*)c->acc_sum.p, (uint32_t)c->acc_total };
			const sphip_shard whole{ 0, n, 0 };
			if (c->adp_on) {
				if ((rc2 = adapt_step_dev(c, c, n, whole, n_samples, out_mean ? (float*)c->accum.p : nullptr, st))) return rc2;
			} else {
				const sp::CamArgs ca = cam_args_of(&c->acc_cam, c->acc_lens);
				if ((rc2 = launch_render(c, c->acc_rays.p, n, nullptr, c->acc_w, n_samples, c->acc_seed, SPHIP_MODE_PT, c->acc_flags, c->rgba.p,
				                         out_mean ? c->accum.p : nullptr, st, nullptr, &p, nullptr, c->acc_has_cam ? &ca : nullptr))) return rc2;
			}
			HIP_TRY(c, hipEventRecord(c->ev_d0, st));
			HIP_TRY(c, hipMemcpyAsync(out_rgba, c->rgba.p, n * 4, hipMemcpyDeviceToHost, st));
			if (out_mean) HIP_TRY(c, hipMemcpyAsync(out_mean, c->accum.p, n * 12, hipMemcpyDeviceToHost, st));
			HIP_TRY(c, hipEventRecord(c->ev_d1, st));
			HIP_TRY(c, hipStreamSynchronize(st));
			c->adp_nact = c->adp_nact_rb;
			c->timed_upload = false;
			c->timed_download = true;
			return SPHIP_OK;
		};
		rc = body();
		if (rc) { (void)hipStreamSynchronize(c->own_stream); (void)hipGetLastError(); }
	}
	if (rc) {
		c->acc_on = false;
		return rc;
	}
	if (traced) c->acc_total += n_samples;
	if (total_out) *total_out = c->acc_total;
	return SPHIP_OK;
}

int sphip_viewport_device(sphip_t* c, const sphip_camera* cam, void* d_rays_out, void* stream) {
	if (!c) return SPHIP_E_INVALID;
	if (!c->kids.empty()) return fail(c, SPHIP_E_STATE, "device-pointer entry points need a single-device context (sphip_create)");
	HIP_TRY(c, hipSetDevice(c->device));
	return launch_viewport(c, cam, d_rays_out, (hipStream_t)stream);
}

int sphip_set_lens(sphip_t* c, const sphip_lens* lens) {
	if (!c) return SPHIP_E_INVALID;
	const sphip_lens l = lens ? *lens : sphip_lens{ 0.0f, 0.0f, 0 };
	if (!std::isfinite(l.aperture) || l.aperture < 0.0f || (l.aperture > 0.0f && !(std::isfinite(l.focus_dist) && l.focus_dist > 0.0f)) || l.reserved != 0)
		return fail(c, SPHIP_E_INVALID, "bad sphip_lens {aperture %g, focus_dist %g, reserved %u}: aperture finite and >= 0, focus_dist finite and > 0 "
		            "when aperture > 0, reserved 0", (double)l.aperture, (double)l.focus_dist, l.reserved);
	c->lens = l;
	return SPHIP_OK;
}

int sphip_camera_rays_device(sphip_t* c, const sphip_camera* cam, uint64_t seed, uint32_t sample, void* d_rays_out, void* stream) {
	if (!c) return SPHIP_E_INVALID;
	if (!c->kids.empty()) return fail(c, SPHIP_E_STATE, "device-pointer entry points need a single-device context (sphip_create)");
	if (!cam || !d_rays_out) return fail(c, SPHIP_E_INVALID, "null camera or ray pointer");
	if (cam->res_x == 0 || cam->res_y == 0 || (uint64_t)cam->res_x * cam->res_y > 0xffffffffull)
		return fail(c, SPHIP_E_INVALID, "bad viewport size %ux%u", cam->res_x, cam->res_y);
	HIP_TRY(c, hipSetDevice(c->device));
	const sp::CamArgs ca = cam_args_of(cam, c->lens);
	hipLaunchKernelGGL(sp::k_camera_rays, dim3((ca.v.n_local + 255) / 256), dim3(256), 0, (hipStream_t)stream, ca, seed, sample, (float*)d_rays_out);
	HIP_TRY(c, hipGetLastError());
	return SPHIP_OK;
}

int sphip_render_camera(sphip_t* c, const sphip_camera* cam, size_t n_samples, uint64_t seed, int mode, int flags,
                        uint8_t* out_rgba, float* out_accum) {
	if (!c) return SPHIP_E_INVALID;
	if (!cam || !out_rgba) return fail(c, SPHIP_E_INVALID, "null camera or output pointer");
	if (!c->kids.empty()) return multi_render(c, nullptr, cam, cam->res_x, cam->res_y, n_samples, seed, mode, flags, out_rgba, out_accum);
	HIP_TRY(c, hipSetDevice(c->device));
	const size_t n = (size_t)cam->res_x * cam->res_y;
	hipStream_t st = c->own_stream;
	int rc;
	if ((rc = ensure(c, c->rays, (n ? n : 1) * 24)) || (rc = ensure(c, c->rgba, (n ? n : 1) * 4))) return rc;
	if (out_accum && (rc = ensure(c, c->accum, n * 12))) return rc;
	if ((rc = launch_viewport(c, cam, c->rays.p, st))) return rc;
	const sp::CamArgs ca = cam_args_of(cam, c->lens);
	if ((rc = launch_render(c, c->rays.p, n, nullptr, cam->res_x, n_samples, seed, mode, flags, c->rgba.p, out_accum ? c->accum.p : nullptr, st,
	                        nullptr, nullptr, nullptr, &ca))) return rc;
	HIP_TRY(c, hipEventRecord(c->ev_d0, st));
	HIP_TRY(c, hipMemcpyAsync(out_rgba, c->rgba.p, n * 4, hipMemcpyDeviceToHost, st));
	if (out_accum) HIP_TRY(c, hipMemcpyAsync(out_accum, c->accum.p, n * 12, hipMemcpyDeviceToHost, st));
	HIP_TRY(c, hipEventRecord(c->ev_d1, st));
	HIP_TRY(c, hipStreamSynchronize(st));
	c->timed_upload = false;
	c->timed_download = true;
	return SPHIP_OK;
}

int sphip_closest_hit_device(sphip_t* c, const void* d_rays, size_t n_rays, const void* d_src_idx, int flags,
                             void* d_out_idx, void* d_out_dist, void* stream) {
	if (!c) return SPHIP_E_INVALID;
	if (!c->kids.empty()) return fail(c, SPHIP_E_STATE, "device-pointer entry points need a single-device context (sphip_create)");
	HIP_TRY(c, hipSetDevice(c->device));
	c->timed_upload = c->timed_download = false;
	return launch_render(c, d_rays, n_rays, nullptr, 0, 1, 0, kModeHits, flags, d_out_idx, d_out_dist, (hipStream_t)stream, (const int*)d_src_idx);
}

int sphip_render(sphip_t* c, const float* rays, size_t w, size_t h, size_t n_samples, uint64_t seed, int mode, int flags,
                 uint8_t* out_rgba, float* out_accum) {
	if (!c) return SPHIP_E_INVALID;
	if (!rays || !out_rgba || w == 0 || h == 0) return fail(c, SPHIP_E_INVALID, "bad render arguments (w=%zu h=%zu)", w, h);
	if (!c->kids.empty()) return multi_render(c, rays, nullptr, w, h, n_samples, seed, mode, flags, out_rgba, out_accum);
	HIP_TRY(c, hipSetDevice(c->device));
	const size_t n = w * h;
	hipStream_t st = c->own_stream;
	int rc;
	if ((rc = ensure(c, c->rays, n * 24)) || (rc = ensure(c, c->rgba, n * 4))) return rc;
	if (out_accum && (rc = ensure(c, c->accum, n * 12))) return rc;
	HIP_TRY(c, hipEventRecord(c->ev_u0, st));
	HIP_TRY(c, hipMemcpyAsync(c->rays.p, rays, n * 24, hipMemcpyHostToDevice, st));
	HIP_TRY(c, hipEventRecord(c->ev_u1, st));
	if ((rc = launch_render(c, c->rays.p, n, nullptr, w, n_samples, seed, mode, flags, c->rgba.p, out_accum ? c->accum.p : nullptr, st))) return rc;
	HIP_TRY(c, hipEventRecord(c->ev_d0, st));
	HIP_TRY(c, hipMemcpyAsync(out_rgba, c->rgba.p, n * 4, hipMemcpyDeviceToHost, st));
	if (out_accum) HIP_TRY(c, hipMemcpyAsync(out_accum, c->accum.p, n * 12, hipMemcpyDeviceToHost, st));
	HIP_TRY(c, hipEventRecord(c->ev_d1, st));
	HIP_TRY(c, hipStreamSynchronize(st));
	c->timed_upload = c->timed_download = true;
	return SPHIP_OK;
}

int sphip_selftest_device(sphip_t* c, int what, const void* in, size_t n, void* out) {
	if (!c) return SPHIP_E_INVALID;
	static const size_t in_b[7] = { 4, 4, 20, 40, 60, 12, 48 }, out_b[7] = { 8, 4, 16, 12, 4, 4, 8 };
	if (what < 0 || what > 6 || !in || !out || n == 0 || n > 0x7fffffffull) return fail(c, SPHIP_E_INVALID, "bad selftest arguments (what=%d n=%zu)", what, n);
	sphip_ctx* k = c->kids.empty() ? c : c->kids[0];
	HIP_TRY(c, hipSetDevice(k->device));
	void *d_in = nullptr, *d_out = nullptr;
	HIP_TRY(c, hipMalloc(&d_in, n * in_b[what]));
	hipError_t e = hipMalloc(&d_out, n * out_b[what]);
	if (e == hipSuccess) e = hipMemcpy(d_in, in, n * in_b[what], hipMemcpyHostToDevice);
	if (e == hipSuccess) {
		if (what == 6) hipLaunchKernelGGL(sp::cylm256::k_selftest_cylm, dim3((unsigned)n), dim3(64), 0, k->own_stream, (const float*)d_in, (uint32_t)n, (float*)d_out);
		else hipLaunchKernelGGL(sp::k_selftest, dim3((unsigned)((n + 255) / 256)), dim3(256), 0, k->own_stream, what, (const void*)d_in, (uint32_t)n, d_out);
		e = hipGetLastError();
	}
	if (e == hipSuccess) e = hipStreamSynchronize(k->own_stream);
	if (e == hipSuccess) e = hipMemcpy(out, d_out, n * out_b[what], hipMemcpyDeviceToHost);
	(void)hipFree(d_in);
	if (d_out) (void)hipFree(d_out);
	if (e != hipSuccess) return fail(c, SPHIP_E_DEVICE, "selftest failed: %s", hipGetErrorString(e));
	return SPHIP_OK;
}

int sphip_selftest_stage1(sphip_t* c, const float* rays, size_t n_rays, uint32_t* out_words, uint32_t* out_tri, int32_t* out_order, uint32_t* tiles_out) {
	if (!c) return SPHIP_E_INVALID;
	if (!c->kids.empty()) return fail(c, SPHIP_E_STATE, "sphip_selftest_stage1 needs a single-device context (sphip_create)");
	if (!c->have_scene) return fail(c, SPHIP_E_STATE, "sphip_selftest_stage1 called before a scene was set");
	if (!tiles_out) return fail(c, SPHIP_E_INVALID, "tiles_out is NULL");
	HIP_TRY(c, hipSetDevice(c->device));
	hipStream_t st = c->own_stream;
	int rc = ensure_cylm(c, st);
	if (rc) return rc;
	uint32_t hdr[8];
	HIP_TRY(c, hipMemcpyAsync(hdr, c->cylm_hdr.p, sizeof hdr, hipMemcpyDeviceToHost, st));
	HIP_TRY(c, hipStreamSynchronize(st));
	const uint32_t tiles = hdr[6];
	const uint32_t T = c->cylm_wide ? sp::cylm512::kMTile : sp::cylm256::kMTile, W = c->cylm_wide ? sp::cylm512::kMWords : sp::cylm256::kMWords;
	const uint32_t grp8 = (c->cylm_wide ? sp::cylm512::kMGrp : sp::cylm256::kMGrp) == 8u ? 1u : 0u;
	*tiles_out = tiles | (T << 20) | (grp8 << 31);
	if (!out_words) return SPHIP_OK;
	if (!rays || !out_order || n_rays == 0 || n_rays % 64 || n_rays > 0x7fffffffull) return fail(c, SPHIP_E_INVALID, "bad stage-1 selftest arguments (n_rays=%zu)", n_rays);
	const size_t words_b = n_rays * tiles * 2 * W * sizeof(uint32_t), tri_b = n_rays * tiles * 2 * (T / 64) * sizeof(uint32_t),
	             order_b = (size_t)tiles * T * sizeof(int32_t);
	void *d_rays = nullptr, *d_words = nullptr, *d_order = nullptr, *d_tri = nullptr;
	hipError_t e = hipMalloc(&d_rays, n_rays * 24);
	if (e == hipSuccess) e = hipMalloc(&d_words, words_b);
	if (e == hipSuccess && out_tri) e = hipMalloc(&d_tri, tri_b);
	if (e == hipSuccess) e = hipMalloc(&d_order, order_b);
	if (e == hipSuccess) e = hipMemcpyAsync(d_rays, rays, n_rays * 24, hipMemcpyHostToDevice, st);
	if (e == hipSuccess) {
		sp::CylStream cs{ (const float4*)c->cylm_rec.p, (const uint32_t*)c->cylm_hdr.p, (const float4*)c->cylm_big.p };
		if (c->cylm_wide)
			hipLaunchKernelGGL(sp::cylm512::k_selftest_stage1, dim3((unsigned)(n_rays / 64)), dim3(64), 0, st, (const float*)d_rays, (uint32_t)n_rays, cs,
		                   (const unsigned int*)c->bounds.p, (uint32_t*)d_words, (uint32_t*)d_tri, (int*)d_order);
		else
			hipLaunchKernelGGL(sp::cylm256::k_selftest_stage1, dim3((unsigned)(n_rays / 64)), dim3(64), 0, st, (const float*)d_rays, (uint32_t)n_rays, cs,
		                   (const unsigned int*)c->bounds.p, (uint32_t*)d_words, (uint32_t*)d_tri, (int*)d_order);
		e = hipGetLastError();
	}
	if (e == hipSuccess) e = hipMemcpyAsync(out_words, d_words, words_b, hipMemcpyDeviceToHost, st);
	if (e == hipSuccess) e = hipMemcpyAsync(out_order, d_order, order_b, hipMemcpyDeviceToHost, st);
	if (e == hipSuccess && out_tri) e = hipMemcpyAsync(out_tri, d_tri, tri_b, hipMemcpyDeviceToHost, st);
	if (e == hipSuccess) e = hipStreamSynchronize(st);
	if (d_rays) (void)hipFree(d_rays);
	if (d_words) (void)hipFree(d_words);
	if (d_order) (void)hipFree(d_order);
	if (d_tri) (void)hipFree(d_tri);
	if (e != hipSuccess) return fail(c, SPHIP_E_DEVICE, "stage-1 selftest failed: %s", hipGetErrorString(e));
	return SPHIP_OK;
}

void sphip_denoise_defaults(sphip_denoise* out) {
	if (!out) return;
	std::memset(out, 0, sizeof *out);
	out->iterations = 5;
	out->normal_log2 = 7;
	out->sigma_depth = 0.1f;
	out->sigma_lum = 4.0f;
}

int sphip_gbuffer_device(sphip_t* c, const void* d_rays, size_t n_rays, int flags, void* d_out_gbuf, void* stream) {
	if (!c) return SPHIP_E_INVALID;
	if (!c->kids.empty()) return fail(c, SPHIP_E_STATE, "device-pointer entry points need a single-device context (sphip_create)");
	HIP_TRY(c, hipSetDevice(c->device));
	c->timed_upload = c->timed_download = false;
	return gbuffer_dev(c, d_rays, n_rays, flags, d_out_gbuf, (hipStream_t)stream);
}

int sphip_denoise_device(sphip_t* c, const sphip_denoise* P, size_t w, size_t h, const void* d_mean, const void* d_var, const void* d_gbuf,
                         void* d_out_rgba, void* d_out_rgb, void* stream) {
	if (!c) return SPHIP_E_INVALID;
	int rc;
	if ((rc = check_denoise(c, P))) return rc;
	if (!c->kids.empty()) return fail(c, SPHIP_E_STATE, "device-pointer entry points need a single-device context (sphip_create)");
	if (!d_mean || !d_gbuf || !d_out_rgba) return fail(c, SPHIP_E_INVALID, "null mean, G-buffer or output pointer");
	if (w == 0 || h == 0 || w >= (1u << 30) || h >= (1u << 30) || w * h > 0xffffffffull) return fail(c, SPHIP_E_INVALID, "bad image size (w=%zu h=%zu)", w, h);
	HIP_TRY(c, hipSetDevice(c->device));
	hipStream_t st = (hipStream_t)stream;
	const size_t n = w * h;
	if ((rc = ensure(c, c->dn_a, n * 16)) || (rc = ensure(c, c->dn_b, n * 16)) || (rc = dn_clock_start(c, st))) return rc;
	const bool k0 = P->iterations == 0;
	hipLaunchKernelGGL(sp::k_dn_pack, dim3((unsigned)((n + 255) / 256)), dim3(256), 0, st, (const float*)d_mean, (const float*)d_var, (uint32_t)n,
	                   k0 ? (float4*)nullptr : (float4*)c->dn_a.p, k0 ? (uint32_t*)d_out_rgba : nullptr, k0 ? (float*)d_out_rgb : nullptr);
	HIP_TRY(c, hipGetLastError());
	c->stats.n_launches = 1;
	if ((rc = atrous_run(c, c->dn_a, c->dn_b, P, w, h, d_var != nullptr, d_gbuf, (uint32_t*)d_out_rgba, (float*)d_out_rgb, st, &c->stats.n_launches))) return rc;
	HIP_TRY(c, hipEventRecord(c->ev_k1, st));
	c->timed_upload = c->timed_download = false;
	c->have_render = true;
	c->last_stream = st;
	c->stats.n_pixels = n;
	c->stats.n_tris = c->n_tris;
	return SPHIP_OK;
}

int sphip_accum_gbuffer(sphip_t* c, void* out_gbuf) {
	if (!c) return SPHIP_E_INVALID;
	if (!out_gbuf) return fail(c, SPHIP_E_INVALID, "null G-buffer output");
	if (!c->acc_on) return fail(c, SPHIP_E_STATE, "sphip_accum_gbuffer called with no accumulation begun");
	if (c->acc_stale) return fail(c, SPHIP_E_STATE, "the scene changed since sphip_accum_begin: begin a new accumulation");
	const size_t n = c->acc_w * c->acc_h;
	if (!c->kids.empty()) {
		const int g = (int)c->kids.size();
		const RowPlan plan(c->acc_w, c->acc_h, g, (size_t)plan_tile_rows(c->acc_h, g));
		std::vector<float> rays(n * 6), lrays;
		for (int r = 0; r < g; ++r) {
			sphip_ctx* k = c->kids[(size_t)r];
			const size_t nr = plan.n_rays(r);
			if (nr == 0) continue;
			HIP_TRY(c, hipSetDevice(k->device));
			lrays.resize(nr * 6);
			HIP_TRY(c, hipMemcpyAsync(lrays.data(), k->acc_rays.p, nr * 24, hipMemcpyDeviceToHost, k->own_stream));
			HIP_TRY(c, hipStreamSynchronize(k->own_stream));
			const sphip_shard sh = plan.shard(r);
			for (size_t i = 0; i < nr; ++i) std::memcpy(&rays[(sh.pixel_base + (i / sh.tile_px) * sh.tile_stride_px + i % sh.tile_px) * 6], &lrays[i * 6], 24);
		}
		sphip_ctx* root = c->kids[0];
		HIP_TRY(c, hipSetDevice(root->device));
		int rc;
		if ((rc = ensure(c, c->dn_rays, n * 24)) || (rc = ensure(c, c->dn_gbuf, n * 32))) return rc;
		HIP_TRY(c, hipMemcpyAsync(c->dn_rays.p, rays.data(), n * 24, hipMemcpyHostToDevice, root->own_stream));
		if (!c->dn_gbuf_ok && (rc = gbuffer_dev(root, c->dn_rays.p, n, c->acc_flags, c->dn_gbuf.p, root->own_stream))) {
			(void)hipStreamSynchronize(root->own_stream);
			return fail(c, rc, "device %d: %s", root->device, root->err.c_str());
		}
		c->dn_gbuf_ok = true;
		HIP_TRY(c, hipMemcpyAsync(out_gbuf, c->dn_gbuf.p, n * 32, hipMemcpyDeviceToHost, root->own_stream));
		HIP_TRY(c, hipStreamSynchronize(root->own_stream));
		return SPHIP_OK;
	}
	HIP_TRY(c, hipSetDevice(c->device));
	hipStream_t st = c->own_stream;
	int rc;
	if ((rc = ensure(c, c->dn_gbuf, n * 32))) return rc;
	if (!c->dn_gbuf_ok && (rc = gbuffer_dev(c, c->acc_rays.p, n, c->acc_flags, c->dn_gbuf.p, st))) { (void)hipStreamSynchronize(st); return rc; }
	c->dn_gbuf_ok = true;
	HIP_TRY(c, hipMemcpyAsync(out_gbuf, c->dn_gbuf.p, n * 32, hipMemcpyDeviceToHost, st));
	HIP_TRY(c, hipStreamSynchronize(st));
	return SPHIP_OK;
}

int sphip_accum_denoise(sphip_t* c, const sphip_denoise* P, uint8_t* out_rgba, float* out_rgb) {
	if (!c) return SPHIP_E_INVALID;
	int rc;
	if ((rc = check_denoise(c, P))) return rc;
	if (!out_rgba) return fail(c, SPHIP_E_INVALID, "null output pointer");
	if (!c->acc_on || c->acc_total == 0) return fail(c, SPHIP_E_STATE, "sphip_accum_denoise needs an accumulation with at least one step");
	if (c->acc_stale) return fail(c, SPHIP_E_STATE, "the scene changed since sphip_accum_begin: begin a new accumulation");
	if (c->acc_w >= (1u << 30) || c->acc_h >= (1u << 30)) return fail(c, SPHIP_E_INVALID, "image too wide or tall for the filter");
	if (!c->kids.empty()) return multi_accum_denoise(c, P, out_rgba, out_rgb);
	HIP_TRY(c, hipSetDevice(c->device));
	hipStream_t st = c->own_stream;
	const size_t n = c->acc_w * c->acc_h;
	rc = accum_denoise_dev(c, c, P, c->acc_rays.p, false, c->adp_on, out_rgb != nullptr, st);
	if (!rc) {
		if (hipMemcpyAsync(out_rgba, c->rgba.p, n * 4, hipMemcpyDeviceToHost, st) != hipSuccess ||
		    (out_rgb && hipMemcpyAsync(out_rgb, c->accum.p, n * 12, hipMemcpyDeviceToHost, st) != hipSuccess) ||
		    hipStreamSynchronize(st) != hipSuccess) rc = fail(c, SPHIP_E_DEVICE, "denoise readback failed: %s", hipGetErrorString(hipGetLastError()));
	}
	if (rc) { (void)hipStreamSynchronize(st); (void)hipGetLastError(); return rc; }
	c->timed_upload = c->timed_download = false;
	return SPHIP_OK;
}

int sphip_get_stats(sphip_t* c, sphip_stats* out) {
	if (!c || !out) return SPHIP_E_INVALID;
	if (!c->kids.empty()) return multi_get_stats(c, out);
	if (!c->have_render) return fail(c, SPHIP_E_STATE, "no render has been issued yet");
	HIP_TRY(c, hipSetDevice(c->device));
	HIP_TRY(c, hipEventSynchronize(c->ev_k1));
	float ms = 0.0f;
	HIP_TRY(c, hipEventElapsedTime(&ms, c->ev_k0, c->ev_k1));
	c->stats.kernel_ms = ms;
	c->stats.upload_ms = c->stats.download_ms = 0.0;
	if (c->timed_upload) { HIP_TRY(c, hipEventElapsedTime(&ms, c->ev_u0, c->ev_u1)); c->stats.upload_ms = ms; }
	if (c->timed_download) { HIP_TRY(c, hipEventSynchronize(c->ev_d1)); HIP_TRY(c, hipEventElapsedTime(&ms, c->ev_d0, c->ev_d1)); c->stats.download_ms = ms; }
	unsigned long long scans = 0;
	HIP_TRY(c, hipMemcpyAsync(&scans, c->counter.p, sizeof scans, hipMemcpyDeviceToHost, c->last_stream));
	HIP_TRY(c, hipStreamSynchronize(c->last_stream));
	c->stats.scans_executed = scans;
#ifdef SP_BVH_STATS
	{
		unsigned long long x[3] = {0, 0, 0};
		(void)hipMemcpy(x, c->counter.p, sizeof x, hipMemcpyDeviceToHost);
		fprintf(stderr, "[bvh stats] scans=%llu steps/scan=%.1f leaves/scan=%.1f\n", x[0], (double)x[1] / (double)(x[0] ? x[0] : 1), (double)x[2] / (double)(x[0] ? x[0] : 1));
	}
#endif
#ifdef SP_PHASE_TIMERS
	{
		unsigned long long x[16] = {};
		(void)hipMemcpy(x, c->counter.p, sizeof x, hipMemcpyDeviceToHost);
		const double tot = (double)(x[8] + x[9] + x[10] + x[11] + x[12]);
		fprintf(stderr, "[phase timers] wave-scans %llu; wave lifetime inside the scan by phase: stage 1 %.1f %%, list building + DMA issue %.1f %%, re-test rounds %.1f %%, exact turns %.1f %%, tile barrier %.1f %% (%.0f cycles per wave-scan)\n",
		        x[13], 100.0 * x[8] / tot, 100.0 * x[9] / tot, 100.0 * x[10] / tot, 100.0 * x[11] / tot, 100.0 * x[12] / tot, tot / (double)(x[13] ? x[13] : 1));
	}
#endif
#ifdef SP_FILTER_STATS
	{
		unsigned long long x[6] = {0, 0, 0, 0, 0, 0};
		(void)hipMemcpy(x, c->counter.p, sizeof x, hipMemcpyDeviceToHost);
		if (c->stats.kernel_variant >= 9)
			fprintf(stderr, "[cyl stats] group bits set=%llu stage-2 rounds(per wave)=%llu wave-tiles=%llu exact tests=%llu -> bits/lane/tile=%.3f rounds/tile=%.2f exact per bit=%.3f lane utilisation in stage 2=%.3f wave-wide exact turns=%llu (%.2f per round, %.3f of their lanes used)\n",
			        x[1], x[2], x[3], x[4], (double)x[1] / (64.0 * (double)x[3]), (double)x[2] / (double)x[3], (double)x[4] / (double)x[1], (double)x[4] / (64.0 * (double)x[2]),
			        x[5], (double)x[5] / (double)x[2], (double)x[4] / (64.0 * (double)x[5]));
		else
		fprintf(stderr, "[filter stats] survivors=%llu rounds(sum of per-wave max)=%llu wave_flushes=%llu overflows=%llu -> survivors/lane/flush=%.3f rounds/flush=%.2f\n",
		        x[1], x[2], x[3], x[4], (double)x[1] / (64.0 * (double)x[3]), (double)x[2] / (double)x[3]);
	}
#endif
	c->stats.n_devices = 1; c->stats.gather_kind = SPHIP_GATHER_NONE; c->stats.gather_ms = 0.0; c->stats.kernel_ms_min = c->stats.kernel_ms;
	*out = c->stats;
	return SPHIP_OK;
}

}
```

Baseline: 1367.

## Split exact group records to global memory and stream two filter tiles per stage

Moves the full-precision per-group triangle records out of the LDS tile into a separate global array with a group-contiguous 7-quad layout. LDS then holds only the f16 matrix fragments plus the Hmax/kappa table, which lets two tiles be DMA'd and filtered per pipeline stage. Stage-2 exact tests now read candidate groups from global/cache instead of LDS, and the candidate list cap shrinks to fit the doubled staging buffers. The intent is to halve per-tile loop, DMA and barrier overhead and to shrink LDS traffic, at the cost of global-memory latency in the exact-test phase and more register pressure from the doubled word arrays.

Result: slower. 1314 (-3.8%).

```diff
diff --git a/spath_amd/csrc/sp_cyl_scan.h b/spath_amd/csrc/sp_cyl_scan.h
--- a/spath_amd/csrc/sp_cyl_scan.h
+++ b/spath_amd/csrc/sp_cyl_scan.h
@@ -18,6 +18,7 @@
 	const float4* rec;
 	const uint32_t* hdr;
 	const float4* big;
+	const float4* grp;
 };
 
 SP_DEV void cyl_store(float4* __restrict__ tile, uint32_t grp, uint32_t u, const float4 q0, const float4 q1) {
diff --git a/spath_amd/csrc/sp_cylm_scan.h b/spath_amd/csrc/sp_cylm_scan.h
--- a/spath_amd/csrc/sp_cylm_scan.h
+++ b/spath_amd/csrc/sp_cylm_scan.h
@@ -24,16 +24,17 @@
 constexpr uint32_t kMBitsFrag = 16u / kMGrp;
 constexpr uint32_t kMFragsPerWord = 32u / kMBitsFrag;
 constexpr uint32_t kMWords = (kMBlocks * kMBitsFrag + 31u) / 32u;
-constexpr uint32_t kMRecQ = kMGroups * 8u;
-constexpr uint32_t kMTileQ = kMRecQ + kMBlocks * 64u;
+constexpr uint32_t kMFragQ = kMBlocks * 64u;
+constexpr uint32_t kMTileQ = kMFragQ + kMBlocks * 2u + 1u;
+constexpr uint32_t kMStage = 2u;
+constexpr uint32_t kMStageQ = kMStage * kMTileQ;
+constexpr uint32_t kMGrpQ = 7u;
 static_assert(kMThreads % 64u == 0u && kMThreads <= 1024u, "whole waves");
-static_assert(kMTileQ % kMThreads == 0u, "whole workgroup LDS-DMA passes");
-static_assert(kMGroups <= 128u, "7-bit group index in a list entry");
-static_assert(kMBlocks * 2u <= kMGroups, "the Hmax table fits chunk 7");
-SP_DEV constexpr uint32_t cylm_slot(uint32_t group, uint32_t chunk) { return chunk * kMGroups + group; }
-SP_DEV constexpr uint32_t cylm_hmq(uint32_t tb, uint32_t hh) { return 7u * kMGroups + tb * 2u + hh; }
-SP_DEV constexpr uint32_t cylm_kq() { return 7u * kMGroups + kMBlocks * 2u; }
-static_assert(kMBlocks * 2u + 1u <= kMGroups, "Hmax table and kappa fit chunk 7");
+static_assert(kMStage * kMGroups <= 256u, "8-bit group index (within the stage) in a list entry");
+static_assert(kMGrp == 8u || kMStage * kMGroups <= 128u, "quads: 7 bits");
+SP_DEV constexpr uint32_t cylm_hmq(uint32_t tb, uint32_t hh) { return kMFragQ + tb * 2u + hh; }
+SP_DEV constexpr uint32_t cylm_kq() { return kMFragQ + kMBlocks * 2u; }
+SP_DEV constexpr uint32_t cylm_gpos(uint32_t g) { return kMGrp == 8u ? ((g & ~3u) | ((g & 1u) << 1) | ((g >> 1) & 1u)) : g; }
 
 SP_DEV float cylm_scale(float rv) {
 	if (!(rv > 1e-30f && rv < 1e30f)) return 0.0f;
@@ -54,19 +55,20 @@
 	lo = to_half(v - (float)hi);
 }
 
-SP_DEV void cylm_store(float4* __restrict__ tile, uint32_t in_tile, const float4 q0, const float4 q1, float S) {
+SP_DEV void cylm_store(float4* __restrict__ tile, float4* __restrict__ grec, uint32_t in_tile, const float4 q0, const float4 q1, float S) {
 	const uint32_t grp = in_tile >> 2, u = in_tile & 3u;
-	tile[cylm_slot(grp, u)] = q0;
-	float* mh = (float*)(tile + cylm_slot(grp, 4u + (u >> 1))) + 2u * (u & 1u);
+	float4* const G = grec + cylm_gpos(grp) * kMGrpQ;
+	G[u] = q0;
+	float* mh = (float*)(G + 4u + (u >> 1)) + 2u * (u & 1u);
 	mh[0] = q1.x; mh[1] = q1.y;
-	((float*)(tile + cylm_slot(grp, 6u)))[u] = q1.z;
+	((float*)(G + 6u))[u] = q1.z;
 	const float m = S > 0.0f ? 16.0f / S : 0.0f;
 	_Float16 bh, bl, ch, cl, xh, xl, yh, yl, zh, zl;
 	half_split(S > 0.0f ? 16.0f * q0.x : 0.0f, bh, bl); half_split(S > 0.0f ? 16.0f * q0.y : 0.0f, ch, cl);
 	half_split(q0.z * m, xh, xl); half_split(q0.w * m, yh, yl); half_split(q1.x * m, zh, zl);
 	const _Float16 z = (_Float16)0.0f;
 	const half8 k0 = { bh, bl, bh, ch, cl, ch, xh, xl }, k1 = { xh, yh, yl, yh, zh, zl, zh, S > 0.0f ? (_Float16)16.0f : z };
-	half8* frag = (half8*)(tile + kMRecQ) + (in_tile >> 5) * 64u + (in_tile & 31u);
+	half8* frag = (half8*)tile + (in_tile >> 5) * 64u + (in_tile & 31u);
 	frag[0] = k0; frag[32] = k1;
 }
 
@@ -129,7 +131,7 @@
 }
 
 __global__ void __launch_bounds__(256) k_cylm_scatter(const float* __restrict__ tris, uint32_t n, const uint32_t* __restrict__ sorted,
-                                                     const uint32_t* __restrict__ hdr, float4* __restrict__ rec, const float4* __restrict__ scan, float4* __restrict__ big) {
+                                                     const uint32_t* __restrict__ hdr, float4* __restrict__ rec, float4* __restrict__ grec, const float4* __restrict__ scan, float4* __restrict__ big) {
 	const uint32_t p = blockIdx.x * 256u + threadIdx.x;
 	if (p >= n) return;
 	const uint32_t i = sorted[p];
@@ -147,21 +149,21 @@
 	const uint32_t c0 = cls == 0 ? 0u : cls == 1 ? hdr[0] : hdr[0] + hdr[1];
 	const size_t pos = (size_t)hdr[3 + cls] * kMTile + (p - c0);
 	const size_t tile = pos / kMTile;
-	cylm_store(rec + tile * kMTileQ, (uint32_t)(pos - tile * kMTile), q0, q1, S);
-}
-
-__global__ void __launch_bounds__(256) k_cylm_pad(const uint32_t* __restrict__ hdr, uint32_t n_tris, float4* __restrict__ rec) {
+	cylm_store(rec + tile * kMTileQ, grec + tile * (kMGroups * kMGrpQ), (uint32_t)(pos - tile * kMTile), q0, q1, S);
+}
+
+__global__ void __launch_bounds__(256) k_cylm_pad(const uint32_t* __restrict__ hdr, uint32_t n_tris, float4* __restrict__ rec, float4* __restrict__ grec) {
 	const uint32_t k = blockIdx.x, tid = threadIdx.x;
 	const uint32_t n = hdr[k], first = hdr[3 + k] * kMTile;
 	const float S = ((const float*)hdr)[7];
 	for (uint32_t pos = n + tid; pos < (n + kMTile - 1u) / kMTile * kMTile; pos += 256u) {
 		const size_t gpos = (size_t)first + pos, tile = gpos / kMTile;
-		cylm_store(rec + tile * kMTileQ, (uint32_t)(gpos - tile * kMTile), make_float4(0.0f, 0.0f, 0.0f, 0.0f),
+		cylm_store(rec + tile * kMTileQ, grec + tile * (kMGroups * kMGrpQ), (uint32_t)(gpos - tile * kMTile), make_float4(0.0f, 0.0f, 0.0f, 0.0f),
 		           make_float4(0.0f, -__builtin_inff(), __uint_as_float(n_tris), 0.0f), S);
 	}
 }
 
-__global__ void __launch_bounds__(kMGroups) k_cylm_hmax(const uint32_t* __restrict__ hdr, float4* __restrict__ rec) {
+__global__ void __launch_bounds__(kMGroups) k_cylm_hmax(const uint32_t* __restrict__ hdr, float4* __restrict__ rec, const float4* __restrict__ grec) {
 	__shared__ uint32_t s_max, s_min;
 	__shared__ float s_h[kMGroups];
 	if (blockIdx.x >= hdr[6]) return;
@@ -170,7 +172,8 @@
 	const uint32_t grp = threadIdx.x, tb = grp >> 3, j = (grp & 7u) >> 1, hh = grp & 1u;
 	const float S = ((const float*)hdr)[7];
 	const float k = S > 0.0f ? 256.0f / S : 1.0f;
-	const float4 a = tile[cylm_slot(grp, 4u)], b = tile[cylm_slot(grp, 5u)];
+	const float4* const G = grec + ((size_t)blockIdx.x * kMGroups + cylm_gpos(grp)) * kMGrpQ;
+	const float4 a = G[4], b = G[5];
 	s_h[grp] = fmaxf(fmaxf(a.y, a.w), fmaxf(b.y, b.w)) * k;
 	__syncthreads();
 	float hm = kMGrp == 8u ? fmaxf(s_h[grp], s_h[grp ^ 2u]) : s_h[grp];
@@ -192,16 +195,19 @@
 	typedef __attribute__((address_space(1))) const void* gptr_t;
 	typedef __attribute__((address_space(3))) void* lptr_t;
 #pragma unroll
-	for (int p = 0; p < (int)(kMTileQ / kMThreads); ++p)
+	for (int p = 0; p < (int)(kMStageQ / kMThreads); ++p)
 		__builtin_amdgcn_global_load_lds((gptr_t)(src + p * kMThreads + tid), (lptr_t)(dst + p * kMThreads + wbase), 16, 0, 0);
-}
-
-struct CylmGroup { float4 q0[4]; float4 mh01, mh23; };
-SP_DEV CylmGroup cylm_group(const float4* tile, uint32_t grp) {
+	constexpr uint32_t done = kMStageQ / kMThreads * kMThreads;
+	if (done + tid < kMStageQ)
+		__builtin_amdgcn_global_load_lds((gptr_t)(src + done + tid), (lptr_t)(dst + done + wbase), 16, 0, 0);
+}
+
+struct CylmGroup { float4 q0[4]; float4 mh01, mh23, idx; };
+SP_DEV CylmGroup cylm_group(const float4* __restrict__ g) {
 	CylmGroup G;
 #pragma unroll
-	for (int u = 0; u < 4; ++u) G.q0[u] = tile[cylm_slot(grp, (uint32_t)u)];
-	G.mh01 = tile[cylm_slot(grp, 4u)]; G.mh23 = tile[cylm_slot(grp, 5u)];
+	for (int u = 0; u < 4; ++u) G.q0[u] = g[u];
+	G.mh01 = g[4]; G.mh23 = g[5]; G.idx = g[6];
 	return G;
 }
 
@@ -327,8 +333,8 @@
 #endif
 }
 
-SP_DEV void cylm_tile_bound(const float4* cur, const CylmRay& R, float (&Dt)[2]) {
-	const float kappa = cur[cylm_kq()].x;
+SP_DEV void cylm_tile_bound(const float4* buf, uint32_t qoff, const CylmRay& R, float (&Dt)[2]) {
+	const float kappa = buf[qoff + cylm_kq()].x;
 #pragma unroll
 	for (int rb = 0; rb < 2; ++rb) Dt[rb] = __builtin_fmaf(R.Dqn[rb], kappa, R.Dn[rb]) * (1.0f + 0x1p-22f);
 }
@@ -360,10 +366,11 @@
 	return word;
 }
 
-SP_DEV void cylm_stage1(const float4* cur, uint32_t tb0, uint32_t nblk, uint32_t lane, const CylmRay& R, const float (&Dt)[2], uint32_t (&word)[2]) {
+SP_DEV void cylm_stage1(const float4* buf, uint32_t qoff, uint32_t tb0, uint32_t nblk, uint32_t lane, const CylmRay& R, const float (&Dt)[2], uint32_t (&word)[2]) {
 	if (nblk == 0u) return;
-	const half8* frags = (const half8*)(cur + kMRecQ) + tb0 * 64u + lane;
-	const float4* hmq = cur + cylm_hmq(tb0, lane >> 5);
+	const uint32_t fq = qoff + tb0 * 64u + lane, hq = qoff + cylm_hmq(tb0, lane >> 5);
+#define frags(i) (((const half8*)buf)[fq + (i)])
+#define hmq(i) (buf[hq + (i)])
 	float16v zero;
 #pragma unroll
 	for (int i = 0; i < 16; ++i) zero[i] = 0.0f;
@@ -376,28 +383,30 @@
 		word[1] = cylm_bits(g1, afr_cur_Hm, Dt[1], word[1]);                                 \
 		__builtin_amdgcn_sched_barrier(0);                                                   \
 		g1 = __builtin_amdgcn_mfma_f32_32x32x16_f16(afr_next, R.bfr[1], zero, 0, 0, 0);
-	half8 afrA = frags[0], afrB;
-	float4 HmA = hmq[0], HmB;
+	half8 afrA = frags(0u), afrB;
+	float4 HmA = hmq(0u), HmB;
 	float16v g0 = __builtin_amdgcn_mfma_f32_32x32x16_f16(afrA, R.bfr[0], zero, 0, 0, 0);
 	float16v g1 = __builtin_amdgcn_mfma_f32_32x32x16_f16(afrA, R.bfr[1], zero, 0, 0, 0);
 	uint32_t tb = 1;
 	for (; tb + 1u < nblk; tb += 2u) {
-		afrB = frags[tb * 64u]; HmB = hmq[tb * 2u];
+		afrB = frags(tb * 64u); HmB = hmq(tb * 2u);
 		SP_S1_STEP(HmA, afrB)
-		afrA = frags[(tb + 1u) * 64u]; HmA = hmq[(tb + 1u) * 2u];
+		afrA = frags((tb + 1u) * 64u); HmA = hmq((tb + 1u) * 2u);
 		SP_S1_STEP(HmB, afrA)
 	}
 	if (tb < nblk) {
-		afrB = frags[tb * 64u]; HmB = hmq[tb * 2u];
+		afrB = frags(tb * 64u); HmB = hmq(tb * 2u);
 		SP_S1_STEP(HmA, afrB)
 		HmA = HmB;
 	}
 #undef SP_S1_STEP
+#undef frags
+#undef hmq
 	word[0] = cylm_bits(g0, HmA, Dt[0], word[0]);
 	word[1] = cylm_bits(g1, HmA, Dt[1], word[1]);
 }
 
-constexpr uint32_t kMCap = 384u;
+constexpr uint32_t kMCap = 344u;
 constexpr uint32_t kMQ2 = 128u;
 constexpr uint32_t kMIdxBits = 26u;
 
@@ -417,8 +426,8 @@
 template <bool BOUNDED = false>
 SP_DEV void scan_cylm(const KArgs& a, const CylStream cs, float rv, const RaySlots<1>& s, float (&bd)[1], int (&bi)[1],
                       const float* tmax = nullptr, bool shadow = false) {
-	__shared__ float4 sm0[kMTileQ];
-	__shared__ float4 sm1[kMTileQ];
+	__shared__ float4 sm0[kMStageQ];
+	__shared__ float4 sm1[kMStageQ];
 	__shared__ unsigned short lst[kMWaves * kMCap];
 	__shared__ uint32_t q2[kMWaves * kMQ2];
 	__shared__ unsigned long long cell[kMThreads];
@@ -491,55 +500,64 @@
 	__syncthreads();
 	cylm_tile_dma(cs.rec, sm0, tid, wbase);
 	__syncthreads();
-	auto tile_body = [&](auto parity, const uint32_t gt) {
+	auto stage_body = [&](auto parity, const uint32_t gt) -> uint32_t {
 		const float4* const cur = decltype(parity)::value ? sm1 : sm0;
 		float4* const nxt = decltype(parity)::value ? sm0 : sm1;
-#ifndef SP_CYLM_LATE_DMA
-		if (gt + 1u < total_tiles) cylm_tile_dma(cs.rec + (size_t)(gt + 1u) * kMTileQ, nxt, tid, wbase);
-#endif
-		SP_PH_STAMP(ph_t0);
 		while (hd.next_class(gt)) {
 			const float t0 = f.Pa[0]; f.Pa[0] = f.Pb[0]; f.Pb[0] = f.Pc[0]; f.Pc[0] = t0;
 			R.build(hd.cls, lane);
 		}
-		const uint32_t nblk = hd.fragments(gt);
-		float Dt[2];
-		cylm_tile_bound(cur, R, Dt);
-		uint32_t word[kMWords][2];
-#pragma unroll
-		for (int w = 0; w < (int)kMWords; ++w) {
-			word[w][0] = word[w][1] = 0u;
-			const uint32_t tb0 = kMFragsPerWord * (uint32_t)w;
-			const uint32_t nb = nblk > tb0 ? (nblk - tb0 < kMFragsPerWord ? nblk - tb0 : kMFragsPerWord) : 0u;
-			cylm_stage1(cur, tb0, nb, lane, R, Dt, word[w]);
-			const uint32_t done = nb * kMBitsFrag;
-#pragma unroll
-			for (int rb = 0; rb < 2; ++rb) word[w][rb] = done == 0u ? 0u : (word[w][rb] << (32u - done));
+		const uint32_t nt = gt + 1u < hd.cend ? kMStage : 1u;
+#ifndef SP_CYLM_LATE_DMA
+		if (gt + nt < total_tiles) cylm_tile_dma(cs.rec + (size_t)(gt + nt) * kMTileQ, nxt, tid, wbase);
+#endif
+		SP_PH_STAMP(ph_t0);
+		uint32_t word[kMStage][kMWords][2];
+#pragma unroll
+		for (int t = 0; t < (int)kMStage; ++t) {
+			const uint32_t nblk = (uint32_t)t < nt ? hd.fragments(gt + (uint32_t)t) : 0u;
+			float Dt[2] = { 0.0f, 0.0f };
+			if ((uint32_t)t < nt) cylm_tile_bound(cur, (uint32_t)t * kMTileQ, R, Dt);
+#pragma unroll
+			for (int w = 0; w < (int)kMWords; ++w) {
+				word[t][w][0] = word[t][w][1] = 0u;
+				const uint32_t tb0 = kMFragsPerWord * (uint32_t)w;
+				const uint32_t nb = nblk > tb0 ? (nblk - tb0 < kMFragsPerWord ? nblk - tb0 : kMFragsPerWord) : 0u;
+				cylm_stage1(cur, (uint32_t)t * kMTileQ, tb0, nb, lane, R, Dt, word[t][w]);
+				const uint32_t done = nb * kMBitsFrag;
+#pragma unroll
+				for (int rb = 0; rb < 2; ++rb) word[t][w][rb] = done == 0u ? 0u : (word[t][w][rb] << (32u - done));
 #ifdef SP_DBG_ALLBITS
-			word[w][0] = word[w][1] = done == 0u ? 0u : (0xffffffffu << (32u - done));
-#endif
+				word[t][w][0] = word[t][w][1] = done == 0u ? 0u : (0xffffffffu << (32u - done));
+#endif
+			}
 		}
 		if (BOUNDED && shadow) {
 #pragma unroll
 			for (int rb = 0; rb < 2; ++rb) {
 				const bool fin = (uint32_t)cell[wbase + (lane & 31u) + 32u * (uint32_t)rb] != 0xffffffffu;
 #pragma unroll
-				for (int w = 0; w < (int)kMWords; ++w) word[w][rb] = fin ? 0u : word[w][rb];
+				for (int t = 0; t < (int)kMStage; ++t)
+#pragma unroll
+				for (int w = 0; w < (int)kMWords; ++w) word[t][w][rb] = fin ? 0u : word[t][w][rb];
 			}
 		}
 		SP_PH_STAMP(ph_t1); SP_PH_ADD(ph_s1, ph_t0, ph_t1);
 #ifdef SP_CYLM_LATE_DMA
-		if (gt + 1u < total_tiles) cylm_tile_dma(cs.rec + (size_t)(gt + 1u) * kMTileQ, nxt, tid, wbase);
-#endif
+		if (gt + nt < total_tiles) cylm_tile_dma(cs.rec + (size_t)(gt + nt) * kMTileQ, nxt, tid, wbase);
+#endif
+		const float4* const grec = cs.grp + (size_t)gt * (kMGroups * kMGrpQ);
 #ifdef SP_EXP_NO_STAGE2
-		for (int w = 0; w < (int)kMWords; ++w) exp_acc ^= word[w][0] ^ word[w][1];
+		for (int t = 0; t < (int)kMStage; ++t) for (int w = 0; w < (int)kMWords; ++w) exp_acc ^= word[t][w][0] ^ word[t][w][1];
 		for (; false;) {
 #else
 		for (;;) {
 #endif
 			uint32_t c = 0;
 #pragma unroll
-			for (int w = 0; w < (int)kMWords; ++w) c += (uint32_t)__builtin_popcount(word[w][0]) + (uint32_t)__builtin_popcount(word[w][1]);
+			for (int t = 0; t < (int)kMStage; ++t)
+#pragma unroll
+			for (int w = 0; w < (int)kMWords; ++w) c += (uint32_t)__builtin_popcount(word[t][w][0]) + (uint32_t)__builtin_popcount(word[t][w][1]);
 			const uint32_t incl = wave_incl_scan(c);
 			const uint32_t all = (uint32_t)__builtin_amdgcn_readlane((int)incl, 63);
 			if (all == 0u) break;
@@ -547,33 +565,37 @@
 			const uint32_t jend = incl < kMCap ? incl : kMCap;
 			if (all <= kMCap) {
 #pragma unroll
+				for (int t = 0; t < (int)kMStage; ++t)
+#pragma unroll
 				for (int w = 0; w < (int)kMWords; ++w)
 #pragma unroll
 				for (int rb = 0; rb < 2; ++rb) {
-					uint32_t m = word[w][rb];
-					const uint32_t eb = (((lane & 31u) + 32u * (uint32_t)rb) << 2) | ((16u * kMGrp * (uint32_t)w + hh) << 8);
+					uint32_t m = word[t][w][rb];
+					const uint32_t eb = (((lane & 31u) + 32u * (uint32_t)rb) << 2) | ((kMGroups * (uint32_t)t + 16u * kMGrp * (uint32_t)w + hh) << 8);
 					while (m != 0u) {
 						const uint32_t e = (uint32_t)__builtin_clz(m);
 						mylst[j++] = (unsigned short)(eb + (e << (kMGrp == 8u ? 10 : 9)));
 						m &= ~(0x80000000u >> e);
 					}
-					word[w][rb] = 0u;
+					word[t][w][rb] = 0u;
 				}
 			} else
 #pragma unroll
+			for (int t = 0; t < (int)kMStage; ++t)
+#pragma unroll
 			for (int w = 0; w < (int)kMWords; ++w)
 #pragma unroll
 			for (int rb = 0; rb < 2; ++rb) {
-				uint32_t m = word[w][rb];
+				uint32_t m = word[t][w][rb];
 				const uint32_t ray = (lane & 31u) + 32u * (uint32_t)rb;
 				while (__any(m != 0u && j < jend)) {
 					if (m != 0u && j < jend) {
 						const uint32_t e = (uint32_t)__builtin_clz(m);
-						mylst[j++] = (unsigned short)((ray << 2) | ((16u * kMGrp * (uint32_t)w + (kMGrp / 2u) * e + hh) << 8));
+						mylst[j++] = (unsigned short)((ray << 2) | ((kMGroups * (uint32_t)t + 16u * kMGrp * (uint32_t)w + (kMGrp / 2u) * e + hh) << 8));
 						m &= ~(0x80000000u >> e);
 					}
 				}
-				word[w][rb] = m;
+				word[t][w][rb] = m;
 			}
 			__builtin_amdgcn_wave_barrier();
 			const uint32_t total = all < kMCap ? all : kMCap;
@@ -586,25 +608,27 @@
 				const bool ok = ent < total;
 				const uint32_t entry = ok ? (uint32_t)mylst[ent] : (lane << 2);
 				const uint32_t la = entry & 0xfcu;
-				const uint32_t grp = entry >> 8;
+				const uint32_t gp = cylm_gpos(entry >> 8);
+				const float4* const g = (const float4*)((const char*)grec + (((gp << 3) - gp) << 4));
+				CylmGroup G[kMGrp / 4u];
+#pragma unroll
+				for (int h = 0; h < (int)(kMGrp / 4u); ++h) G[h] = cylm_group(g + kMGrpQ * (uint32_t)h);
 				const float dx = wave_fetch(la, s.dir[0].x), dy = wave_fetch(la, s.dir[0].y), dz = wave_fetch(la, s.dir[0].z);
 				const float Pa = wave_fetch(la, f.Pa[0]), Pb = wave_fetch(la, f.Pb[0]), Pc = wave_fetch(la, f.Pc[0]);
 				const float D = wave_fetch(la, f.D[0]), Dq = wave_fetch(la, f.Dq[0]);
 				uint32_t cand = 0;
 #pragma unroll
 				for (int h = 0; h < (int)(kMGrp / 4u); ++h) {
-					const CylmGroup G = cylm_group(cur, grp + 2u * (uint32_t)h);
 #pragma unroll
 					for (int u = 0; u < 4; ++u) {
-						const float mz = u == 0 ? G.mh01.x : u == 1 ? G.mh01.z : u == 2 ? G.mh23.x : G.mh23.z;
-						const float Hh = u == 0 ? G.mh01.y : u == 1 ? G.mh01.w : u == 2 ? G.mh23.y : G.mh23.w;
-						const float x = cyl_x(G.q0[u], mz, Hh, Pa, Pb, Pc, -dx, -dy, -dz, D);
+						const float mz = u == 0 ? G[h].mh01.x : u == 1 ? G[h].mh01.z : u == 2 ? G[h].mh23.x : G[h].mh23.z;
+						const float Hh = u == 0 ? G[h].mh01.y : u == 1 ? G[h].mh01.w : u == 2 ? G[h].mh23.y : G[h].mh23.w;
+						const float x = cyl_x(G[h].q0[u], mz, Hh, Pa, Pb, Pc, -dx, -dy, -dz, D);
 						cand = __builtin_amdgcn_alignbit(cand, __float_as_uint(x - Dq), 31);
 					}
 				}
 				cand = ok ? cand : 0u;
 				SP_PH_STAMP(ph_t1); SP_PH_ADD(ph_retest, ph_t0, ph_t1);
-				const uint32_t* const gidx = (const uint32_t*)(cur + cylm_slot(grp, 6u));
 				const uint32_t lhi = la << (kMIdxBits - 2u);
 				for (;;) {
 					const bool mine = cand != 0u;
@@ -614,7 +638,10 @@
 					if (q2n + cnt > kMQ2) exact_batch(64u);
 					const uint32_t k = mine ? (uint32_t)__builtin_ctz(cand) : kMGrp - 1u;
 					const uint32_t u = kMGrp - 1u - k;
-					const uint32_t idx = gidx[8u * (u >> 2) + (u & 3u)];
+					float4 ix = G[0].idx;
+					if constexpr (kMGrp == 8u) { const bool second = (u & 4u) != 0u; ix.x = second ? G[kMGrp / 4u - 1u].idx.x : ix.x; ix.y = second ? G[kMGrp / 4u - 1u].idx.y : ix.y; ix.z = second ? G[kMGrp / 4u - 1u].idx.z : ix.z; ix.w = second ? G[kMGrp / 4u - 1u].idx.w : ix.w; }
+					const float lo2 = (u & 1u) ? ix.y : ix.x, hi2 = (u & 1u) ? ix.w : ix.z;
+					const uint32_t idx = __float_as_uint((u & 2u) ? hi2 : lo2);
 					if (mine) myq2[q2n + __builtin_amdgcn_mbcnt_hi((uint32_t)(mk >> 32), __builtin_amdgcn_mbcnt_lo((uint32_t)mk, 0u))] = lhi | idx;
 					q2n += cnt;
 					cand &= cand - 1u;
@@ -630,30 +657,29 @@
 		while (q2n >= 64u) exact_batch(64u);
 #endif
 #ifdef SP_FILTER_STATS
-		if (lane == 0) atomicAdd(a.scans + 3, 1ull);
+		if (lane == 0) atomicAdd(a.scans + 3, (unsigned long long)nt);
 #endif
 		SP_PH_STAMP(ph_t0); SP_PH_ADD(ph_list, ph_t1, ph_t0);
 		if (BOUNDED && shadow) {
 			__asm__ volatile("s_waitcnt vmcnt(0)" ::: "memory");
-			if (!__syncthreads_or((uint32_t)cell[tid] == 0xffffffffu ? 1 : 0)) return false;
+			if (!__syncthreads_or((uint32_t)cell[tid] == 0xffffffffu ? 1 : 0)) return 0u;
 		} else
 		__syncthreads();
 		SP_PH_STAMP(ph_t1); SP_PH_ADD(ph_bar, ph_t0, ph_t1);
-		return true;
+		return nt;
 	};
-	if constexpr (BOUNDED) {
+	{
 		bool all_done = false;
-		for (uint32_t gt = 0; gt < total_tiles; gt += 2u) {
-			if (!tile_body(std::integral_constant<int, 0>{}, gt)) { all_done = true; break; }
-			if (gt + 1u < total_tiles && !tile_body(std::integral_constant<int, 1>{}, gt + 1u)) { all_done = true; break; }
+		for (uint32_t gt = 0; gt < total_tiles;) {
+			uint32_t nt = stage_body(std::integral_constant<int, 0>{}, gt);
+			if (BOUNDED && nt == 0u) { all_done = true; break; }
+			gt += nt;
+			if (gt >= total_tiles) break;
+			nt = stage_body(std::integral_constant<int, 1>{}, gt);
+			if (BOUNDED && nt == 0u) { all_done = true; break; }
+			gt += nt;
 		}
 		if (q2n && !all_done) exact_batch(q2n);
-	} else {
-		for (uint32_t gt = 0; gt < total_tiles; gt += 2u) {
-			tile_body(std::integral_constant<int, 0>{}, gt);
-			if (gt + 1u < total_tiles) tile_body(std::integral_constant<int, 1>{}, gt + 1u);
-		}
-		if (q2n) exact_batch(q2n);
 	}
 #ifdef SP_PHASE_TIMERS
 	if (lane == 0) {
@@ -691,14 +717,15 @@
 		__syncthreads();
 		for (uint32_t q = lane; q < kMTileQ; q += 64u) sm[q] = cs.rec[(size_t)gt * kMTileQ + q];
 		__syncthreads();
+		const float4* const grec = cs.grp + (size_t)gt * (kMGroups * kMGrpQ);
 		const uint32_t nblk = hd.fragments(gt);
 		float Dt[2];
-		cylm_tile_bound(sm, R, Dt);
+		cylm_tile_bound(sm, 0u, R, Dt);
 		for (uint32_t w = 0; w < kMWords; ++w) {
 			uint32_t word[2] = { 0u, 0u };
 			const uint32_t tb0 = kMFragsPerWord * w;
 			const uint32_t nb = nblk > tb0 ? (nblk - tb0 < kMFragsPerWord ? nblk - tb0 : kMFragsPerWord) : 0u;
-			cylm_stage1(sm, tb0, nb, lane, R, Dt, word);
+			cylm_stage1(sm, 0u, tb0, nb, lane, R, Dt, word);
 			const uint32_t done = nb * kMBitsFrag;
 #pragma unroll
 			for (int rb = 0; rb < 2; ++rb)
@@ -709,7 +736,7 @@
 #pragma unroll
 			for (int i = 0; i < 16; ++i) zero[i] = 0.0f;
 			for (uint32_t tb = 0; tb < kMBlocks; ++tb) {
-				const half8 afr = ((const half8*)(sm + kMRecQ))[tb * 64u + lane];
+				const half8 afr = ((const half8*)sm)[tb * 64u + lane];
 				const float16v g0 = __builtin_amdgcn_mfma_f32_32x32x16_f16(afr, R.bfr[0], zero, 0, 0, 0);
 				const float16v g1 = __builtin_amdgcn_mfma_f32_32x32x16_f16(afr, R.bfr[1], zero, 0, 0, 0);
 #pragma unroll
@@ -719,7 +746,7 @@
 #pragma unroll
 					for (int j = 0; j < 4; ++j) {
 						const uint32_t grp = tb * 8u + 2u * (uint32_t)j + hh;
-						const float4 a = sm[cylm_slot(grp, 4u)], b = sm[cylm_slot(grp, 5u)];
+						const float4 a = grec[cylm_gpos(grp) * kMGrpQ + 4u], b = grec[cylm_gpos(grp) * kMGrpQ + 5u];
 						const float H4[4] = { a.y * kH, a.w * kH, b.y * kH, b.w * kH };
 #pragma unroll
 						for (int i = 0; i < 4; ++i) {
@@ -737,7 +764,7 @@
 		}
 		if (blockIdx.x == 0) {
 			for (uint32_t grp = lane; grp < kMGroups; grp += 64u) {
-				const float4 gi = sm[cylm_slot(grp, 6u)];
+				const float4 gi = grec[cylm_gpos(grp) * kMGrpQ + 6u];
 				int* o = out_order + (size_t)gt * kMTile + 4u * grp;
 				o[0] = (int)__float_as_uint(gi.x); o[1] = (int)__float_as_uint(gi.y); o[2] = (int)__float_as_uint(gi.z); o[3] = (int)__float_as_uint(gi.w);
 			}
diff --git a/spath_amd/csrc/spath_hip.hip b/spath_amd/csrc/spath_hip.hip
--- a/spath_amd/csrc/spath_hip.hip
+++ b/spath_amd/csrc/spath_hip.hip
@@ -37,7 +37,7 @@
 	int device = 0;
 	hipStream_t own_stream = nullptr;
 	hipEvent_t ev_k0 = nullptr, ev_k1 = nullptr, ev_u0 = nullptr, ev_u1 = nullptr, ev_d0 = nullptr, ev_d1 = nullptr;
-	DevBuf tris, mats, scan, filt, bounds, samp, rays, rgba, accum, counter, work, bvh_nodes, bvh_rec, bvh_idx, sort_kv, sort_hist, bvh_meta, cyl_rec, cyl_cnt, cyl_hdr, prim, cylm_rec, cylm_hdr, cylm_big;
+	DevBuf tris, mats, scan, filt, bounds, samp, rays, rgba, accum, counter, work, bvh_nodes, bvh_rec, bvh_idx, sort_kv, sort_hist, bvh_meta, cyl_rec, cyl_cnt, cyl_hdr, prim, cylm_rec, cylm_grp, cylm_hdr, cylm_big;
 	bool bvh_valid = false, filt_valid = false, cyl_valid = false, cylm_valid = false;
 	bool cylm_wide = false;
 	uint32_t bvh_leaves = 0;
@@ -192,13 +192,15 @@
 	const uint32_t n = (uint32_t)c->n_tris, nblocks = (n + 255) / 256, max_tiles = n / SP_CM(kMTile) + 4;
 	int rc;
 	if ((rc = ensure(c, c->sort_kv, (size_t)n * 16)) || (rc = ensure(c, c->cylm_hdr, 256)) || (rc = ensure(c, c->cylm_big, sp::cylm256::kMBig * 48)) ||
-	    (rc = ensure(c, c->cylm_rec, (size_t)max_tiles * SP_CM(kMTileQ) * 16))) return rc;
+	    (rc = ensure(c, c->cylm_rec, (size_t)max_tiles * SP_CM(kMTileQ) * 16)) ||
+	    (rc = ensure(c, c->cylm_grp, (size_t)max_tiles * SP_CM(kMGroups) * SP_CM(kMGrpQ) * 16))) return rc;
 	uint32_t* keys = (uint32_t*)c->sort_kv.p;
 	uint32_t* vals = (uint32_t*)c->sort_kv.p + (size_t)2 * n;
 	uint32_t* hdr = (uint32_t*)c->cylm_hdr.p;
 	const float* tris = (const float*)c->tris.p;
 	const unsigned int* bnd = (const unsigned int*)c->bounds.p;
 	float4* rec = (float4*)c->cylm_rec.p;
+	float4* grec = (float4*)c->cylm_grp.p;
 	HIP_TRY(c, hipMemsetAsync(hdr, 0, 256, st));
 	hipLaunchKernelGGL(sp::cylm256::k_cylm_count_big, dim3(nblocks), dim3(256), 0, st, tris, n, bnd, hdr);
 	hipLaunchKernelGGL(sp::cylm256::k_cylm_keys, dim3(nblocks), dim3(256), 0, st, tris, n, bnd, keys, vals, hdr);
@@ -207,14 +209,14 @@
 	const uint32_t* sorted = vals + (size_t)half * n;
 	if (WIDE) {
 		hipLaunchKernelGGL(sp::cylm512::k_cylm_hdr, dim3(1), dim3(1), 0, st, hdr, bnd);
-		hipLaunchKernelGGL(sp::cylm512::k_cylm_scatter, dim3(nblocks), dim3(256), 0, st, tris, n, sorted, (const uint32_t*)hdr, rec, (const float4*)c->scan.p, (float4*)c->cylm_big.p);
-		hipLaunchKernelGGL(sp::cylm512::k_cylm_pad, dim3(3), dim3(256), 0, st, (const uint32_t*)hdr, n, rec);
-		hipLaunchKernelGGL(sp::cylm512::k_cylm_hmax, dim3(max_tiles), dim3(sp::cylm512::kMGroups), 0, st, (const uint32_t*)hdr, rec);
+		hipLaunchKernelGGL(sp::cylm512::k_cylm_scatter, dim3(nblocks), dim3(256), 0, st, tris, n, sorted, (const uint32_t*)hdr, rec, grec, (const float4*)c->scan.p, (float4*)c->cylm_big.p);
+		hipLaunchKernelGGL(sp::cylm512::k_cylm_pad, dim3(3), dim3(256), 0, st, (const uint32_t*)hdr, n, rec, grec);
+		hipLaunchKernelGGL(sp::cylm512::k_cylm_hmax, dim3(max_tiles), dim3(sp::cylm512::kMGroups), 0, st, (const uint32_t*)hdr, rec, (const float4*)grec);
 	} else {
 		hipLaunchKernelGGL(sp::cylm256::k_cylm_hdr, dim3(1), dim3(1), 0, st, hdr, bnd);
-		hipLaunchKernelGGL(sp::cylm256::k_cylm_scatter, dim3(nblocks), dim3(256), 0, st, tris, n, sorted, (const uint32_t*)hdr, rec, (const float4*)c->scan.p, (float4*)c->cylm_big.p);
-		hipLaunchKernelGGL(sp::cylm256::k_cylm_pad, dim3(3), dim3(256), 0, st, (const uint32_t*)hdr, n, rec);
-		hipLaunchKernelGGL(sp::cylm256::k_cylm_hmax, dim3(max_tiles), dim3(sp::cylm256::kMGroups), 0, st, (const uint32_t*)hdr, rec);
+		hipLaunchKernelGGL(sp::cylm256::k_cylm_scatter, dim3(nblocks), dim3(256), 0, st, tris, n, sorted, (const uint32_t*)hdr, rec, grec, (const float4*)c->scan.p, (float4*)c->cylm_big.p);
+		hipLaunchKernelGGL(sp::cylm256::k_cylm_pad, dim3(3), dim3(256), 0, st, (const uint32_t*)hdr, n, rec, grec);
+		hipLaunchKernelGGL(sp::cylm256::k_cylm_hmax, dim3(max_tiles), dim3(sp::cylm256::kMGroups), 0, st, (const uint32_t*)hdr, rec, (const float4*)grec);
 	}
 #undef SP_CM
 	HIP_TRY(c, hipGetLastError());
@@ -542,6 +544,7 @@
 	src2.cylm.rec = (const float4*)c->cylm_rec.p;
 	src2.cylm.hdr = (const uint32_t*)c->cylm_hdr.p;
 	src2.cylm.big = (const float4*)c->cylm_big.p;
+	src2.cylm.grp = (const float4*)c->cylm_grp.p;
 	const unsigned int* bnd = (const unsigned int*)c->bounds.p;
 	sp::BvhArgs B{};
 	if (variant == kVariantAccel) {
@@ -1405,7 +1408,7 @@
 	(void)hipSetDevice(c->device);
 	if (c->own_stream) (void)hipStreamSynchronize(c->own_stream);
 	DevBuf* bufs[] = { &c->tris, &c->mats, &c->scan, &c->filt, &c->bounds, &c->samp, &c->rays, &c->rgba, &c->accum, &c->counter, &c->work,
-	                   &c->bvh_nodes, &c->bvh_rec, &c->bvh_idx, &c->sort_kv, &c->sort_hist, &c->bvh_meta, &c->cyl_rec, &c->cyl_cnt, &c->cyl_hdr, &c->prim, &c->cylm_rec, &c->cylm_hdr, &c->cylm_big,
+	                   &c->bvh_nodes, &c->bvh_rec, &c->bvh_idx, &c->sort_kv, &c->sort_hist, &c->bvh_meta, &c->cyl_rec, &c->cyl_cnt, &c->cyl_hdr, &c->prim, &c->cylm_rec, &c->cylm_grp, &c->cylm_hdr, &c->cylm_big,
 	                   &c->acc_rays, &c->acc_sum, &c->adp_s12, &c->adp_cnt, &c->adp_list[0], &c->adp_list[1], &c->adp_rays, &c->adp_keep,
 	                   &c->adp_blk, &c->adp_nact_d, &c->adp_wst, &c->dn_cls, &c->dn_hit, &c->dn_gbuf, &c->dn_a, &c->dn_b, &c->dn_rays, &c->nee_tab, &c->spec };
 	for (auto b : bufs) if (b->p) (void)hipFree(b->p);
@@ -1772,7 +1775,7 @@
 	if (e == hipSuccess) e = hipMalloc(&d_order, order_b);
 	if (e == hipSuccess) e = hipMemcpyAsync(d_rays, rays, n_rays * 24, hipMemcpyHostToDevice, st);
 	if (e == hipSuccess) {
-		sp::CylStream cs{ (const float4*)c->cylm_rec.p, (const uint32_t*)c->cylm_hdr.p, (const float4*)c->cylm_big.p };
+		sp::CylStream cs{ (const float4*)c->cylm_rec.p, (const uint32_t*)c->cylm_hdr.p, (const float4*)c->cylm_big.p, (const float4*)c->cylm_grp.p };
 		if (c->cylm_wide)
 			hipLaunchKernelGGL(sp::cylm512::k_selftest_stage1, dim3((unsigned)(n_rays / 64)), dim3(64), 0, st, (const float*)d_rays, (uint32_t)n_rays, cs,
 		                   (const unsigned int*)c->bounds.p, (uint32_t*)d_words, (uint32_t*)d_tri, (int*)d_order);
```
